# LPMP/BDD

Hardware: AMD Instinct MI355X
Metric: parallel-MMA iterations/sec, 10.5M BDD nodes, 1 GPU (+ achieved HBM GB/s in roofline) (higher is better)
Workload: dtype f32

## Files before the change

### bdd_amd/capi.py

```python
from __future__ import annotations

import ctypes as C
import os
import subprocess

_HERE = os.path.dirname(os.path.abspath(__file__))
LIB_PATH = os.path.abspath(os.environ["BDDMMA_LIB"]) if os.environ.get("BDDMMA_LIB") else os.path.join(_HERE, "csrc", "libbdd_mma_hip.so")

OK = 0
ERR_INVALID_ARGUMENT, ERR_INVALID_BDD, ERR_DEVICE, ERR_STATE, ERR_UNSUPPORTED, ERR_IO = -1, -2, -3, -4, -5, -6
F32, F64 = 0, 1
K_FORWARD_MM, K_BACKWARD_MM, K_FINISH_DELTA, K_OTHER, K_COUNT = 0, 1, 2, 3, 4


class Options(C.Structure):
    _fields_ = [("pack_width", C.c_uint32), ("wide_pack_width", C.c_uint32), ("deterministic", C.c_uint32),
                ("vars_per_bin", C.c_uint32), ("stage_cap", C.c_uint32), ("waves_per_block", C.c_uint32),
                ("keep_bdd_order", C.c_uint32), ("resident_sweeps", C.c_uint32), ("exchange_by_variable", C.c_uint32),
                ("variant_flags", C.c_uint32), ("pack_fill", C.c_uint32), ("pack_stagger", C.c_uint32)]


class LbfgsParams(C.Structure):
    _fields_ = [("history_size", C.c_int32), ("init_step_size", C.c_double), ("req_rel_lb_increase", C.c_double),
                ("step_size_decrease_factor", C.c_double), ("step_size_increase_factor", C.c_double)]


class LbfgsState(C.Structure):
    _fields_ = [("step_size", C.c_double), ("last_applied_step", C.c_double), ("mma_iterations", C.c_uint64),
                ("lbfgs_iterations", C.c_uint64), ("history_entries", C.c_int32), ("num_unsuccessful_updates", C.c_int32),
                ("last_kind", C.c_int32), ("last_trials", C.c_int32)]


class RunResult(C.Structure):
    _fields_ = [("iterations", C.c_uint64), ("lb_initial", C.c_double), ("lb_final", C.c_double),
                ("seconds", C.c_double), ("stop_reason", C.c_int32)]


class Profile(C.Structure):
    _fields_ = [("launches", C.c_uint64 * K_COUNT), ("total_ms", C.c_double * K_COUNT)]


_V, _U64, _I, _D = C.c_void_p, C.c_uint64, C.c_int, C.c_double
SIGNATURES = {
    "bddmma_create": (_I, [C.POINTER(_V), _I, _I, _V, _V, _U64, _V, _U64, C.POINTER(Options)]),
    "bddmma_destroy": (None, [_V]),
    "bddmma_device_count": (_I, []),
    "bddmma_device_chip": (_I, [_I, C.POINTER(C.c_uint32), C.POINTER(C.c_uint32), C.POINTER(C.c_uint64)]),
    "bddmma_set_layout_threads": (_I, [_I]),
    "bddmma_set_thread_layout_threads": (_I, [_I]),
    "bddmma_last_error": (C.c_char_p, [_V]),
    "bddmma_nr_variables": (_U64, [_V]),
    "bddmma_nr_bdds": (_U64, [_V]),
    "bddmma_nr_layers": (_U64, [_V]),
    "bddmma_nr_bdd_nodes": (_U64, [_V]),
    "bddmma_nr_hops": (_U64, [_V]),
    "bddmma_nr_packs": (_U64, [_V]),
    "bddmma_solve_sweep_kind": (_I, [_V]),
    "bddmma_fused_small": (_I, [_V]),
    "bddmma_nontemporal_loads": (_I, [_V]),
    "bddmma_precision": (_I, [_V]),
    "bddmma_device": (_I, [_V]),
    "bddmma_num_bdds_per_var": (_I, [_V, _V]),
    "bddmma_layer_variables": (_I, [_V, _V]),
    "bddmma_layer_bdds": (_I, [_V, _V]),
    "bddmma_nodes_per_hop": (_I, [_V, _V]),
    "bddmma_layers_per_hop": (_I, [_V, _V]),
    "bddmma_update_costs": (_I, [_V, _V, _U64, _V, _U64, _I, _I]),
    "bddmma_set_cost": (_I, [_V, _D, _U64]),
    "bddmma_get_solver_costs": (_I, [_V, _V, _V, _V, _I]),
    "bddmma_set_solver_costs": (_I, [_V, _V, _V, _V, _I]),
    "bddmma_primal_objective_vec": (_I, [_V, _V, _I]),
    "bddmma_forward_run": (_I, [_V]),
    "bddmma_backward_run": (_I, [_V]),
    "bddmma_lower_bound": (_I, [_V, C.POINTER(_D)]),
    "bddmma_lower_bound_per_bdd": (_I, [_V, _V, _I]),
    "bddmma_iteration": (_I, [_V, _D]),
    "bddmma_iterations": (_I, [_V, _D, _U64]),
    "bddmma_learned_iterations": (_I, [_V, _V, _I, _U64, _D, _D, _V, _V, _V, _U64, _D, _I, C.POINTER(_U64)]),
    "bddmma_learned_iterations_omega_vec": (_I, [_V, _V, _I, _U64, _V, _I, _D, _V, _V, _V, _U64, _D, _I, C.POINTER(_U64)]),
    "bddmma_isotropic_dist_weights": (_I, [_V, _V, _I]),
    "bddmma_forward_mm": (_I, [_V, _D, _V, _I]),
    "bddmma_backward_mm": (_I, [_V, _D, _V, _I]),
    "bddmma_normalize_delta": (_I, [_V, _V, _I]),
    "bddmma_distribute_delta": (_I, [_V]),
    "bddmma_get_delta": (_I, [_V, _V, _I]),
    "bddmma_set_delta": (_I, [_V, _V, _I]),
    "bddmma_min_marginals": (_I, [_V, _I, _V, _V, _V, _I]),
    "bddmma_min_marginal_diff": (_I, [_V, _V, _I]),
    "bddmma_sum_marginals": (_I, [_V, _I, _I, _V, _V, _V, _I]),
    "bddmma_smooth_solution": (_I, [_V, _V, _I]),
    "bddmma_grad_min_marginal_diff": (_I, [_V, _V, _V, _V, _I]),
    "bddmma_grad_lower_bound_per_bdd": (_I, [_V, _V, _V, _V, _I, _I]),
    "bddmma_grad_distribute_delta": (_I, [_V, _V, _V, _V, _I]),
    "bddmma_grad_cost_perturbation": (_I, [_V, _V, _V, _V, _V, _I]),
    "bddmma_grad_learned_iterations": (_I, [_V, _V, _I, _D, _V, _I, _V, _V, _V, _V, _V, _U64, _U64, _U64, _I]),
    "bddmma_bdds_solution": (_I, [_V, _I, _V, _I]),
    "bddmma_net_solver_costs": (_I, [_V, _V, _I]),
    "bddmma_make_dual_feasible": (_I, [_V, _V, _I]),
    "bddmma_gradient_step": (_I, [_V, _V, _D, _I]),
    "bddmma_lbfgs_create": (_I, [C.POINTER(_V), _V, C.POINTER(LbfgsParams)]),
    "bddmma_lbfgs_destroy": (None, [_V]),
    "bddmma_lbfgs_iteration": (_I, [_V]),
    "bddmma_lbfgs_update_costs": (_I, [_V, _V, _U64, _V, _U64, _I, _I]),
    "bddmma_lbfgs_flush": (_I, [_V]),
    "bddmma_lbfgs_get_state": (_I, [_V, C.POINTER(LbfgsState)]),
    "bddmma_perturb_primal_costs": (_I, [_V, _V, _D, C.c_uint32, C.c_uint32, C.POINTER(C.c_uint32), _V, _V, _V]),
    "bddmma_run_solver": (_I, [_V, _V, _U64, _D, _D, _D, _I, C.POINTER(RunResult)]),
    "bddmma_run_solver_host_loop": (_I, [_V, _V, _U64, _D, _D, _D, _I, C.POINTER(RunResult)]),
    "bddmma_batch_create": (_I, [C.POINTER(_V), C.POINTER(_V), _U64]),
    "bddmma_batch_destroy": (None, [_V]),
    "bddmma_batch_last_error": (C.c_char_p, [_V]),
    "bddmma_batch_size": (_U64, [_V]),
    "bddmma_batch_iterations": (_I, [_V, _D, _U64]),
    "bddmma_batch_time_iterations": (_I, [_V, _D, _U64, C.POINTER(_D)]),
    "bddmma_batch_run_solver": (_I, [_V, _U64, _D, _D, _D, C.POINTER(RunResult)]),
    "bddmma_batch_lower_bounds": (_I, [_V, C.POINTER(_D)]),
    "bddmma_incremental_mm_agreement_rounding": (_I, [_V, _V, _D, _D, _U64, _U64, C.c_uint32, _I, _V, C.POINTER(_I)]),
    "bddmma_save": (_I, [_V, C.c_char_p]),
    "bddmma_load": (_I, [C.POINTER(_V), _I, C.c_char_p]),
    "bddmma_synchronize": (_I, [_V]),
    "bddmma_set_profiling": (_I, [_V, _I]),
    "bddmma_get_profile": (_I, [_V, C.POINTER(Profile)]),
    "bddmma_time_iterations": (_I, [_V, _D, _U64, C.POINTER(_D)]),
    "bddmma_time_kernel": (_I, [_V, _I, _U64, C.POINTER(_D)]),
    "bddmma_device_bytes": (_U64, [_V]),
    "bddmma_device_allocated_bytes": (_U64, [_V]),
    "bddmma_layout_create": (_I, [C.POINTER(_V), _V, _V, _U64, C.POINTER(Options)]),
    "bddmma_layout_create_for_chip": (_I, [C.POINTER(_V), _V, _V, _U64, C.POINTER(Options), _I, C.c_uint32, C.c_uint32]),
    "bddmma_layout_destroy": (None, [_V]),
    "bddmma_layout_size": (_U64, [_V, _I]),
    "bddmma_layout_copy": (_I, [_V, _I, _V]),
    "bddmma_layout_res2_records": (_I, [_V, _I, _V, _V, _V]),
    "bddmma_layout_stream_records": (_I, [_V, _I, _V, _V, _V]),
    "bddmma_layout_layer_records": (_I, [_V, _I, _V, _V, _V]),
    "bddmma_layout_seg_exchange": (_I, [_V, _I, _I, _V, _V, _V, _V]),
}

_I64P, _U64P = C.POINTER(C.c_int64), C.POINTER(C.c_uint64)
ILP_SIGNATURES = {
    "bddilp_last_error": (C.c_char_p, []),
    "bddilp_parse_lp": (_I, [C.c_char_p, C.POINTER(_V)]),
    "bddilp_parse_opb": (_I, [C.c_char_p, C.POINTER(_V)]),
    "bddilp_parse": (_I, [C.c_char_p, C.POINTER(_V)]),
    "bddilp_destroy": (None, [_V]),
    "bddilp_nr_variables": (_U64, [_V]),
    "bddilp_nr_constraints": (_U64, [_V]),
    "bddilp_variable_name": (C.c_char_p, [_V, _U64]),
    "bddilp_objective": (_I, [_V, _V, C.POINTER(_D)]),
    "bddilp_constraint_size": (_U64, [_V, _U64]),
    "bddilp_constraint": (_I, [_V, _U64, _V, _V, C.POINTER(_I), C.POINTER(C.c_int64)]),
    "bddilp_constraint_name": (C.c_char_p, [_V, _U64]),
    "bddilp_normalize": (_I, [_V]),
    "bddilp_to_bdds": (_I, [_V, _I, _U64, C.POINTER(_V)]),
    "bddilp_bdds_create": (_I, [C.POINTER(_V)]),
    "bddilp_bdds_add_row": (_I, [_V, _V, _V, _U64, _I, C.c_int64, C.POINTER(_I)]),
    "bddilp_bdds_split": (_I, [_V, _U64, _U64, _I, _U64P, _U64P]),
    "bddilp_bdds_destroy": (None, [_V]),
    "bddilp_bdds_nr_bdds": (_U64, [_V]),
    "bddilp_bdds_nr_instructions": (_U64, [_V]),
    "bddilp_bdds_nr_variables": (_U64, [_V]),
    "bddilp_bdds_instructions": (_V, [_V]),
    "bddilp_bdds_delimiters": (_V, [_V]),
    "bddilp_write_bdd_lp": (_I, [_V, _V, _U64, _V, _U64, C.c_char_p]),
    "bddilp_export_graphviz": (_I, [_V, _V, _U64, _U64, C.c_char_p]),
    "bddilp_random_set_cover": (_I, [_U64, _U64, _U64, _U64, _V, _V]),
}

_lib = None


def build(verbose: bool = False) -> None:
    out = subprocess.run(["make", "-C", os.path.join(_HERE, "csrc"), "-j4"], capture_output=True, text=True)
    if out.returncode != 0:
        raise RuntimeError("building libbdd_mma_hip.so failed:\n" + out.stdout + out.stderr)
    if verbose:
        print(out.stdout)


def lib():
    global _lib
    if _lib is None:
        if not os.path.exists(LIB_PATH):
            raise RuntimeError(f"{LIB_PATH} is missing: run `make -C bdd_amd/csrc` (or __graft_entry__.build()); "
                               "bdd_amd has no CPU fallback")
        L = C.CDLL(LIB_PATH)
        for name, (res, args) in list(SIGNATURES.items()) + list(ILP_SIGNATURES.items()):
            f = getattr(L, name)
            f.restype = res
            f.argtypes = args
        _lib = L
    return _lib


class BddMmaError(RuntimeError):
    pass


def check(rc: int, handle=None):
    if rc != OK:
        msg = lib().bddmma_last_error(handle)
        raise BddMmaError(f"bdd_mma error {rc}: {msg.decode() if msg else ''}")
```

### bdd_amd/csrc/capi.cpp

```cpp
#include <chrono>
#include <cmath>
#include <cstdio>
#include <cstdlib>
#include <cstring>
#include <limits>
#include <new>
#include <string>
#include <vector>

#include "../../include/bdd_mma.h"
#include "layout.hpp"
#include "solver.hpp"

using namespace bddmma;

struct bddmma_lbfgs;
extern "C" int bddmma_lbfgs_iteration(bddmma_lbfgs* l);
extern "C" int bddmma_lbfgs_update_costs(bddmma_lbfgs* l, const void* lo, uint64_t n_lo, const void* hi, uint64_t n_hi, int elem_precision,
                                         int on_device);

namespace {
thread_local std::string g_err;

template <typename F>
int guarded(bddmma_solver* s, F&& f)
{
    if (!s || !s->impl) return BDDMMA_ERR_INVALID_ARGUMENT;
    try {
        return f(s->impl);
    } catch (const std::bad_alloc&) {
        s->impl->err = "out of host memory";
        return BDDMMA_ERR_DEVICE;
    } catch (const std::exception& e) {
        s->impl->err = e.what();
        return BDDMMA_ERR_DEVICE;
    }
}
template <typename F>
int guarded(const bddmma_solver* s, F&& f) { return guarded(const_cast<bddmma_solver*>(s), f); }

template <typename F>
int guarded_batch(bddmma_batch* b, F&& f)
{
    if (!b || !b->impl) return BDDMMA_ERR_INVALID_ARGUMENT;
    try {
        return f(b->impl);
    } catch (const std::exception& e) {
        b->impl->err = e.what();
        return BDDMMA_ERR_DEVICE;
    }
}

template <typename T>
int copy_host(const std::vector<T>& v, T* out)
{
    if (!out) return BDDMMA_ERR_INVALID_ARGUMENT;
    if (!v.empty()) std::memcpy(out, v.data(), v.size() * sizeof(T));
    return BDDMMA_OK;
}
}

extern "C" {

int bddmma_create(bddmma_solver** out, int precision, int device, const bddmma_instruction* instr,
                  const uint64_t* bdd_delims, uint64_t n_bdds, const double* costs_hi, uint64_t n_costs,
                  const bddmma_options* opts)
{
    if (!out) return BDDMMA_ERR_INVALID_ARGUMENT;
    *out = nullptr;
    try {
#ifdef BDDMMA_EXPERIMENTAL
        static const bool timing = std::getenv("BDDMMA_LAYOUT_TIMING") != nullptr;
#else
        constexpr bool timing = false;
#endif
        auto t_last = std::chrono::steady_clock::now();
        auto lap = [&](const char* what) {
            if (!timing) return;
            const auto now = std::chrono::steady_clock::now();
            std::fprintf(stderr, "[create] %-28s %8.1f ms\n", what, std::chrono::duration<double, std::milli>(now - t_last).count());
            t_last = now;
        };
        HostLayout L;
        ChipInfo chip;
        int rc = query_chip(device, &chip, g_err);
        if (rc) return rc;
        rc = build_layout(instr, bdd_delims, n_bdds, opts, L, g_err, false, precision == BDDMMA_F64 ? 8 : 4, chip);
        if (rc) return rc;
        lap("host layout");
        SolverBase* impl = nullptr;
        rc = create_solver(&impl, precision, device, L, opts, g_err);
        if (rc) return rc;
        lap("device buffers + upload");
        impl->n_packs_narrow = L.narrow.n_packs();
        impl->n_packs_wide = L.wide.n_packs() + L.huge.n_packs();
        if (costs_hi && n_costs) {
            rc = impl->update_costs(nullptr, 0, costs_hi, n_costs, BDDMMA_F64, 0);
            if (rc) {
                g_err = impl->err;
                delete impl;
                return rc;
            }
        }
        lap("update_costs");
        *out = new bddmma_solver{impl};
        return BDDMMA_OK;
    } catch (const std::exception& e) {
        g_err = e.what();
        return BDDMMA_ERR_DEVICE;
    }
}

int bddmma_device_count(void) { return device_count(); }
int bddmma_device_chip(int device, uint32_t* n_cus, uint32_t* lds_bytes_per_cu, uint64_t* max_resident_threads)
{
    if (device < 0 || device >= device_count()) { g_err = "no such HIP device"; return BDDMMA_ERR_DEVICE; }
    ChipInfo chip;
    const int rc = query_chip(device, &chip, g_err);
    if (rc) return rc;
    if (n_cus) *n_cus = chip.n_cus;
    if (lds_bytes_per_cu) *lds_bytes_per_cu = chip.lds_bytes;
    if (max_resident_threads) *max_resident_threads = chip.max_resident_threads;
    return BDDMMA_OK;
}
int bddmma_set_layout_threads(int n)
{
    if (n < 0) return BDDMMA_ERR_INVALID_ARGUMENT;
    set_layout_threads((unsigned)n);
    return BDDMMA_OK;
}
int bddmma_set_thread_layout_threads(int n)
{
    if (n < 0) return BDDMMA_ERR_INVALID_ARGUMENT;
    set_thread_layout_threads((unsigned)n);
    return BDDMMA_OK;
}

void bddmma_destroy(bddmma_solver* s)
{
    if (!s) return;
    delete s->impl;
    delete s;
}

const char* bddmma_last_error(const bddmma_solver* s) { return (s && s->impl) ? s->impl->err.c_str() : g_err.c_str(); }

uint64_t bddmma_nr_variables(const bddmma_solver* s) { return s && s->impl ? s->impl->n_vars : 0; }
uint64_t bddmma_nr_bdds(const bddmma_solver* s) { return s && s->impl ? s->impl->n_bdds : 0; }
uint64_t bddmma_nr_layers(const bddmma_solver* s) { return s && s->impl ? s->impl->n_layers : 0; }
uint64_t bddmma_nr_bdd_nodes(const bddmma_solver* s) { return s && s->impl ? s->impl->n_input_nodes : 0; }
uint64_t bddmma_nr_hops(const bddmma_solver* s) { return s && s->impl ? s->impl->n_hops : 0; }
uint64_t bddmma_nr_packs(const bddmma_solver* s) { return s && s->impl ? s->impl->n_packs_narrow + s->impl->n_packs_wide : 0; }
int bddmma_solve_sweep_kind(const bddmma_solver* s) { return s && s->impl ? s->impl->solve_sweep_kind : -1; }
int bddmma_fused_small(const bddmma_solver* s) { return s && s->impl ? (s->impl->fused_small ? 1 : 0) : -1; }
int bddmma_nontemporal_loads(const bddmma_solver* s) { return s && s->impl ? (s->impl->nt_loads ? 1 : 0) : -1; }
int bddmma_precision(const bddmma_solver* s) { return s && s->impl ? s->impl->precision : -1; }
int bddmma_device(const bddmma_solver* s) { return s && s->impl ? s->impl->device : -1; }
uint64_t bddmma_device_bytes(const bddmma_solver* s) { return s && s->impl ? s->impl->dev_bytes : 0; }
uint64_t bddmma_device_allocated_bytes(const bddmma_solver* s) { return s && s->impl ? s->impl->dev_alloc_bytes : 0; }

int bddmma_num_bdds_per_var(const bddmma_solver* s, int32_t* out)
{
    return guarded(s, [&](SolverBase* b) { return copy_host(b->h_nbdds, out); });
}
int bddmma_layer_variables(const bddmma_solver* s, int32_t* out)
{
    return guarded(s, [&](SolverBase* b) { return copy_host(b->h_layer_var, out); });
}
int bddmma_layer_bdds(const bddmma_solver* s, int32_t* out)
{
    return guarded(s, [&](SolverBase* b) { return copy_host(b->h_layer_bdd, out); });
}
int bddmma_nodes_per_hop(const bddmma_solver* s, uint64_t* out)
{
    return guarded(s, [&](SolverBase* b) { return copy_host(b->nodes_per_hop, out); });
}
int bddmma_layers_per_hop(const bddmma_solver* s, uint64_t* out)
{
    return guarded(s, [&](SolverBase* b) { return copy_host(b->layers_per_hop, out); });
}

int bddmma_update_costs(bddmma_solver* s, const void* lo, uint64_t n_lo, const void* hi, uint64_t n_hi,
                        int elem_precision, int on_device)
{
    return guarded(s, [&](SolverBase* b) {
        if (elem_precision != BDDMMA_F32 && elem_precision != BDDMMA_F64) {
            b->err = "elem_precision must be BDDMMA_F32 or BDDMMA_F64";
            return BDDMMA_ERR_INVALID_ARGUMENT;
        }
        return b->update_costs(lo, n_lo, hi, n_hi, elem_precision, on_device);
    });
}
int bddmma_set_cost(bddmma_solver* s, double c, uint64_t var)
{
    return guarded(s, [&](SolverBase* b) { return b->set_cost(c, var); });
}
int bddmma_get_solver_costs(const bddmma_solver* s, void* lo, void* hi, void* mm, int on_device)
{
    return guarded(s, [&](SolverBase* b) { return b->get_solver_costs(lo, hi, mm, on_device); });
}
int bddmma_set_solver_costs(bddmma_solver* s, const void* lo, const void* hi, const void* mm, int on_device)
{
    return guarded(s, [&](SolverBase* b) { return b->set_solver_costs(lo, hi, mm, on_device); });
}
int bddmma_primal_objective_vec(bddmma_solver* s, void* out, int on_device)
{
    return guarded(s, [&](SolverBase* b) { return b->primal_objective_vec(out, on_device); });
}
int bddmma_forward_run(bddmma_solver* s) { return guarded(s, [&](SolverBase* b) { return b->forward_run(); }); }
int bddmma_backward_run(bddmma_solver* s) { return guarded(s, [&](SolverBase* b) { return b->backward_run(); }); }
int bddmma_lower_bound(bddmma_solver* s, double* lb)
{
    return guarded(s, [&](SolverBase* b) { return lb ? b->lower_bound(lb) : BDDMMA_ERR_INVALID_ARGUMENT; });
}
int bddmma_lower_bound_per_bdd(bddmma_solver* s, void* out, int on_device)
{
    return guarded(s, [&](SolverBase* b) { return b->lower_bound_per_bdd(out, on_device); });
}
int bddmma_iteration(bddmma_solver* s, double omega)
{
    return guarded(s, [&](SolverBase* b) { return b->iteration(omega); });
}
int bddmma_iterations(bddmma_solver* s, double omega, uint64_t n)
{
    return guarded(s, [&](SolverBase* b) { return b->iterations(omega, n); });
}
int bddmma_learned_iterations(bddmma_solver* s, const void* dist_weights, int weights_on_device, uint64_t num_itr, double omega,
                              double improvement_slope, void* sol_avg, void* lb_first_diff_avg, void* lb_second_diff_avg,
                              uint64_t compute_history_for_itr, double history_avg_beta, int outputs_on_device, uint64_t* itr_done)
{
    return guarded(s, [&](SolverBase* b) {
        return b->learned_iterations(dist_weights, weights_on_device, num_itr, omega, improvement_slope, sol_avg, lb_first_diff_avg,
                                     lb_second_diff_avg, compute_history_for_itr, history_avg_beta, outputs_on_device, itr_done, nullptr, 0);
    });
}
int bddmma_learned_iterations_omega_vec(bddmma_solver* s, const void* dist_weights, int weights_on_device, uint64_t num_itr, const void* omega_vec,
                                        int omega_vec_on_device, double improvement_slope, void* sol_avg, void* lb_first_diff_avg,
                                        void* lb_second_diff_avg, uint64_t compute_history_for_itr, double history_avg_beta, int outputs_on_device,
                                        uint64_t* itr_done)
{
    return guarded(s, [&](SolverBase* b) {
        if (!omega_vec) {
            if (itr_done) *itr_done = 0;
            b->err = "learned_iterations: omega_vec is null";
            return BDDMMA_ERR_INVALID_ARGUMENT;
        }
        return b->learned_iterations(dist_weights, weights_on_device, num_itr, 0.0, improvement_slope, sol_avg, lb_first_diff_avg,
                                     lb_second_diff_avg, compute_history_for_itr, history_avg_beta, outputs_on_device, itr_done, omega_vec,
                                     omega_vec_on_device);
    });
}
int bddmma_isotropic_dist_weights(bddmma_solver* s, void* out, int on_device)
{
    return guarded(s, [&](SolverBase* b) { return out ? b->isotropic_dist_weights(out, on_device) : BDDMMA_ERR_INVALID_ARGUMENT; });
}
int bddmma_forward_mm(bddmma_solver* s, double omega, void* d, int on_device)
{
    return guarded(s, [&](SolverBase* b) { return d ? b->forward_mm(omega, d, on_device) : BDDMMA_ERR_INVALID_ARGUMENT; });
}
int bddmma_backward_mm(bddmma_solver* s, double omega, void* d, int on_device)
{
    return guarded(s, [&](SolverBase* b) { return d ? b->backward_mm(omega, d, on_device) : BDDMMA_ERR_INVALID_ARGUMENT; });
}
int bddmma_normalize_delta(const bddmma_solver* s, void* d, int on_device)
{
    return guarded(s, [&](SolverBase* b) { return d ? b->normalize_delta(d, on_device) : BDDMMA_ERR_INVALID_ARGUMENT; });
}
int bddmma_distribute_delta(bddmma_solver* s) { return guarded(s, [&](SolverBase* b) { return b->distribute_delta(); }); }
int bddmma_get_delta(const bddmma_solver* s, void* out, int on_device)
{
    return guarded(s, [&](SolverBase* b) { return out ? b->get_delta(out, on_device) : BDDMMA_ERR_INVALID_ARGUMENT; });
}
int bddmma_set_delta(bddmma_solver* s, const void* in, int on_device)
{
    return guarded(s, [&](SolverBase* b) { return in ? b->set_delta(in, on_device) : BDDMMA_ERR_INVALID_ARGUMENT; });
}
int bddmma_min_marginals(bddmma_solver* s, int sorted, int32_t* var, void* mm0, void* mm1, int on_device)
{
    return guarded(s, [&](SolverBase* b) { return b->min_marginals(sorted, var, mm0, mm1, on_device); });
}
int bddmma_min_marginal_diff(bddmma_solver* s, void* out, int on_device)
{
    return guarded(s, [&](SolverBase* b) { return out ? b->min_marginal_diff(out, on_device) : BDDMMA_ERR_INVALID_ARGUMENT; });
}
int bddmma_sum_marginals(bddmma_solver* s, int sorted, int log_probs, int32_t* var, void* sm0, void* sm1, int on_device)
{
    return guarded(s, [&](SolverBase* b) { return (sm0 && sm1) ? b->sum_marginals(sorted, log_probs, var, sm0, sm1, on_device) : BDDMMA_ERR_INVALID_ARGUMENT; });
}
int bddmma_smooth_solution(bddmma_solver* s, void* out, int on_device)
{
    return guarded(s, [&](SolverBase* b) { return out ? b->smooth_solution(out, on_device) : BDDMMA_ERR_INVALID_ARGUMENT; });
}
int bddmma_grad_min_marginal_diff(bddmma_solver* s, const void* grad_mm, void* grad_lo_out, void* grad_hi_out, int on_device)
{
    return guarded(s, [&](SolverBase* b) {
        return (grad_mm && grad_lo_out && grad_hi_out) ? b->grad_min_marginal_diff(grad_mm, grad_lo_out, grad_hi_out, on_device) : BDDMMA_ERR_INVALID_ARGUMENT;
    });
}
int bddmma_grad_lower_bound_per_bdd(bddmma_solver* s, const void* grad_lb_per_bdd, void* grad_lo_out, void* grad_hi_out, int smooth, int on_device)
{
    return guarded(s, [&](SolverBase* b) {
        return (grad_lb_per_bdd && grad_lo_out && grad_hi_out) ? b->grad_lower_bound_per_bdd(grad_lb_per_bdd, grad_lo_out, grad_hi_out, smooth, on_device)
                                                               : BDDMMA_ERR_INVALID_ARGUMENT;
    });
}
int bddmma_grad_distribute_delta(bddmma_solver* s, const void* grad_lo, const void* grad_hi, void* grad_deferred_mm_out, int on_device)
{
    return guarded(s, [&](SolverBase* b) {
// ... 671 lines not shown
```

### bdd_amd/csrc/kernels/common.hpp

```cpp
#pragma once

namespace bddmma {

enum : int { FWD_PLAIN = 0, FWD_SOLVE = 1, FWD_SOLUTION = 2 };
enum : int { BWD_PLAIN = 0, BWD_SOLVE = 1, BWD_MARGINALS = 2 };

template <typename REAL>
struct DevPtrs {
    const uint32_t* nwords;
    uint32_t n_nwords;
    const uint64_t* wwords;
    uint32_t wide_slot_base;
    REAL* F;
    REAL* T;
    REAL* lohi;
    const REAL* delta_lay;
    REAL* mm_binned;
    const uint32_t* lpos;
    const uint32_t* cs_entry;
    const uint16_t* cs_slot;
    uint32_t n_slots;
    uint32_t n_layers;
    uint32_t n_narrow_layers;
    double* lb_partial;
    REAL* x_layer;
    union {
        REAL* mm0_out;
        const REAL* omega_lay;
    };
    REAL* mm1_out;
    char* sol_out;
    const uint32_t* stop;
    uint32_t run_iter;
    uint32_t big;
};
struct RunGate {
    const uint32_t* stop = nullptr;
    uint32_t iter = 0;
};
constexpr uint32_t RUN_NOT_STOPPED = 0xFFFFFFFFu;

__device__ __forceinline__ bool run_stopped(const RunGate& g) { return g.stop != nullptr && *g.stop <= g.iter; }
#define BDDMMA_EXIT_IF(done_cond, dev)                                     \
    {                                                                      \
        const bool done_ = (done_cond);                                    \
        if (done_ | ((dev).stop != nullptr)) {                             \
            if (done_ || *(dev).stop <= (dev).run_iter) return;            \
        }                                                                  \
    }

struct PackDev {
    const uint32_t* pack_hop_ptr;
    const uint32_t* hop_node_off;
    const uint32_t* hop_layer_off;
    const uint8_t* pack_steps;
    const uint16_t* hop_root;
    const uint32_t* pack_word_off;
    const uint32_t* pack_group_ptr;
    const uint32_t* grp_layer_off;
    const uint32_t* grp_hop_end;
    const uint32_t* quad_round_ptr;
    const uint32_t* cs_ptr;
    uint32_t stage_cap;
    uint32_t seg_off;
    uint32_t n_packs;
    uint32_t lb_base;
    uint32_t nt_potentials;
    uint32_t xcd_chunk;
    const uint32_t* hdr_pack;
    const uint32_t* hdr_quad;
};

#ifdef BDDMMA_STAMPS
__device__ unsigned long long* g_bddmma_stamps = nullptr;
#define BDDMMA_STAMP(slot, idx)                                                                              \
    do {                                                                                                     \
        if (g_bddmma_stamps != nullptr) {                                                                    \
            asm volatile("s_waitcnt vmcnt(0) lgkmcnt(0)" ::: "memory");                                      \
            const unsigned long long t_ = __builtin_amdgcn_s_memrealtime();                      \
            if ((threadIdx.x & 63) == 0) g_bddmma_stamps[(size_t)(slot) * 8 + (idx)] = t_;                   \
        }                                                                                                    \
    } while (0)
#else
#define BDDMMA_STAMP(slot, idx) do { } while (0)
#endif

template <typename REAL> struct Pair;
template <> struct Pair<float> { using type = float2; };
template <> struct Pair<double> { using type = double2; };

template <typename REAL> __device__ __forceinline__ REAL inf_v();
template <> __device__ __forceinline__ float inf_v<float>() { return __builtin_huge_valf(); }
template <> __device__ __forceinline__ double inf_v<double>() { return __builtin_huge_val(); }

__device__ __forceinline__ float rmin(float a, float b) { return __builtin_fminf(a, b); }
__device__ __forceinline__ double rmin(double a, double b) { return __builtin_fmin(a, b); }
__device__ __forceinline__ bool rfinite(float a) { return __builtin_isfinite(a); }
__device__ __forceinline__ bool rfinite(double a) { return __builtin_isfinite(a); }

template <typename REAL>
__device__ __forceinline__ REAL mm_diff(REAL m0, REAL m1, REAL omega)
{
    const bool fin = (int)rfinite(m0) & (int)rfinite(m1);
    const REAL t = omega * (m1 - m0);
    return fin ? t : REAL(0);
}
template <bool OV, typename REAL>
__device__ __forceinline__ REAL omega_of(const DevPtrs<REAL>& d, REAL omega, uint32_t l)
{
    if constexpr (OV) return d.omega_lay[l];
    else return omega;
}
__device__ __forceinline__ float min0(float x)
{
    float r;
    asm("v_min_f32_e64 %0, %1, 0" : "=v"(r) : "v"(x));
    return r;
}
__device__ __forceinline__ float min0_neg(float x)
{
    float r;
    asm("v_min_f32_e64 %0, -%1, 0" : "=v"(r) : "v"(x));
    return r;
}
__device__ __forceinline__ double min0(double x) { return rmin(x, 0.0); }
__device__ __forceinline__ double min0_neg(double x) { return rmin(-x, 0.0); }

template <typename REAL>
__device__ __forceinline__ void lds_min(REAL* p, REAL v)
{
    __hip_atomic_fetch_min(p, v, __ATOMIC_RELAXED, __HIP_MEMORY_SCOPE_WORKGROUP);
}

template <bool GLOBAL, typename REAL>
__device__ __forceinline__ void frontier_min(REAL* p, REAL v)
{
    if (GLOBAL) __hip_atomic_fetch_min(p, v, __ATOMIC_RELAXED, __HIP_MEMORY_SCOPE_AGENT);
    else __hip_atomic_fetch_min(p, v, __ATOMIC_RELAXED, __HIP_MEMORY_SCOPE_WORKGROUP);
}
template <bool GLOBAL, typename REAL>
__device__ __forceinline__ REAL frontier_load(const REAL* p)
{
    if (GLOBAL) return __hip_atomic_load(p, __ATOMIC_RELAXED, __HIP_MEMORY_SCOPE_AGENT);
    return *p;
}

__device__ __forceinline__ uint32_t block_to_pack(uint32_t bid, uint32_t n_packs, uint32_t chunk)
{
    if (chunk == 0) {
        const uint32_t per = (n_packs + 7u) >> 3;
        return (bid & 7u) * per + (bid >> 3);
    }
    const uint32_t x = bid & 7u, i = bid >> 3;
    return ((i / chunk) * 8u + x) * chunk + i % chunk;
}

__device__ __forceinline__ float dpp_from_next(float v)
{
    const int x = __builtin_bit_cast(int, v);
    return __builtin_bit_cast(float, __builtin_amdgcn_update_dpp(x, x, 0x130, 0xF, 0xF, false));
}
__device__ __forceinline__ float dpp_from_prev(float v)
{
    const int x = __builtin_bit_cast(int, v);
    return __builtin_bit_cast(float, __builtin_amdgcn_update_dpp(x, x, 0x138, 0xF, 0xF, false));
}
__device__ __forceinline__ double dpp_from_next(double v)
{
    const long long x = __builtin_bit_cast(long long, v);
    const int lo = (int)x, hi = (int)(x >> 32);
    const unsigned int l2 = (unsigned int)__builtin_amdgcn_update_dpp(lo, lo, 0x130, 0xF, 0xF, false);
    const unsigned int h2 = (unsigned int)__builtin_amdgcn_update_dpp(hi, hi, 0x130, 0xF, 0xF, false);
    return __builtin_bit_cast(double, ((unsigned long long)h2 << 32) | l2);
}
#ifndef BDDMMA_SEG_FOLD_F32
#define BDDMMA_SEG_FOLD_F32 2
#endif
template <typename REAL>
constexpr int SEG_FOLD_STEPS = sizeof(REAL) == 4 ? BDDMMA_SEG_FOLD_F32 : 1;
template <int CTRL>
__device__ __forceinline__ float dpp_row(float v)
{
    const int x = __builtin_bit_cast(int, v);
    return __builtin_bit_cast(float, __builtin_amdgcn_update_dpp(x, x, CTRL, 0xF, 0xF, false));
}
template <int CTRL>
__device__ __forceinline__ double dpp_row(double v)
{
    const long long x = __builtin_bit_cast(long long, v);
    const int lo = (int)x, hi = (int)(x >> 32);
    const unsigned int l2 = (unsigned int)__builtin_amdgcn_update_dpp(lo, lo, CTRL, 0xF, 0xF, false);
    const unsigned int h2 = (unsigned int)__builtin_amdgcn_update_dpp(hi, hi, CTRL, 0xF, 0xF, false);
    return __builtin_bit_cast(double, ((unsigned long long)h2 << 32) | l2);
}
__device__ __forceinline__ double dpp_from_prev(double v)
{
    const long long x = __builtin_bit_cast(long long, v);
    const int lo = (int)x, hi = (int)(x >> 32);
    const unsigned int l2 = (unsigned int)__builtin_amdgcn_update_dpp(lo, lo, 0x138, 0xF, 0xF, false);
    const unsigned int h2 = (unsigned int)__builtin_amdgcn_update_dpp(hi, hi, 0x138, 0xF, 0xF, false);
    return __builtin_bit_cast(double, ((unsigned long long)h2 << 32) | l2);
}

__device__ __forceinline__ void seg_fence()
{
    __builtin_amdgcn_fence(__ATOMIC_RELEASE, "wavefront");
    __builtin_amdgcn_wave_barrier();
    __builtin_amdgcn_fence(__ATOMIC_ACQUIRE, "wavefront");
}
__device__ __forceinline__ void seg_pair_min(double& a, double& b, uint32_t pos, uint32_t len)
{
    const double a2 = dpp_from_next(a), b2 = dpp_from_next(b);
    if (pos == 0 && len == 2) {
        a = rmin(a, a2);
        b = rmin(b, b2);
    }
    const double a1 = dpp_from_prev(a), b1 = dpp_from_prev(b);
    if (pos == 1) {
        a = a1;
        b = b1;
    }
}
__device__ __forceinline__ void seg_pair_min(float& a, float& b, uint32_t pos, uint32_t len)
// ... 247 lines not shown
```

### bdd_amd/csrc/kernels/narrow3.hpp

```cpp
#pragma once

namespace bddmma {

constexpr int N3_W = 128;
template <typename REAL>
__device__ __forceinline__ void lds_ld2(REAL& a, REAL& b, const unsigned char* lds, uint32_t off)
{
    const REAL* p = reinterpret_cast<const REAL*>(lds + off);
    a = p[0];
    b = p[1];
}

template <typename REAL, bool NT>
__device__ __forceinline__ void pot_pair_load(typename Pair<REAL>::type& v, rsrc_t rh, uint32_t voff, uint32_t soff)
{
    constexpr int AUX = NT ? 2 : BDDMMA_LD_POT_AUX;
    if constexpr (sizeof(REAL) == 4) v = __builtin_bit_cast(float2, __builtin_amdgcn_raw_buffer_load_b64(rh, voff, soff, AUX));
    else v = __builtin_bit_cast(double2, __builtin_amdgcn_raw_buffer_load_b128(rh, voff, soff, AUX));
}

__device__ __forceinline__ void pot_store(float v, rsrc_t rh, uint32_t voff, uint32_t soff, uint32_t ) { hop_store(v, rh, voff, soff); }
__device__ __forceinline__ void pot_store(double v, rsrc_t rh, uint32_t voff, uint32_t soff, uint32_t nt)
{
    if (nt) hop_store<2>(v, rh, voff, soff);
    else hop_store<>(v, rh, voff, soff);
}

template <typename REAL>
__device__ __forceinline__ void pot_store_layer(REAL a, REAL b, bool two, rsrc_t rh, uint32_t off_a, uint32_t soff, uint32_t nt)
{
    using P2 = typename Pair<REAL>::type;
    const uint32_t off2 = two ? off_a : (uint32_t)LREC_NO_STORE, off1 = two ? (uint32_t)LREC_NO_STORE : off_a;
    P2 v;
    v.x = a;
    v.y = b;
    if constexpr (sizeof(REAL) == 4) {
        using u2 = decltype(__builtin_amdgcn_raw_buffer_load_b64(rh, 0, 0, 0));
        __builtin_amdgcn_raw_buffer_store_b64(__builtin_bit_cast(u2, v), rh, off2, soff, BDDMMA_ST_FT_AUX_F32);
        pot_store(a, rh, off1, soff, nt);
    } else {
        using u4 = decltype(__builtin_amdgcn_raw_buffer_load_b128(rh, 0, 0, 0));
        const u4 data = __builtin_bit_cast(u4, v);
        if (nt) __builtin_amdgcn_raw_buffer_store_b128(data, rh, off2, soff, 2);
        else __builtin_amdgcn_raw_buffer_store_b128(data, rh, off2, soff, BDDMMA_ST_AUX);
        asm volatile("s_nop 0" ::"v"(data) : "memory");
        pot_store(a, rh, off1, soff, nt);
    }
}

#ifndef BDDMMA_N3_LOOKAHEAD
#define BDDMMA_N3_LOOKAHEAD(REAL) (sizeof(REAL) == 8 ? 2 : BDDMMA_LOOKAHEAD)
#endif
template <typename REAL, int WPB, bool NT = false, int LA = BDDMMA_LOOKAHEAD, bool OV = false>
__device__ __forceinline__ void fwd_narrow3_body(const DevPtrs<REAL>& d, const PackDev& pk, const uint32_t* __restrict__ lrec,
                                                 const uint32_t* __restrict__ lrec_off, uint32_t lrec_words, REAL omega, uint32_t block_id)
{
    constexpr int W = N3_W;
    constexpr uint32_t S = sizeof(REAL);
    constexpr uint32_t BUF = (W + 128) * S;
    using P2 = typename Pair<REAL>::type;
    extern __shared__ __attribute__((aligned(16))) unsigned char dyn_lds[];
    P2* sD = reinterpret_cast<P2*>(dyn_lds);
    __shared__ __attribute__((aligned(16))) unsigned char sF_[WPB][2][BUF];
    __shared__ __attribute__((aligned(16))) unsigned char sT_[WPB][2][BUF];
    __shared__ uint32_t sOffN_[WPB][HOP_WIN], sOffL_[WPB][HOP_WIN], sOffR_[WPB][HOP_WIN];
    const uint32_t tid = threadIdx.x;
    const int wave = __builtin_amdgcn_readfirstlane((int)(tid >> 6));
    const int lane = tid & 63;
    unsigned char* sFw = &sF_[wave][0][0];
    unsigned char* sTw = &sT_[wave][0][0];
    const uint32_t n_quads = (pk.n_packs + WPB - 1) / WPB;
    const uint32_t quad = block_to_pack(block_id, n_quads, pk.xcd_chunk);
    BDDMMA_EXIT_IF(quad >= n_quads, d)
    const uint32_t p = quad * WPB + wave;
    const bool has_pack = p < pk.n_packs;
    const bool hdr = pk.hdr_pack != nullptr;
    const uint32_t* const hp = hdr ? pk.hdr_pack + 8 * (size_t)(has_pack ? p : 0) : nullptr;
    const uint32_t q0 = !has_pack ? 0 : (hdr ? hp[4] : pk.pack_hop_ptr[p]);
    const uint32_t q1 = !has_pack ? 0 : (hdr ? q0 + (hp[5] & 0xFFFFu) : pk.pack_hop_ptr[p + 1]);
    const uint32_t rbase = has_pack ? lrec_off[p] : 0;
    const uint32_t c0_h = hdr ? pk.hdr_quad[4 * (size_t)quad] : 0, cnt_h = hdr ? pk.hdr_quad[4 * (size_t)quad + 1] : 0;
    BDDMMA_STAMP(p, 0);
    const REAL INF = inf_v<REAL>();
    const uint32_t slot_first = !has_pack ? 0 : (hdr ? hp[0] : pk.hop_node_off[q0]), l0 = !has_pack ? 0 : (hdr ? hp[2] : pk.hop_layer_off[q0]);
    NarrowRs<REAL> rs(d);
    rs.rebase_layers(d, l0);
    uint32_t ent[STAGE_ITERS], esl[STAGE_ITERS];
    if (hdr) stage_load_tables<REAL, WPB, (NT ? 2 : BDDMMA_LD_TAB_AUX)>(ent, esl, rs, c0_h, cnt_h, tid);
    REAL* const Tp = d.T + slot_first;
    REAL* const Fp = d.F + slot_first;
    const REAL* const lohi_p = d.lohi + 2 * (size_t)l0;
    const rsrc_t rr = make_rsrc(lrec, lrec_words);
    HopWindow hw{sOffN_[wave], sOffL_[wave], sOffR_[wave], q0, q1, slot_first, l0};
    constexpr int D = LA;
    uint32_t o[2 * D + 3];
    uint32_t lb[D + 2];
    u4v rc[2 * D + 1];
    P2 tr[D + 1];
    P2 Lr[D + 1];
    REAL Wr[OV ? D + 1 : 1];
    const rsrc_t rw = omega_rsrc<OV>(d, l0);
#pragma unroll
    for (int i = 0; i < 2 * D + 3; ++i) o[i] = 0;
#pragma unroll
    for (int i = 0; i < D + 2; ++i) lb[i] = 0;
    auto ldrec = [&](uint32_t h) { return __builtin_amdgcn_raw_buffer_load_b128(rr, (uint32_t)lane * 16u, (rbase + h * 64u) * 16u, 0); };
    const uint32_t sink = (W + 2 * (uint32_t)lane) * S;
    if (has_pack) {
        hw.fill(pk, q0, lane);
#pragma unroll
        for (int i = 0; i < 2 * D + 3; ++i) o[i] = hw.node_off(q0 + i);
#pragma unroll
        for (int i = 0; i < D + 2; ++i) lb[i] = hw.layer_off(q0 + i);
#pragma unroll
        for (int r = 0; r < 2; ++r) {
            const uint32_t j = lane + 64 * r;
            lds_st<REAL>(sFw, j * S, (j < o[1] - o[0]) ? REAL(0) : INF);
        }
#pragma unroll
        for (int b = 0; b < 2; ++b) {
            lds_st<REAL>(sTw, b * BUF + sink, REAL(0));
            lds_st<REAL>(sTw, b * BUF + sink + S, INF);
        }
#pragma unroll
        for (int i = 0; i < 2 * D; ++i) rc[i] = ldrec((uint32_t)i);
        {
            P2 t1;
            pot_pair_load<REAL, NT>(t1, hop_rsrc(Tp, o[1], o[2] - o[1]), 2u * (uint32_t)lane * S, o[1] * S);
#pragma unroll
            for (int i = 0; i < D; ++i) pot_pair_load<REAL, NT>(tr[i], hop_rsrc(Tp, o[i + 2], o[i + 3] - o[i + 2]), 2u * (uint32_t)lane * S, o[i + 2] * S);
            if (2u * (uint32_t)lane < o[2] - o[1]) lds_st<P2>(sTw, 2u * (uint32_t)lane * S, t1);
        }
#pragma unroll
        for (int i = 0; i < D; ++i) hop_load(Lr[i], rs.lohi, (uint32_t)lane * (uint32_t)sizeof(P2), lb[i] * (uint32_t)sizeof(P2));
        if constexpr (OV) {
#pragma unroll
            for (int i = 0; i < D; ++i) hop_load(Wr[i], rw, (uint32_t)lane * S, lb[i] * S);
        }
        wave_sync();
    } else {
#pragma unroll
        for (int i = 0; i < 2 * D; ++i) rc[i] = u4v{0u, 0u, 0u, 0u};
    }
    uint32_t cur = 0;
    uint32_t q = q0;
    const uint32_t g0 = (has_pack && !hdr) ? pk.pack_group_ptr[p] : 0;
    const uint32_t ng = !has_pack ? 0 : (hdr ? 1u : pk.pack_group_ptr[p + 1] - g0);
    const uint32_t r0 = hdr ? 0 : pk.quad_round_ptr[quad];
    const uint32_t n_rounds = hdr ? 1u : pk.quad_round_ptr[quad + 1] - r0;
    const uint32_t db = (uint32_t)wave * pk.stage_cap * (uint32_t)sizeof(P2);
    for (uint32_t k = 0; k < n_rounds; ++k) {
    uint32_t gl0 = 0, cnt = 0, qe = q1;
    if (hdr) {
        cnt = cnt_h;
        stage_load_pairs<REAL, WPB>(sD, ent, esl, rs, cnt, tid);
        qe = has_pack ? q1 : q;
    } else {
        const uint32_t c0 = pk.cs_ptr[r0 + k];
        cnt = pk.cs_ptr[r0 + k + 1] - c0;
        stage_load<REAL, WPB, (NT ? 2 : BDDMMA_LD_TAB_AUX)>(sD, ent, esl, rs, c0, cnt, tid);
        if (k < ng) {
            gl0 = pk.grp_layer_off[g0 + k] - l0;
            qe = pk.grp_hop_end[g0 + k];
        } else {
            qe = q;
        }
    }
    if (WPB > 1) __syncthreads(); else wave_sync();
    BDDMMA_STAMP(p, 1);
    auto hop = [&]() {
        if (q + 2 * D + 3 >= hw.base + HOP_WIN && hw.base + HOP_WIN <= q1) hw.fill(pk, q, lane);
        const uint32_t nb = o[0];
        const uint32_t n3 = o[3] - o[2];
        const uint32_t fc = cur * BUF, fn = (cur ^ 1u) * BUF;
        const uint32_t stg = db + (lb[0] - gl0 + (uint32_t)lane) * (uint32_t)sizeof(P2);
        rc[2 * D] = ldrec(q - q0 + 2 * D);
#ifndef BDDMMA_EXP_NO_HOP_LOADS
        pot_pair_load<REAL, NT>(tr[D], hop_rsrc(Tp, o[D + 2], o[D + 3] - o[D + 2]), 2u * (uint32_t)lane * S, o[D + 2] * S);
        hop_load(Lr[D], rs.lohi, (uint32_t)lane * (uint32_t)sizeof(P2), lb[D] * (uint32_t)sizeof(P2));
        if constexpr (OV) hop_load(Wr[D], rw, (uint32_t)lane * S, lb[D] * S);
#endif
        const u4v ra = rc[0];
        const P2 c = Lr[0];
        const uint32_t flags = ra[2] >> 16;
        REAL fa, fb;
        lds_ld2(fa, fb, sFw, fc + (ra[2] & 0xFFFFu));
        const REAL tla = lds_ld<REAL>(sTw, fc + (ra[0] & 0xFFFFu)), tha = lds_ld<REAL>(sTw, fc + (ra[0] >> 16));
        const REAL tlb = lds_ld<REAL>(sTw, fc + (ra[1] & 0xFFFFu)), thb = lds_ld<REAL>(sTw, fc + (ra[1] >> 16));
        const P2 dd = lds_ld<P2>(dyn_lds, stg);
        const uint32_t o_new = hw.node_off(q + 2 * D + 3);
        const uint32_t l_next = hw.layer_off(q + D + 2);
        if (2u * (uint32_t)lane < n3) lds_st<P2>(sTw, fn + 2u * (uint32_t)lane * S, tr[0]);
        lds_st<P2>(sFw, fn + 2u * (uint32_t)lane * S, P2{INF, INF});
        wave_sync();
        fa = (flags & LREC_REAL) ? fa : INF;
        fb = (flags & LREC_TWO) ? fb : INF;
        const REAL m0 = rmin((fa + c.x) + tla, (fb + c.x) + tlb);
        const REAL m1 = rmin((fa + c.y) + tha, (fb + c.y) + thb);
        const REAL mm = mm_diff1(m0, m1, OV ? Wr[0] : omega);
        P2 nc;
        nc.x = (c.x + min0(mm)) + dd.x;
        nc.y = (c.y + min0_neg(mm)) + dd.y;
#ifndef BDDMMA_EXP_NO_HOP_STORES
        const rsrc_t rl = hop_rsrc(reinterpret_cast<const P2*>(lohi_p), lb[0], lb[1] - lb[0]);
        hop_store(nc, rl, (uint32_t)lane * (uint32_t)sizeof(P2), lb[0] * (uint32_t)sizeof(P2));
#endif
        if (flags & LREC_REAL) lds_st<REAL>(dyn_lds, stg, mm);
        lds_min(reinterpret_cast<REAL*>(sFw + fn + (ra[0] & 0xFFFFu)), fa + nc.x);
        lds_min(reinterpret_cast<REAL*>(sFw + fn + (ra[0] >> 16)), fa + nc.y);
        lds_min(reinterpret_cast<REAL*>(sFw + fn + (ra[1] & 0xFFFFu)), fb + nc.x);
        lds_min(reinterpret_cast<REAL*>(sFw + fn + (ra[1] >> 16)), fb + nc.y);
#ifndef BDDMMA_EXP_NO_HOP_STORES
        {
            const rsrc_t rf = hop_rsrc(Fp, nb, o[1] - o[0]);
            pot_store_layer<REAL>(fa, fb, (flags & LREC_TWO) != 0, rf, ra[3] & 0xFFFFu, nb * S, pk.nt_potentials);
        }
#endif
        wave_sync();
        cur ^= 1u;
        shift(o, o_new);
        shift(lb, l_next);
        shift(rc);
        shift(Lr);
        shift(tr);
        shift(Wr);
        ++q;
    };
    while (q + HOP_UNROLL <= qe) {
#pragma unroll
        for (int u = 0; u < HOP_UNROLL; ++u) hop();
    }
    while (q < qe) hop();
    BDDMMA_STAMP(p, 3);
    if (WPB > 1) __syncthreads(); else wave_sync();
    BDDMMA_STAMP(p, 2);
    stage_flush<REAL, WPB>(sD, ent, esl, rs, cnt, tid);
    BDDMMA_STAMP(p, 4);
    if (WPB > 1 && k + 1 < n_rounds) __syncthreads();
    }
}

#ifndef BDDMMA_N3_WAVES
#define BDDMMA_N3_WAVES(REAL) (sizeof(REAL) == 4 ? 5 : 4)
#endif
template <typename REAL, int WPB, bool NT = false, bool OV = false>
__global__ void __launch_bounds__(64 * WPB) __attribute__((amdgpu_waves_per_eu(BDDMMA_N3_WAVES(REAL)))) k_fwd_narrow3(DevPtrs<REAL> d, PackDev pk, const uint32_t* __restrict__ lrec, const uint32_t* __restrict__ lrec_off,
                                                          uint32_t lrec_words, REAL omega)
{
    fwd_narrow3_body<REAL, WPB, NT, BDDMMA_N3_LOOKAHEAD(REAL), OV>(d, pk, lrec, lrec_off, lrec_words, omega, blockIdx.x);
}

template <typename REAL, int WPB, bool NT = false, int LA = BDDMMA_LOOKAHEAD, bool OV = false>
__device__ __forceinline__ void bwd_narrow3_body(const DevPtrs<REAL>& d, const PackDev& pk, const uint32_t* __restrict__ lrec,
                                                 const uint32_t* __restrict__ lrec_off, uint32_t lrec_words, REAL omega, uint32_t block_id)
{
    constexpr int W = N3_W;
    constexpr uint32_t S = sizeof(REAL);
    constexpr uint32_t BUF = (W + 128) * S;
    using P2 = typename Pair<REAL>::type;
    extern __shared__ __attribute__((aligned(16))) unsigned char dyn_lds[];
    P2* sD = reinterpret_cast<P2*>(dyn_lds);
    __shared__ __attribute__((aligned(16))) unsigned char sT_[WPB][2][BUF];
    __shared__ uint32_t sOffN_[WPB][HOP_WIN], sOffL_[WPB][HOP_WIN], sOffR_[WPB][HOP_WIN];
    const uint32_t tid = threadIdx.x;
    const int wave = __builtin_amdgcn_readfirstlane((int)(tid >> 6));
    const int lane = tid & 63;
    unsigned char* sTw = &sT_[wave][0][0];
    const uint32_t n_quads = (pk.n_packs + WPB - 1) / WPB;
    const uint32_t quad = block_to_pack(block_id, n_quads, pk.xcd_chunk);
    BDDMMA_EXIT_IF(quad >= n_quads, d)
    const uint32_t p = quad * WPB + wave;
    const bool has_pack = p < pk.n_packs;
    const bool hdr = pk.hdr_pack != nullptr;
    const uint32_t* const hp = hdr ? pk.hdr_pack + 8 * (size_t)(has_pack ? p : 0) : nullptr;
    const uint32_t q0 = !has_pack ? 0 : (hdr ? hp[4] : pk.pack_hop_ptr[p]);
    const uint32_t q1 = !has_pack ? 0 : (hdr ? q0 + (hp[5] & 0xFFFFu) : pk.pack_hop_ptr[p + 1]);
    const uint32_t rbase = has_pack ? lrec_off[p] : 0;
    const uint32_t c0_h = hdr ? pk.hdr_quad[4 * (size_t)quad] : 0, cnt_h = hdr ? pk.hdr_quad[4 * (size_t)quad + 1] : 0;
    BDDMMA_STAMP(p, 0);
    const REAL INF = inf_v<REAL>();
    const uint32_t slot_first = !has_pack ? 0 : (hdr ? hp[0] : pk.hop_node_off[q0]), l0 = !has_pack ? 0 : (hdr ? hp[2] : pk.hop_layer_off[q0]);
    NarrowRs<REAL> rs(d);
    rs.rebase_layers(d, l0);
    uint32_t ent[STAGE_ITERS], esl[STAGE_ITERS];
    if (hdr) stage_load_tables<REAL, WPB, (NT ? 2 : BDDMMA_LD_TAB_AUX)>(ent, esl, rs, c0_h, cnt_h, tid);
    REAL* const Tp = d.T + slot_first;
    REAL* const Fp = d.F + slot_first;
    const REAL* const lohi_p = d.lohi + 2 * (size_t)l0;
    REAL* const x_p = d.x_layer != nullptr ? d.x_layer + l0 : nullptr;
    const rsrc_t rr = make_rsrc(lrec, lrec_words);
    HopWindow hw{sOffN_[wave], sOffL_[wave], sOffR_[wave], q0, q1, slot_first, l0};
    auto nb_of = [&](uint32_t qq) { return hw.node_off(qq); };
    constexpr int D = LA;
    uint32_t o[2 * D + 2];
    uint32_t lb[D + 2];
    u4v rc[2 * D + 1];
    P2 fr[D + 1];
    P2 Lr[D + 1];
    REAL Wr[OV ? D + 1 : 1];
    const rsrc_t rw = omega_rsrc<OV>(d, l0);
#pragma unroll
    for (int i = 0; i < 2 * D + 2; ++i) o[i] = 0;
#pragma unroll
    for (int i = 0; i < D + 2; ++i) lb[i] = 0;
    uint32_t q = q1;
    auto ldrec = [&](uint32_t qq) { return __builtin_amdgcn_raw_buffer_load_b128(rr, (uint32_t)lane * 16u, (rbase + (qq >= q0 ? qq - q0 : 0u) * 64u) * 16u, 0); };
    auto ldf = [&](P2& f, const u4v& r, uint32_t nb, uint32_t n) {
        pot_pair_load<REAL, NT>(f, hop_rsrc(Fp, nb, n), r[3] & 0xFFFFu, nb * S);
    };
    const uint32_t sink = (W + 2 * (uint32_t)lane) * S;
    if (has_pack) {
#pragma unroll
        for (int b = 0; b < 2; ++b) {
            lds_st<REAL>(sTw, b * BUF + sink, REAL(0));
            lds_st<REAL>(sTw, b * BUF + sink + S, INF);
        }
        hw.fill(pk, q1 + 1 > q0 + HOP_WIN ? q1 + 1 - HOP_WIN : q0, lane);
#pragma unroll
        for (int i = 0; i < 2 * D + 2; ++i) o[i] = nb_of(q1 >= q0 + i ? q1 - i : q0);
#pragma unroll
        for (int i = 0; i < D + 2; ++i) lb[i] = hw.layer_off(q1 >= q0 + i ? q1 - i : q0);
#pragma unroll
        for (int i = 0; i < 2 * D; ++i) rc[i] = ldrec(q1 >= q0 + i + 1 ? q1 - 1 - i : q0);
#pragma unroll
        for (int i = 0; i < D; ++i) {
            ldf(fr[i], rc[i], o[i + 1], o[i] - o[i + 1]);
            hop_load(Lr[i], rs.lohi, (uint32_t)lane * (uint32_t)sizeof(P2), lb[i + 1] * (uint32_t)sizeof(P2));
            if constexpr (OV) hop_load(Wr[i], rw, (uint32_t)lane * S, lb[i + 1] * S);
        }
    } else {
#pragma unroll
        for (int i = 0; i < 2 * D; ++i) rc[i] = u4v{0u, 0u, 0u, 0u};
    }
    uint32_t cur = 0;
    const uint32_t g0 = (has_pack && !hdr) ? pk.pack_group_ptr[p] : 0;
    const uint32_t ng = !has_pack ? 0 : (hdr ? 1u : pk.pack_group_ptr[p + 1] - g0);
    const uint32_t r0 = hdr ? 0 : pk.quad_round_ptr[quad];
    const uint32_t n_rounds = hdr ? 1u : pk.quad_round_ptr[quad + 1] - r0;
    const uint32_t db = (uint32_t)wave * pk.stage_cap * (uint32_t)sizeof(P2);
    for (uint32_t k = n_rounds; k-- > 0;) {
    uint32_t gl0 = 0, cnt = 0, qs = q0;
    if (hdr) {
        cnt = cnt_h;
        stage_load_pairs<REAL, WPB>(sD, ent, esl, rs, cnt, tid);
        qs = has_pack ? q0 : q;
    } else {
        const uint32_t c0 = pk.cs_ptr[r0 + k];
        cnt = pk.cs_ptr[r0 + k + 1] - c0;
        stage_load<REAL, WPB, (NT ? 2 : BDDMMA_LD_TAB_AUX)>(sD, ent, esl, rs, c0, cnt, tid);
        if (k < ng) {
            gl0 = pk.grp_layer_off[g0 + k] - l0;
            qs = (k == 0) ? q0 : pk.grp_hop_end[g0 + k - 1];
        } else {
            qs = q;
        }
    }
    if (WPB > 1) __syncthreads(); else wave_sync();
    BDDMMA_STAMP(p, 1);
    auto hop = [&]() {
        --q;
        if (q < hw.base + 2 * D + 1 && hw.base > q0) hw.fill(pk, q + 1 > q0 + HOP_WIN ? q + 1 - HOP_WIN : q0, lane);
        const uint32_t nb = o[1];
        const uint32_t tc = cur * BUF, tn = (cur ^ 1u) * BUF;
        const uint32_t stg = db + (lb[1] - gl0 + (uint32_t)lane) * (uint32_t)sizeof(P2);
        rc[2 * D] = ldrec(q >= q0 + 2 * D ? q - 2 * D : q0);
#ifndef BDDMMA_EXP_NO_HOP_LOADS
        ldf(fr[D], rc[D], o[D + 1], o[D] - o[D + 1]);
        hop_load(Lr[D], rs.lohi, (uint32_t)lane * (uint32_t)sizeof(P2), lb[D + 1] * (uint32_t)sizeof(P2));
        if constexpr (OV) hop_load(Wr[D], rw, (uint32_t)lane * S, lb[D + 1] * S);
#endif
        const u4v ra = rc[0];
        const P2 c = Lr[0];
        const uint32_t flags = ra[2] >> 16;
        const REAL tla = lds_ld<REAL>(sTw, tc + (ra[0] & 0xFFFFu)), tha = lds_ld<REAL>(sTw, tc + (ra[0] >> 16));
        const REAL tlb = lds_ld<REAL>(sTw, tc + (ra[1] & 0xFFFFu)), thb = lds_ld<REAL>(sTw, tc + (ra[1] >> 16));
        const P2 dd = lds_ld<P2>(dyn_lds, stg);
        const uint32_t o_new = (q >= q0 + 2 * D + 1) ? nb_of(q - 1 - 2 * D) : o[2 * D + 1];
        const uint32_t l_next = hw.layer_off(q >= q0 + D + 1 ? q - 1 - D : q0);
        const REAL fa = (flags & LREC_REAL) ? fr[0].x : INF;
        const REAL fb = (flags & LREC_TWO) ? fr[0].y : INF;
        const REAL m0 = rmin((fa + c.x) + tla, (fb + c.x) + tlb);
        const REAL m1 = rmin((fa + c.y) + tha, (fb + c.y) + thb);
        const REAL mm = mm_diff1(m0, m1, OV ? Wr[0] : omega);
        P2 nc;
        nc.x = (c.x + min0(mm)) + dd.x;
        nc.y = (c.y + min0_neg(mm)) + dd.y;
        const REAL ta = rmin(nc.y + tha, nc.x + tla);
        const REAL tb = rmin(nc.y + thb, nc.x + tlb);
#ifndef BDDMMA_EXP_NO_HOP_STORES
        const rsrc_t rl = hop_rsrc(reinterpret_cast<const P2*>(lohi_p), lb[1], lb[0] - lb[1]);
        hop_store(nc, rl, (uint32_t)lane * (uint32_t)sizeof(P2), lb[1] * (uint32_t)sizeof(P2));
#endif
        if (flags & LREC_REAL) {
            lds_st<REAL>(dyn_lds, stg, mm);
            lds_st<REAL>(sTw, tn + (ra[2] & 0xFFFFu), ta);
        }
        if (flags & LREC_TWO) lds_st<REAL>(sTw, tn + (ra[2] & 0xFFFFu) + S, tb);
        if (x_p != nullptr) {
            const rsrc_t rx = hop_rsrc(x_p, lb[1], lb[0] - lb[1]);
            hop_store((nc.y - nc.x) + mm, rx, (uint32_t)lane * S, lb[1] * S);
        }
#ifndef BDDMMA_EXP_NO_HOP_STORES
        {
            const rsrc_t rt = hop_rsrc(Tp, nb, o[0] - o[1]);
            pot_store_layer<REAL>(ta, tb, (flags & LREC_TWO) != 0, rt, ra[3] & 0xFFFFu, nb * S, pk.nt_potentials);
        }
#endif
        wave_sync();
        cur ^= 1u;
        shift(o, o_new);
        shift(lb, l_next);
        shift(rc);
        shift(Lr);
        shift(fr);
        shift(Wr);
    };
    while (q >= qs + HOP_UNROLL) {
#pragma unroll
        for (int u = 0; u < HOP_UNROLL; ++u) hop();
    }
    while (q > qs) hop();
    BDDMMA_STAMP(p, 3);
    if (WPB > 1) __syncthreads(); else wave_sync();
    BDDMMA_STAMP(p, 2);
    stage_flush<REAL, WPB>(sD, ent, esl, rs, cnt, tid);
    BDDMMA_STAMP(p, 4);
    if (WPB > 1 && k > 0) __syncthreads();
    }
    if (!has_pack) return;
    const uint32_t n0 = nb_of(q0 + 1) - nb_of(q0);
    double s = 0.0;
#pragma unroll
    for (int r = 0; r < 2; ++r) {
        const uint32_t j = lane + 64 * r;
        if (j < n0) s += (double)lds_ld<REAL>(sTw, cur * BUF + j * S);
    }
    for (int off2 = 32; off2 > 0; off2 >>= 1) s += __shfl_down(s, off2);
    if (lane == 0) d.lb_partial[pk.lb_base + p] = s;
}

template <typename REAL, int WPB, bool NT = false, bool OV = false>
__global__ void __launch_bounds__(64 * WPB) __attribute__((amdgpu_waves_per_eu(BDDMMA_N3_WAVES(REAL)))) k_bwd_narrow3(DevPtrs<REAL> d, PackDev pk, const uint32_t* __restrict__ lrec, const uint32_t* __restrict__ lrec_off,
                                                          uint32_t lrec_words, REAL omega)
{
    bwd_narrow3_body<REAL, WPB, NT, BDDMMA_N3_LOOKAHEAD(REAL), OV>(d, pk, lrec, lrec_off, lrec_words, omega, blockIdx.x);
}

}
```

### bdd_amd/csrc/solver.hpp

```cpp
#pragma once
#include <hip/hip_runtime.h>

#include <cstdint>
#include <limits>
#include <memory>
#include <string>
#include <utility>
#include <vector>

#include "../../include/bdd_mma.h"
#include "layout.hpp"

namespace bddmma {

struct SolverBase {
    int precision = BDDMMA_F32, device = -1;
    hipStream_t stream = nullptr;
    std::string err;
    uint64_t n_vars = 0, n_bdds = 0, n_layers = 0, n_hops = 0, n_input_nodes = 0, n_slots = 0;
    int solve_sweep_kind = 0;
    uint32_t pack_width = 0, wide_pack_width = 0, wide_slot_base = 0;
    uint64_t dev_bytes = 0;
    uint64_t dev_alloc_bytes = 0;
    bool fwd_valid = false, bwd_valid = false;
    uint64_t cost_epoch = 0;
    bool deterministic = false;
    std::vector<uint64_t> nodes_per_hop, layers_per_hop;
    std::vector<int32_t> h_nbdds, h_layer_var, h_layer_bdd;
    std::vector<uint32_t> h_var_ptr;
    uint32_t n_packs_narrow = 0, n_packs_wide = 0;
    LayoutScalars lay_scalars{};
    bddmma_options saved_opts{};
    virtual int download_layout(HostLayout& H) = 0;
    virtual int init_from_layout(const HostLayout& L, const bddmma_options* opts) = 0;

    bool profiling = false;
    uint32_t prof_stride = 1;
    uint64_t prof_iter = 0;
    bool prof_active = false;
    std::vector<std::pair<hipEvent_t, hipEvent_t>> ev_pool;
    std::vector<int> ev_class;
    size_t ev_used = 0;
    hipEvent_t ev_t0 = nullptr, ev_t1 = nullptr;

    virtual ~SolverBase() {}
    virtual int forward_run() = 0;
    virtual int backward_run() = 0;
    virtual int lower_bound(double* lb) = 0;
    virtual int lower_bound_enqueue(int slot) = 0;
    virtual int lower_bound_fetch(int slot, double* lb) = 0;
    virtual int lower_bound_per_bdd(void* out, int on_device) = 0;
    virtual int iteration(double omega) = 0;
    virtual int iterations(double omega, uint64_t n)
    {
        for (uint64_t i = 0; i < n; ++i)
            if (int rc = iteration(omega)) return rc;
        return BDDMMA_OK;
    }
    virtual int learned_iterations(const void* dist_weights, int weights_on_device, uint64_t num_itr, double omega, double improvement_slope,
                                   void* sol_avg, void* lb_first_diff_avg, void* lb_second_diff_avg, uint64_t compute_history_for_itr,
                                   double history_avg_beta, int outputs_on_device, uint64_t* itr_done, const void* omega_vec,
                                   int omega_vec_on_device) = 0;
    virtual int isotropic_dist_weights(void* out, int on_device) = 0;
    double initial_lb_change = std::numeric_limits<double>::infinity();
    std::shared_ptr<int> lbfgs_attached = std::make_shared<int>(0);
    bool fused_small = false;
    bool nt_loads = false;
    virtual int run_plain(uint64_t max_iter, double tolerance, double slope, double time_limit, int verbose, bddmma_run_result* res) = 0;
    virtual int forward_mm(double omega, void* delta, int on_device) = 0;
    virtual int backward_mm(double omega, void* delta, int on_device) = 0;
    virtual int normalize_delta(void* delta, int on_device) = 0;
    virtual int distribute_delta() = 0;
    virtual int get_delta(void* out, int on_device) = 0;
    virtual int set_delta(const void* in, int on_device) = 0;
    virtual int update_costs(const void* lo, uint64_t n_lo, const void* hi, uint64_t n_hi, int elem_precision, int on_device) = 0;
    virtual int set_cost(double c, uint64_t var) = 0;
    virtual int get_solver_costs(void* lo, void* hi, void* mm, int on_device) = 0;
    virtual int set_solver_costs(const void* lo, const void* hi, const void* mm, int on_device) = 0;
    virtual int primal_objective_vec(void* out, int on_device) = 0;
    virtual int min_marginals(int sorted, int32_t* var, void* mm0, void* mm1, int on_device) = 0;
    virtual int min_marginal_diff(void* out, int on_device) = 0;
    virtual int sum_marginals(int sorted, int log_probs, int32_t* var, void* sm0, void* sm1, int on_device) = 0;
    virtual int smooth_solution(void* out, int on_device) = 0;
    virtual int grad_min_marginal_diff(const void* grad_mm, void* grad_lo, void* grad_hi, int on_device) = 0;
    virtual int grad_lower_bound_per_bdd(const void* grad_lb, void* grad_lo, void* grad_hi, int smooth, int on_device) = 0;
    virtual int grad_distribute_delta(const void* grad_lo, const void* grad_hi, void* grad_deferred_mm, int on_device) = 0;
    virtual int grad_cost_perturbation(const void* grad_lo, const void* grad_hi, void* grad_lo_pert, void* grad_hi_pert, int on_device) = 0;
    virtual int grad_learned_iterations(const void* dist_weights, int weights_on_device, double omega, const void* omega_vec, int omega_vec_on_device,
                                        void* grad_lo, void* grad_hi, void* grad_mm, void* grad_dist_weights_out, void* grad_omega_out, uint64_t after,
                                        uint64_t n, uint64_t num_caches, int on_device) = 0;
    virtual int bdds_solution(int sorted, char* sol, int on_device) = 0;
    virtual int net_solver_costs(void* out, int on_device) = 0;
    virtual int make_dual_feasible(void* g, int on_device) = 0;
    virtual int gradient_step(const void* g, double step, int on_device) = 0;
    virtual int projection_means(const void* g_dev) = 0;
    virtual int gradient_step_projected(const void* g_dev, double step) = 0;
    virtual bool projection_fuses_lincomb() const = 0;
    virtual int projection_means_lincomb(const LinComb& lc, const void* tag) = 0;
    virtual void* stream_handle() = 0;
    struct LbfgsViews {
        const void* x_layer;
    };
    virtual int bdds_solution_async(char* dev_out, int prezeroed) = 0;
    virtual int lbfgs_views(LbfgsViews* out) = 0;
    virtual int time_kernel(int kind, uint64_t reps, double* ms) = 0;
    virtual int rounding_round(double delta, uint32_t round, uint32_t seed, uint32_t counts[4], char* sol_host, void* c0_host, void* c1_host,
                               bool apply_update, int* applied) = 0;
    virtual int rounding_scratch(void** c0_dev, void** c1_dev) = 0;

    int synchronize();
    void prof_begin(int kclass);
    void prof_end(int kclass);
    int set_profiling(int on);
    int get_profile(bddmma_profile* out);
    int time_iterations(double omega, uint64_t n, double* ms);
};

struct BatchBase {
    std::string err;
    virtual ~BatchBase() {}
    virtual uint64_t size() const = 0;
    virtual int iterations(double omega, uint64_t n) = 0;
    virtual int run_plain(uint64_t max_iter, double tolerance, double slope, double time_limit, bddmma_run_result* res) = 0;
    virtual int time_iterations(double omega, uint64_t n, double* ms) = 0;
    virtual int lower_bounds(double* out) = 0;
};
int create_batch(BatchBase** out, SolverBase* const* members, uint64_t n, std::string& err);

int device_count();
int query_chip(int device, ChipInfo* out, std::string& err);
int create_solver(SolverBase** out, int precision, int device, const HostLayout& L, const bddmma_options* opts, std::string& err);

}

struct bddmma_solver {
    bddmma::SolverBase* impl = nullptr;
};
struct bddmma_batch {
    bddmma::BatchBase* impl = nullptr;
};
```

### bdd_amd/csrc/solver_impl.hpp

```cpp
#pragma once
#include <hip/hip_runtime.h>
#include <atomic>
#include <chrono>
#include <cmath>
#include <cstdio>
#include <cstdlib>
#include <cstring>
#include <limits>
#include <memory>
#include <string>
#include <thread>
#include <type_traits>
#include <vector>
#include "../../include/bdd_mma.h"
#include "kernels.hpp"
#include "layout.hpp"
#include "solver.hpp"

namespace bddmma {

static inline void cpu_relax()
{
#if defined(__x86_64__) || defined(__i386__)
    __asm__ __volatile__("pause");
#elif defined(__aarch64__)
    __asm__ __volatile__("yield");
#else
    std::this_thread::yield();
#endif
}


#define HIPCHK(expr)                                                                                   \
    do {                                                                                               \
        hipError_t e_ = (expr);                                                                        \
        if (e_ != hipSuccess) {                                                                        \
            err = std::string(#expr) + ": " + hipGetErrorString(e_);                                   \
            return BDDMMA_ERR_DEVICE;                                                                  \
        }                                                                                              \
    } while (0)

static inline uint32_t cdiv(uint64_t a, uint32_t b) { return (uint32_t)((a + b - 1) / b); }

template <int V0, int... Vs, class F>
decltype(auto) pick(uint32_t v, F&& f)
{
    if constexpr (sizeof...(Vs) == 0) return f(std::integral_constant<int, V0>{});
    else return v == (uint32_t)V0 ? f(std::integral_constant<int, V0>{}) : pick<Vs...>(v, static_cast<F&&>(f));
}

template <typename REAL, typename... TAIL>
struct PullSweep {
    using Fn = void (*)(DevPtrs<REAL>, PackDev, const uint32_t*, const uint32_t*, uint32_t, unsigned char*, TAIL...);
    Fn narrow, wide, huge;
    size_t (*bytes)(size_t, uint32_t);
    unsigned char* scratch;
};

#ifndef BDDMMA_EX_ACC
#define BDDMMA_EX_ACC double
#endif
template <typename REAL>
struct SolverT final : SolverBase {
    uint32_t* d_nwords = nullptr;
    uint32_t* d_pack_word_off = nullptr;
    uint32_t n_nwords = 0;
    uint64_t* d_wwords = nullptr;
    REAL *d_F = nullptr, *d_T = nullptr, *d_lohi = nullptr;
    REAL* d_lo = nullptr;
    REAL* d_hi = nullptr;
    int32_t *d_var = nullptr, *d_bdd = nullptr, *d_nbdds = nullptr;
    uint32_t *d_var_ptr = nullptr, *d_var_layers = nullptr, *d_root_slot = nullptr;
    REAL* d_delta_var = nullptr;
    bool delta_var_valid = true;
    REAL* d_delta_lay = nullptr;
    REAL* d_mm_binned = nullptr;
    REAL *d_delta_c = nullptr, *d_delta_lay_c = nullptr;
    REAL* d_alpha_ent = nullptr;
    REAL* d_omega_lay = nullptr;
    REAL* d_hist = nullptr;
    REAL* d_hist_out = nullptr;
    uint16_t* d_bvar = nullptr;
    uint32_t *d_evar = nullptr, *d_lpos = nullptr, *d_vpos = nullptr, *d_bin_ptr = nullptr;
    uint32_t *d_pack_group_ptr = nullptr, *d_grp_layer_off = nullptr, *d_grp_hop_end = nullptr;
    uint32_t *d_quad_round_ptr = nullptr, *d_cs_ptr = nullptr, *d_cs_entry = nullptr;
    uint16_t* d_cs_slot = nullptr;
    uint32_t wpb = 1;
    bool entry_by_var = false;
    bool exch_small = false, exch_medium = false;
    bool use_seg = false;
    uint32_t *d_seg_bin = nullptr, *d_seg_thr = nullptr;
    uint16_t* d_seg_perm = nullptr;
    uint32_t seg_lds = 0, seg_tile_off = 0, seg_cnt_off = 0, seg_groups = 0;
    bool big = false;
    uint32_t opts_variant = 0;
    uint32_t n_cus = 256, lds_cu = 160 * 1024;
    bool narrow_seg = false;
    uint32_t vars_per_bin = 0, n_bins = 0, stage_cap = 0, stage_lds = 0, exch_lds = 0, n_narrow_layers = 0;
    double *d_lb_partial = nullptr, *d_lb = nullptr;
    double* h_lb = nullptr;
    uint64_t *h_lb_seq = nullptr, *d_lb_seq = nullptr;
    uint64_t lb_seq_next = 0, lb_seq_expect[3] = {0, 0, 0};
    bool lb_cached = false;
    double lb_cache = 0.0;
    bool lb_slot_known[2] = {false, false}, lb_slot_enqueued[2] = {false, false};
    double lb_slot_value[2] = {0.0, 0.0};
    uint64_t lb_gen = 0, lb_slot_gen[2] = {0, 0};
    RunCtl* d_run_ctl = nullptr;
    RunHost *h_run = nullptr, *d_run_host = nullptr;
    const uint32_t* run_stop = nullptr;
    uint32_t run_iter = 0;
    RunGate gate() const { return RunGate{run_stop, run_iter}; }
    RunStep run_step{};
    REAL* d_x_layer = nullptr;
    bool x_layer_valid = false;
    void costs_changed()
    {
        fwd_valid = bwd_valid = x_layer_valid = false;
        ++cost_epoch;
    }
    CostQuot* d_cost_q = nullptr;
    uint8_t* d_cost_flags = nullptr;
    uint32_t* d_counts = nullptr;
    REAL *d_tmp0 = nullptr, *d_tmp1 = nullptr;
    char* d_sol = nullptr;
    struct PackBufs {
        uint32_t *pack_hop_ptr = nullptr, *hop_node_off = nullptr, *hop_layer_off = nullptr;
        uint8_t* pack_steps = nullptr;
        uint16_t* hop_root = nullptr;
        uint32_t n_packs = 0;
    } nb_, wb_, hb_;
    uint32_t wide_lds = 0, wide_threads = 256, wide_npt = 1;
    bool n3_nt = false;
    bool beyond_cache = false;
    bool n12_nt = false;
    uint32_t nt_potentials = 0;
    bool mixed = false;
    bool mixed_fwd = true;
    uint32_t mixed_npt = 1, mixed_lds = 0;
    uint32_t *d_pack_hdr = nullptr, *d_quad_hdr = nullptr;
    bool use_res = false;
    uint32_t res_ns = 0, res_nl = 0, res_lds = 0;
    bool use_res2 = false;
    uint32_t *d_res2_rec = nullptr, *d_res2_rec_off = nullptr;
    uint32_t res2_n_words = 0, res2_lds = 0, res2_ns = 0, res2_nl = 0;
    bool use_narrow2 = false, narrow_gen = false;
    uint32_t *d_srec = nullptr, *d_srec_off = nullptr;
    bool res_hdr_ok = false;
    const uint32_t* n2_hdr_pack() const { return res_hdr_ok ? d_pack_hdr : nullptr; }
    const uint32_t* n2_hdr_quad() const { return res_hdr_ok ? d_quad_hdr : nullptr; }
    uint32_t srec_words = 0;
    bool small_ok = false, small_rl = false;
    int small_nw = 1;
    uint32_t small_lds = 0;
    SmallDev small{};
    uint32_t* d_small_lds = nullptr;
    bool use_narrow3 = false;
    uint32_t *d_lrec = nullptr, *d_lrec_off = nullptr;
    uint32_t lrec_words = 0;
    uint32_t huge_pack_width = 0;
    unsigned char* d_huge_scratch = nullptr;

    std::vector<void*> allocs;

    ~SolverT() override
    {
        if (device >= 0) (void)hipSetDevice(device);
        for (void* p : allocs) (void)hipFree(p);
        if (h_lb) (void)hipHostFree(h_lb);
        if (h_lb_seq) (void)hipHostFree(h_lb_seq);
        if (h_run) (void)hipHostFree(h_run);
        if (d_run_ctl) (void)hipFree(d_run_ctl);
        for (auto& e : ev_pool) {
            (void)hipEventDestroy(e.first);
            (void)hipEventDestroy(e.second);
        }
        if (ev_t0) (void)hipEventDestroy(ev_t0);
        if (ev_t1) (void)hipEventDestroy(ev_t1);
        if (stream) (void)hipStreamDestroy(stream);
    }

    struct Arena { char* base = nullptr; uint64_t size = 0, used = 0; };
    std::vector<Arena> arenas;
    uint64_t arena_chunk = 0;
    uint64_t arena_skew = 0;
    template <typename T>
    int dalloc(T** p, uint64_t n)
    {
        const uint64_t bytes = std::max<uint64_t>(n, 1) * sizeof(T) + 1024;
        if (arena_chunk == 0) {
            HIPCHK(hipMalloc((void**)p, bytes));
            allocs.push_back(*p);
            dev_bytes += bytes;
            dev_alloc_bytes += bytes;
            return BDDMMA_OK;
        }
        const uint64_t need = (bytes + 4095) / 4096 * 4096 + arena_skew;
        if (arenas.empty() || arenas.back().used + need > arenas.back().size) {
            Arena a;
            a.size = std::max(arenas.empty() ? arena_chunk : std::min<uint64_t>(arena_chunk, 64ull << 20), need);
            HIPCHK(hipMalloc((void**)&a.base, a.size));
            allocs.push_back(a.base);
            arenas.push_back(a);
            dev_alloc_bytes += a.size;
        }
        Arena& a = arenas.back();
        *p = reinterpret_cast<T*>(a.base + a.used);
        a.used += need;
        dev_bytes += bytes;
        return BDDMMA_OK;
    }
    struct DevField { const void* ptr = nullptr; uint64_t count = 0; };
    DevField dev_fields[LAYOUT_ARRAY_IDS];
    template <typename T>
    int upload(T** p, const std::vector<T>& h, int id = 0)
    {
        int rc = dalloc(p, h.size());
        if (rc) return rc;
        if (!h.empty()) HIPCHK(hipMemcpyAsync(*p, h.data(), h.size() * sizeof(T), hipMemcpyHostToDevice, stream));
        if (id) dev_fields[id] = DevField{*p, h.size()};
        return BDDMMA_OK;
    }
    int download_layout(HostLayout& H) override
    {
        HIPCHK(hipSetDevice(device));
        H = HostLayout();
        set_layout_scalars(H, lay_scalars);
        hipError_t e = hipSuccess;
        visit_layout_arrays(H, [&](int id, auto& vec) {
            using T = typename std::remove_reference_t<decltype(vec)>::value_type;
            if (id == 36) { vec.assign(nodes_per_hop.begin(), nodes_per_hop.end()); return; }
            if (id == 37) { vec.assign(layers_per_hop.begin(), layers_per_hop.end()); return; }
            const DevField& f = dev_fields[id];
            vec.resize(f.count);
            if (f.count && e == hipSuccess) e = hipMemcpyAsync(vec.data(), f.ptr, f.count * sizeof(T), hipMemcpyDeviceToHost, stream);
        });
        if (e == hipSuccess) e = hipStreamSynchronize(stream);
        HIPCHK(e);
        return BDDMMA_OK;
    }
    int upload_packs(PackBufs& b, const PackSet& ps, int id0)
    {
        b.n_packs = ps.n_packs();
        int rc;
        if ((rc = upload(&b.pack_hop_ptr, ps.pack_hop_ptr, id0))) return rc;
        if ((rc = upload(&b.hop_node_off, ps.hop_node_off, id0 + 1))) return rc;
        if ((rc = upload(&b.hop_layer_off, ps.hop_layer_off, id0 + 2))) return rc;
        if ((rc = upload(&b.pack_steps, ps.pack_steps, id0 + 3))) return rc;
        return BDDMMA_OK;
    }

    int init_from_layout(const HostLayout& L, const bddmma_options* opts) override { return init(L, opts); }
    int init(const HostLayout& L, const bddmma_options* opts)
    {
        HIPCHK(hipSetDevice(device));
        {
            ChipInfo chip;
            std::string e;
            if (query_chip(device, &chip, e)) { err = e; return BDDMMA_ERR_DEVICE; }
            n_cus = chip.n_cus;
            lds_cu = chip.lds_bytes;
        }
        HIPCHK(hipStreamCreateWithFlags(&stream, hipStreamNonBlocking));
        HIPCHK(hipEventCreate(&ev_t0));
        HIPCHK(hipEventCreate(&ev_t1));
        n_vars = L.n_vars; n_bdds = L.n_bdds; n_layers = L.n_layers; n_hops = L.n_hops;
        n_input_nodes = L.n_input_nodes; n_slots = L.n_slots; pack_width = L.pack_width;
        wide_pack_width = L.wide_pack_width;
        nodes_per_hop = L.nodes_per_hop; layers_per_hop = L.layers_per_hop;
        h_nbdds = L.num_bdds_per_var; h_var_ptr = L.var_ptr;
        h_layer_var = L.layer_var; h_layer_bdd = L.layer_bdd;
        lay_scalars = layout_scalars(L);
        if (opts) saved_opts = *opts;
        deterministic = opts && opts->deterministic;
        {
            const uint64_t est = (uint64_t)n_slots * 2 * sizeof(REAL) + (uint64_t)n_layers * (5 * sizeof(REAL) + 24) + (uint64_t)n_vars * 24 +
                                 L.narrow_words_unique.size() * 4 + L.wide_words.size() * 8;
            const uint64_t want = est + est / 2 + est / 8 + std::min<uint64_t>(16ull << 20, est / 2 + (1ull << 20));
            if (want <= (640ull << 20)) arena_chunk = (want + (2ull << 20) - 1) / (2ull << 20) * (2ull << 20);
#ifdef BDDMMA_EXPERIMENTAL
            if (const char* ar = std::getenv("BDDMMA_EXP_ARENA")) {
                unsigned long long mib = 0, skew = 0;
                if (std::sscanf(ar, "%llu,%llu", &mib, &skew) >= 1) { arena_chunk = mib << 20; arena_skew = skew; }
            }
#endif
        }
        big = (uint64_t)n_slots * sizeof(REAL) >= 0xFFFF0000ull || 2ull * n_layers * sizeof(REAL) >= 0xFFFF0000ull || (opts && (opts->variant_flags & 0x4000u));
        if ((uint64_t)n_slots * sizeof(REAL) >= 0xFFFF0000ull || 2ull * n_layers * sizeof(REAL) >= 0xFFFF0000ull) {
            if (L.wide.n_packs() || L.huge.n_packs() || deterministic || L.ex.entry_by_var) {
                err = "instance too large for the 32-bit buffer offsets of this configuration: " + std::to_string(n_slots) + " node slots, " +
                      std::to_string(n_layers) + " layers of " + std::to_string(sizeof(REAL)) +
                      "-byte values (arrays of 4 GiB and more are supported for narrow packs with the binned exchange)";
                return BDDMMA_ERR_UNSUPPORTED;
            }
        }
        int rc;
        if ((rc = upload(&d_nwords, L.narrow_words_unique, 1))) return rc;
        n_nwords = (uint32_t)L.narrow_words_unique.size();
        if ((rc = upload(&d_pack_word_off, L.narrow_word_off, 2))) return rc;
        if ((rc = upload(&d_wwords, L.wide_words, 3))) return rc;
        if ((rc = upload(&d_var, L.layer_var, 4))) return rc;
        if ((rc = upload(&d_bdd, L.layer_bdd, 5))) return rc;
        if ((rc = upload(&d_nbdds, L.num_bdds_per_var, 6))) return rc;
        if ((rc = upload(&d_var_ptr, L.var_ptr, 7))) return rc;
        if ((rc = upload(&d_var_layers, L.var_layers, 8))) return rc;
        if ((rc = upload(&d_root_slot, L.bdd_root_slot, 9))) return rc;
        if ((rc = upload_packs(nb_, L.narrow, 10))) return rc;
        if (L.narrow.hop_root.size() + 1 != L.narrow.hop_node_off.size() && !L.narrow.hop_node_off.empty()) {
            err = "narrow hop_root table does not match the hop records";
            return BDDMMA_ERR_INVALID_ARGUMENT;
// ... 11 lines not shown
        wide_slot_base = L.narrow_slots;
        if ((rc = dalloc(&d_F, n_slots))) return rc;
        if ((rc = dalloc(&d_T, n_slots))) return rc;
        if ((rc = dalloc(&d_lohi, 2 * n_layers + 2))) return rc;
        d_lo = d_lohi;
        d_hi = d_lohi + 1;
        if ((rc = dalloc(&d_mm_binned, n_layers))) return rc;
        if ((rc = dalloc(&d_delta_lay, 2 * n_layers))) return rc;
        if ((rc = dalloc(&d_delta_lay_c, 2 * n_layers))) return rc;
        if ((rc = upload(&d_evar, L.ex.evar, 22))) return rc;
        if ((rc = upload(&d_bvar, L.ex.bvar, 23))) return rc;
        if ((rc = upload(&d_lpos, L.ex.lpos, 24))) return rc;
        if ((rc = upload(&d_vpos, L.ex.vpos, 25))) return rc;
        if ((rc = upload(&d_bin_ptr, L.ex.bin_ptr, 26))) return rc;
        if ((rc = upload(&d_pack_group_ptr, L.ex.pack_group_ptr, 27))) return rc;
        if ((rc = upload(&d_grp_layer_off, L.ex.grp_layer_off, 28))) return rc;
        if ((rc = upload(&d_grp_hop_end, L.ex.grp_hop_end, 29))) return rc;
        if ((rc = upload(&d_quad_round_ptr, L.ex.quad_round_ptr, 30))) return rc;
        if ((rc = upload(&d_cs_ptr, L.ex.cs_ptr, 31))) return rc;
        if ((rc = upload(&d_cs_entry, L.ex.cs_entry, 32))) return rc;
        if ((rc = upload(&d_cs_slot, L.ex.cs_slot, 33))) return rc;
        wpb = L.ex.waves_per_block;
        entry_by_var = L.ex.entry_by_var;
        {
            const uint32_t P = L.narrow.n_packs();
            if (P >= 64) {
                uint64_t part[8] = {0, 0, 0, 0, 0, 0, 0, 0}, total = 0;
                const uint32_t per = (P + 7) / 8;
                for (uint32_t p = 0; p < P; ++p) {
                    const uint32_t h = L.narrow.pack_hop_ptr[p + 1] - L.narrow.pack_hop_ptr[p];
                    part[std::min<uint32_t>(7, p / per)] += h;
                    total += h;
                }
                uint64_t mx = 0;
                for (uint64_t v : part) mx = std::max(mx, v);
                if (mx * 8 * 10 > total * 11) xcd_chunk_auto = 32;
            }
        }
        for (uint8_t st : L.narrow.pack_steps) narrow_seg = narrow_seg || st >= 2;
        vars_per_bin = L.ex.vars_per_bin; n_bins = L.ex.n_bins; stage_cap = L.ex.stage_cap;
        n_narrow_layers = L.ex.grp_layer_off.empty() ? 0 : L.ex.grp_layer_off.back();
        stage_lds = L.ex.waves_per_block * stage_cap * 2 * (uint32_t)sizeof(REAL);
        exch_lds = vars_per_bin * 2 * (uint32_t)sizeof(double);
        const uint32_t narrow_static = L.ex.waves_per_block * (3 * (pack_width + 2) * (uint32_t)sizeof(REAL) + 2 * 64 * 4 + 2) + seg_bytes(L.ex.waves_per_block);
        if (exch_lds > lds_cu - 1024 || stage_lds + narrow_static > lds_cu - 1024) {
            err = "vars_per_bin / stage_cap / waves_per_block need more LDS than a CU has (" + std::to_string(stage_lds + narrow_static) + " B per sweep workgroup)";
            return BDDMMA_ERR_INVALID_ARGUMENT;
        }
        if ((rc = dalloc(&d_tmp0, n_layers))) return rc;
        if ((rc = dalloc(&d_tmp1, n_layers))) return rc;
        if ((rc = dalloc(&d_sol, n_layers))) return rc;
        if ((rc = dalloc(&d_delta_var, 2 * n_vars))) return rc;
        if ((rc = dalloc(&d_delta_c, 2 * n_vars))) return rc;
        if ((rc = dalloc(&d_lb_partial, nb_.n_packs + wb_.n_packs + hb_.n_packs))) return rc;
        HIPCHK(hipHostMalloc((void**)&h_lb, 3 * sizeof(double), hipHostMallocMapped | hipHostMallocCoherent));
        HIPCHK(hipHostGetDevicePointer((void**)&d_lb, h_lb, 0));
        HIPCHK(hipHostMalloc((void**)&h_lb_seq, 3 * sizeof(uint64_t), hipHostMallocMapped | hipHostMallocCoherent));
        HIPCHK(hipHostGetDevicePointer((void**)&d_lb_seq, h_lb_seq, 0));
        std::memset((void*)h_lb_seq, 0, 3 * sizeof(uint64_t));
        if ((rc = dalloc(&d_counts, 4))) return rc;
        HIPCHK(hipMemsetAsync(d_F, 0, n_slots * sizeof(REAL), stream));
        HIPCHK(hipMemsetAsync(d_T, 0, n_slots * sizeof(REAL), stream));
        HIPCHK(hipMemsetAsync(d_lohi, 0, 2 * n_layers * sizeof(REAL), stream));
        HIPCHK(hipMemsetAsync(d_mm_binned, 0, n_layers * sizeof(REAL), stream));
        for (REAL* p : {d_delta_var, d_delta_c}) HIPCHK(hipMemsetAsync(p, 0, 2 * n_vars * sizeof(REAL), stream));
        for (REAL* p : {d_delta_lay, d_delta_lay_c}) HIPCHK(hipMemsetAsync(p, 0, 2 * n_layers * sizeof(REAL), stream));
        opts_variant = opts ? opts->variant_flags : 0u;
        mixed_fwd = (opts_variant & 2u) == 0;
        beyond_cache = dev_bytes > (640ull << 20);
        nt_potentials = (sizeof(REAL) == 8 && beyond_cache) ? 1u : 0u;
        exch_small = vars_per_bin <= EXS_MAX_VARS_PER_BIN;
        exch_medium = !exch_small && vars_per_bin <= EXM_MAX_VARS_PER_BIN;
        if (deterministic && !entry_by_var && !big && !(opts_variant & 0x20000u)) {
            const uint32_t T = exch_small ? EXS_THREADS : exch_medium ? EXM_THREADS : EX_THREADS;
            SegExchange SE;
            build_seg_exchange(L, T, (uint32_t)sizeof(REAL), SE);
            constexpr uint32_t VEC = 16 / sizeof(REAL);
            if (SE.ok && SE.max_groups <= 4 && SE.max_entries <= (uint64_t)SEG_MAXL * T * VEC) {
                const uint32_t Z = (SE.max_entries + VEC - 1) / VEC * VEC;
                seg_tile_off = ((Z + 1) * (uint32_t)sizeof(REAL) + 15u) & ~15u;
                seg_cnt_off = seg_tile_off + SE.max_slots * 2u * (uint32_t)sizeof(REAL);
                seg_lds = (seg_cnt_off + SE.max_slots * 2u + 15u) & ~15u;
                if (seg_lds + 1024 <= lds_cu) {
                    if ((rc = upload(&d_seg_bin, SE.bin))) return rc;
                    if ((rc = upload(&d_seg_perm, SE.perm))) return rc;
                    if ((rc = upload(&d_seg_thr, SE.thr))) return rc;
                    use_seg = true;
                    seg_groups = SE.max_groups;
                }
            }
        }
        if ((rc = upload(&d_pack_hdr, L.res.pack_hdr, 34))) return rc;
        if ((rc = upload(&d_quad_hdr, L.res.quad_hdr, 35))) return rc;
        res_hdr_ok = L.res.ok && nb_.n_packs > 0;
        if (nb_.n_packs && L.res.ok) {
            res_ns = (L.res.max_slots + 255) / 256 * 256;
            res_nl = (L.res.max_layers + 127) / 128 * 128;
            res_lds = wpb * stage_cap * 2 * (uint32_t)sizeof(REAL) + wpb * res_wave_bytes(sizeof(REAL), res_ns, res_nl);
            const uint32_t static_lds = wpb * (2 * (pack_width + 2) * (uint32_t)sizeof(REAL) + 512) + seg_bytes(wpb);
            const uint32_t mode = opts ? opts->resident_sweeps : 0;
            const bool fits = res_lds + static_lds <= lds_cu - 512;
            const uint64_t wgs_per_cu = fits ? (lds_cu) / (res_lds + static_lds) : 0;
            const bool all_in_flight = (uint64_t)nb_.n_packs * 256 <= 2880ull * n_cus && (uint64_t)cdiv(nb_.n_packs, wpb) <= (uint64_t)n_cus * std::min<uint64_t>(wgs_per_cu, 2048 / (64 * wpb));
            use_res = fits && mode != 1 && (mode == 2 || all_in_flight) && !big;
            if (pack_width == 64 && !narrow_seg && mode != 1 && !big && !(opts && (opts->variant_flags & 0x800u))) {
                res2_ns = res2_slot_capacity((uint32_t)sizeof(REAL), L.res.max_slots);
                res2_nl = res2_layer_capacity((uint32_t)sizeof(REAL), L.res.max_layers);
                res2_lds = wpb * stage_cap * 2 * (uint32_t)sizeof(REAL) + wpb * res2_wave_bytes(sizeof(REAL), res2_ns, res2_nl);
                const uint64_t wgs2 = res2_lds + 256 <= lds_cu ? std::min<uint64_t>((lds_cu) / (res2_lds + 256), 2048 / (64 * wpb)) : 0;
                const uint64_t in_flight = (uint64_t)n_cus * wgs2 * wpb;
                const bool auto_ok = sizeof(REAL) == 4 ? (uint64_t)nb_.n_packs * 100 <= in_flight * 145 : (uint64_t)nb_.n_packs <= in_flight;
                if (wgs2 && (mode == 2 || auto_ok)) {
                    Res2Records R2;
                    build_res2_records(L, sizeof(REAL), res2_ns, res2_nl, R2);
                    if (R2.ok && R2.rec.size() * sizeof(uint32_t) < (1ull << 31)) {
                        if ((rc = upload(&d_res2_rec, R2.rec))) return rc;
                        if ((rc = upload(&d_res2_rec_off, R2.rec_off))) return rc;
                        res2_n_words = (uint32_t)R2.rec.size();
                        use_res2 = use_res = true;
                    }
                }
            }
        }
        uint32_t narrow2_static = 0;
        if (nb_.n_packs && !use_res && !wb_.n_packs && !(opts && (opts->variant_flags & 0x1000u))) {
            StreamRecords SR;
            build_stream_records(L, sizeof(REAL), SR);
            narrow2_static = L.ex.waves_per_block * ((2 * pack_width + 2 + pack_width + 2) * (uint32_t)sizeof(REAL) + 3 * 64 * 4 + 64);
            const bool forced = opts && (opts->variant_flags & 0x2000u);
            const bool shared = forced || (SR.rec.size() * sizeof(uint32_t) <= (uint64_t)L.narrow_slots * sizeof(REAL) / 2 &&
                                           (sizeof(REAL) == 8 || n_slots <= 16'000'000ull));
            if (SR.ok && shared && stage_lds + narrow2_static + seg_bytes(L.ex.waves_per_block) <= 64 * 1024) {
                if ((rc = upload(&d_srec, SR.rec))) return rc;
                if ((rc = upload(&d_srec_off, SR.rec_off))) return rc;
                srec_words = (uint32_t)SR.rec.size();
                use_narrow2 = true;
                narrow_gen = narrow_seg;
                for (uint16_t r : L.narrow.hop_root) narrow_gen = narrow_gen || r != NO_ROOT;
            }
        }
        if (nb_.n_packs && !use_res && !wb_.n_packs && !hb_.n_packs && !narrow_seg && pack_width == 128 && (L.ex.waves_per_block == 4 || L.ex.waves_per_block == 8) &&
            !(opts && (opts->variant_flags & 0x41000u))) {
            LayerRecords LR;
            build_layer_records(L, sizeof(REAL), LR);
            const uint32_t n3_static = L.ex.waves_per_block * (4 * (128 + 128) * (uint32_t)sizeof(REAL) + 3 * 64 * 4);
            const bool forced = opts && (opts->variant_flags & 0x2000u);
            const bool shared = forced || (LR.rec.size() * sizeof(uint32_t) <= (uint64_t)L.narrow_slots * sizeof(REAL) / 2 && n_slots <= 16'000'000ull);
            if (LR.ok && shared && stage_lds + n3_static <= lds_cu - 1024) {
                if ((rc = upload(&d_lrec, LR.rec))) return rc;
                if ((rc = upload(&d_lrec_off, LR.rec_off))) return rc;
                lrec_words = (uint32_t)LR.rec.size();
                use_narrow3 = true;
                n3_nt = sizeof(REAL) == 8 && nt_potentials != 0;
            }
        }
        if (nb_.n_packs && !use_res && !use_narrow3 && !wb_.n_packs && !hb_.n_packs && !narrow_seg && !narrow_gen && pack_width == 128 &&
            (L.ex.waves_per_block == 4 || L.ex.waves_per_block == 8) && (beyond_cache || (opts && (opts->variant_flags & 0x100000u))))
#ifndef BDDMMA_EXP_NO_N12_NT
            n12_nt = !use_narrow2 || sizeof(REAL) == 8;
#else
            n12_nt = false;
#endif
        nt_loads = n3_nt || n12_nt;
        if (wb_.n_packs) {
            wide_threads = std::min<uint32_t>(1024, std::max<uint32_t>(64, ((wide_pack_width + 1) / 2 + 63) / 64 * 64));
            wide_npt = (wide_pack_width + wide_threads - 1) / wide_threads;
            wide_npt = wide_npt <= 1 ? 1 : (wide_npt <= 2 ? 2 : 4);
            wide_lds = (uint32_t)wide2_lds_bytes(sizeof(REAL), wide_pack_width, true);
            if (wide_lds > lds_cu || wide_pack_width > 4096) {
                err = "wide_pack_width " + std::to_string(wide_pack_width) + " needs " + std::to_string(wide_lds) + " B of LDS (> 160 KiB)";
                return BDDMMA_ERR_UNSUPPORTED;
            }
        }
        if (wb_.n_packs && nb_.n_packs && !use_res && !(opts && (opts->variant_flags & 1u))) {
            const uint32_t threads = 64 * wpb;
            const uint32_t npt = (wide_pack_width + threads - 1) / threads;
            const uint32_t narrow_dyn = stage_lds + seg_bytes(wpb);
            if (npt <= 4 && wide_lds <= narrow_dyn + 16 * 1024 && std::max(narrow_dyn, wide_lds) + narrow_static <= 64 * 1024) {
                mixed = true;
                mixed_npt = npt <= 1 ? 1 : (npt <= 2 ? 2 : 4);
                mixed_lds = std::max(narrow_dyn, wide_lds);
            }
        }
        if (use_res2 && res_hdr_ok && nb_.n_packs <= SMALL_MAX_PACKS && !wb_.n_packs && !hb_.n_packs && !deterministic && !entry_by_var && !big &&
            L.var_ptr.size() == n_vars + 1 && L.ex.vpos.size() == n_layers && !(opts && (opts->variant_flags & 0x80000u))) {
            const uint32_t np = nb_.n_packs;
            std::vector<uint32_t> lds_off(n_layers);
            uint32_t max_hops = 0;
            bool ok = true;
            for (uint32_t k = 0; k < (uint32_t)n_layers && ok; ++k) {
                const uint32_t l = L.var_layers[k];
                uint32_t p = 0;
                while (p < np && !(l >= L.res.pack_hdr[8 * (size_t)p + 2] && l < L.res.pack_hdr[8 * (size_t)p + 2] + L.res.pack_hdr[8 * (size_t)p + 3])) ++p;
                if (p == np || l - L.res.pack_hdr[8 * (size_t)p + 2] >= res2_nl) { ok = false; break; }
                lds_off[k] = (p * small_stage_stride(res2_nl) + (l - L.res.pack_hdr[8 * (size_t)p + 2])) * 2u * (uint32_t)sizeof(REAL);
            }
            for (uint32_t p = 0; p < np; ++p) max_hops = std::max(max_hops, L.res.pack_hdr[8 * (size_t)p + 5] & 0xFFFFu);
            small = SmallDev{};
            small.ns = res2_ns; small.nl = res2_nl; small.n_packs = np; small.wpb = wpb; small.n_quads = cdiv(np, wpb);
            small.n_vars = (uint32_t)n_vars; small.n_entries = (uint32_t)n_layers; small.rec_words = res2_n_words;
            small.rec_cap = (max_hops + 1u) * 1024u;
            uint32_t bytes = small_lds_bytes((uint32_t)sizeof(REAL), np, (uint32_t)n_vars, (uint32_t)n_layers, small);
            small_rl = bytes + 512 <= lds_cu;
            if (!small_rl) {
                small.rec_cap = 0;
                bytes = small_lds_bytes((uint32_t)sizeof(REAL), np, (uint32_t)n_vars, (uint32_t)n_layers, small);
            }
            if (ok && bytes + 512 <= lds_cu) {
                if ((rc = upload(&d_small_lds, lds_off))) return rc;
                small.pack_hdr = d_pack_hdr; small.quad_hdr = d_quad_hdr; small.rec = d_res2_rec; small.rec_off = d_res2_rec_off;
                small.var_ptr = d_var_ptr; small.var_lds = d_small_lds; small.var_ent = d_vpos;
                small_lds = bytes;
                small_nw = np <= 1 ? 1 : np <= 2 ? 2 : np <= 4 ? 4 : np <= 8 ? 8 : 16;
                small_ok = true;
                fused_small = true;
            }
        }
        resolve_kernels();
        if ((rc = raise_lds_limits(kern))) return rc;
        solve_sweep_kind = !nb_.n_packs ? BDDMMA_SWEEPS_NONE : mixed ? BDDMMA_SWEEPS_MIXED : (use_res && use_res2) ? BDDMMA_SWEEPS_RESIDENT2 : use_res ? BDDMMA_SWEEPS_RESIDENT1
                           : use_narrow3 ? BDDMMA_SWEEPS_STREAMING3 : use_narrow2 ? BDDMMA_SWEEPS_STREAMING2 : BDDMMA_SWEEPS_STREAMING1;
        HIPCHK(hipStreamSynchronize(stream));
        return BDDMMA_OK;
    }

    DevPtrs<REAL> ptrs(const REAL* delta_lay) const
    {
        DevPtrs<REAL> d;
        d.nwords = d_nwords; d.n_nwords = n_nwords; d.wwords = d_wwords; d.wide_slot_base = wide_slot_base;
        d.F = d_F; d.T = d_T; d.lohi = d_lohi;
        d.delta_lay = delta_lay; d.mm_binned = d_mm_binned; d.lpos = d_lpos; d.cs_entry = d_cs_entry; d.cs_slot = d_cs_slot;
        d.n_slots = (uint32_t)n_slots; d.n_layers = (uint32_t)n_layers; d.n_narrow_layers = n_narrow_layers;
        d.lb_partial = d_lb_partial;
        d.mm0_out = d_tmp0; d.mm1_out = d_tmp1; d.sol_out = d_sol;
        d.x_layer = d_x_layer;
        d.stop = run_stop;
        d.run_iter = run_iter;
        d.big = big ? 1u : 0u;
        return d;
    }
    PackDev pdev(const PackBufs& b, uint32_t lb_base, uint32_t seg_off = 0) const
    {
        const bool narrow_set = &b == &nb_;
        return PackDev{b.pack_hop_ptr, b.hop_node_off, b.hop_layer_off, b.pack_steps, b.hop_root, d_pack_word_off,
                       d_pack_group_ptr, d_grp_layer_off, d_grp_hop_end, d_quad_round_ptr, d_cs_ptr, stage_cap, seg_off, b.n_packs, lb_base,
                       nt_potentials, xcd_chunk(), narrow_set ? n2_hdr_pack() : nullptr, narrow_set ? n2_hdr_quad() : nullptr};
    }
    uint32_t seg_bytes(uint32_t w) const { return narrow_seg ? w * 128 * (uint32_t)sizeof(REAL) : 0; }
    uint32_t xcd_chunk_auto = 0;
    uint32_t xcd_chunk() const { return xcd_chunk_auto; }
    uint32_t narrow_grid(uint32_t n_quads) const
    {
        const uint32_t c = xcd_chunk();
        return c ? 8 * c * cdiv(n_quads, 8 * c) : 8 * cdiv(n_quads, 8);
    }

    template <typename FN>
    struct Kern { FN fn = nullptr; uint32_t lds = 0; };
    using NarrowFn = void (*)(DevPtrs<REAL>, PackDev, REAL);
    using RecFn = void (*)(DevPtrs<REAL>, PackDev, const uint32_t*, const uint32_t*, uint32_t, REAL);
    using ResFn = void (*)(const uint32_t*, const uint32_t*, uint32_t, uint32_t, uint32_t, uint32_t, const uint32_t*, uint32_t, DevPtrs<REAL>, PackDev, REAL);
    using Res2Fn = void (*)(const uint32_t*, const uint32_t*, uint32_t, uint32_t, uint32_t, uint32_t, const uint32_t*, uint32_t, const uint32_t*,
                            const uint32_t*, uint32_t, DevPtrs<REAL>, PackDev, REAL);
    using WideFn = void (*)(DevPtrs<REAL>, PackDev, REAL, uint32_t);
    using HugeFn = void (*)(DevPtrs<REAL>, PackDev, REAL, uint32_t, unsigned char*);
    using MixedFn = void (*)(DevPtrs<REAL>, PackDev, PackDev, REAL, uint32_t);
    using ExFn = void (*)(const REAL*, const uint32_t*, const uint16_t*, const uint32_t*, uint32_t, uint32_t, uint32_t, uint32_t, const int32_t*, REAL*, REAL*,
                          RunStep, const REAL*);
    using SegFn = void (*)(const REAL*, const uint4*, const uint32_t*, uint32_t, const uint4*, const uint2*, uint32_t, uint32_t, REAL*, RunStep, const REAL*);
    using ProjFn = void (*)(REAL*, const uint32_t*, const uint16_t*, const int32_t*, uint32_t, uint32_t, uint32_t);
    using SmallFn = void (*)(SmallDev, DevPtrs<REAL>, PackDev, REAL, uint32_t, RunStep);
    using TransFn = void (*)(const REAL*, REAL*, PackDev, const uint32_t*, const uint16_t*, uint32_t, uint32_t, REAL*, REAL);
    using LincombFn = void (*)(LinComb, REAL*, PackDev, const uint32_t*, const uint16_t*, uint32_t, uint32_t);
    struct Sweep {
        Res2Fn res2 = nullptr;
        ResFn res = nullptr;
        RecFn rec = nullptr;
        NarrowFn narrow = nullptr;
        uint32_t narrow_lds = 0, w = 1, seg_off = 0;
        const uint32_t *rec_tab = nullptr, *rec_off = nullptr;
        uint32_t rec_words = 0;
        Kern<WideFn> wide;
        Kern<MixedFn> mixed;
        HugeFn huge = nullptr;
        const void* narrow_fn() const { return res2 ? (const void*)res2 : res ? (const void*)res : rec ? (const void*)rec : (const void*)narrow; }
    };
    struct Kernels {
        Sweep sweep[2][3];
        uint32_t ex_threads = 0;
        Kern<ExFn> ex[2], ex_w, ex_raw;
        Kern<SegFn> seg[2], seg_w;
        Kern<ProjFn> project;
        Kern<SmallFn> small;
        Kern<TransFn> transpose[2];
        Kern<LincombFn> lincomb[2];
    } kern;
    Sweep ov_sweep[2];
    template <int MODE, bool OV>
    Sweep resolve_sweep(bool bwd) const
    {
        constexpr bool SOLVE = MODE == FWD_SOLVE;
        static_assert(!OV || SOLVE, "omega per layer: solve sweeps only");
        Sweep s;
        if (hb_.n_packs) s.huge = bwd ? &k_bwd_wide<REAL, MODE, true, OV> : &k_fwd_wide<REAL, MODE, true, OV>;
        if (wb_.n_packs)
            s.wide = {pick<1, 2, 4>(wide_npt, [&](auto N) -> WideFn { return bwd ? &k_bwd_wide2<REAL, MODE, N.value, OV> : &k_fwd_wide2<REAL, MODE, N.value, OV>; }),
                      wide_lds};
        if (!nb_.n_packs) return s;
        if constexpr (!SOLVE) {
            s.narrow = pick<64, 128, 256>(pack_width, [&](auto PW) -> NarrowFn {
                constexpr int R = PW.value / 64;
                return bwd ? &k_bwd_narrow<REAL, R, MODE, 1, true, false, false> : &k_fwd_narrow<REAL, R, MODE, 1, true, false, false>;
            });
            s.narrow_lds = seg_bytes(1);
        } else {
            s.w = wpb;
            s.seg_off = use_res ? res_lds : stage_lds;
            s.narrow_lds = (use_res && use_res2) ? res2_lds : s.seg_off + seg_bytes(wpb);
            pick<64, 128, 256>(pack_width, [&](auto PW) {
                pick<1, 2, 4, 8>(wpb, [&](auto W_) {
                    constexpr int R = PW.value / 64, W = W_.value, W48 = W == 8 ? 8 : 4;
                    const bool w48 = W == 4 || W == 8;
                    if (use_res && use_res2) s.res2 = bwd ? &k_bwd_res2<REAL, W, OV> : &k_fwd_res2<REAL, W, OV>;
                    else if (use_res) s.res = bwd ? &k_bwd_res<REAL, R, W, OV> : &k_fwd_res<REAL, R, W, OV>;
                    else if (use_narrow3 && w48) {
                        s.rec = bwd ? &k_bwd_narrow3<REAL, W48, false, OV> : &k_fwd_narrow3<REAL, W48, false, OV>;
                        if constexpr (sizeof(REAL) == 8)
                            if (n3_nt) s.rec = bwd ? &k_bwd_narrow3<REAL, W48, true, OV> : &k_fwd_narrow3<REAL, W48, true, OV>;
                        s.rec_tab = d_lrec; s.rec_off = d_lrec_off; s.rec_words = lrec_words;
                    } else if (use_narrow2) {
                        if (n12_nt && R == 2 && w48) s.rec = bwd ? &k_bwd_narrow2<REAL, 2, W48, false, sizeof(REAL) == 8, OV> : &k_fwd_narrow2<REAL, 2, W48, false, sizeof(REAL) == 8, OV>;
                        else if (narrow_gen) s.rec = bwd ? &k_bwd_narrow2<REAL, R, W, true, false, OV> : &k_fwd_narrow2<REAL, R, W, true, false, OV>;
                        else s.rec = bwd ? &k_bwd_narrow2<REAL, R, W, false, false, OV> : &k_fwd_narrow2<REAL, R, W, false, false, OV>;
                        s.rec_tab = d_srec; s.rec_off = d_srec_off; s.rec_words = srec_words;
                    } else if (n12_nt && R == 2 && w48) s.narrow = bwd ? &k_bwd_narrow<REAL, 2, MODE, W48, false, true, OV> : &k_fwd_narrow<REAL, 2, MODE, W48, false, true, OV>;
                    else if (!narrow_seg) s.narrow = bwd ? &k_bwd_narrow<REAL, R, MODE, W, false, false, OV> : &k_fwd_narrow<REAL, R, MODE, W, false, false, OV>;
                    else s.narrow = bwd ? &k_bwd_narrow<REAL, R, MODE, W, true, false, OV> : &k_fwd_narrow<REAL, R, MODE, W, true, false, OV>;
                });
            });
            if (mixed)
                s.mixed = {pick<64, 128, 256>(pack_width, [&](auto PW) {
                               return pick<1, 2, 4, 8>(wpb, [&](auto W) {
                                   return pick<1, 2, 4>(mixed_npt, [&](auto N) -> MixedFn {
                                       constexpr int R = PW.value / 64;
                                       return bwd ? &k_bwd_mixed<REAL, R, W.value, N.value, OV> : &k_fwd_mixed<REAL, R, W.value, N.value, OV>;
                                   });
                               });
                           }),
                           mixed_lds};
        }
        return s;
    }
    void resolve_kernels()
    {
        for (int bwd = 0; bwd < 2; ++bwd) {
            kern.sweep[bwd][FWD_PLAIN] = resolve_sweep<FWD_PLAIN, false>(bwd);
            kern.sweep[bwd][FWD_SOLVE] = resolve_sweep<FWD_SOLVE, false>(bwd);
            kern.sweep[bwd][FWD_SOLUTION] = resolve_sweep<FWD_SOLUTION, false>(bwd);
        }
        kern.ex_threads = exch_small ? EXS_THREADS : exch_medium ? EXM_THREADS : EX_THREADS;
        pick<EXS_THREADS, EXM_THREADS, EX_THREADS>(kern.ex_threads, [&](auto T_) {
            constexpr int T = T_.value, U = T == EXS_THREADS ? EXS_UNROLL : T == EXM_THREADS ? EXM_UNROLL : EX_UNROLL,
                          N = T == EXS_THREADS ? EXS_NPT : T == EXM_THREADS ? EXM_NPT : EX_NPT;
            kern.ex[0] = {&k_exchange_reduce<REAL, BDDMMA_EX_ACC, EX_ITER, T, U, N, false>, exch_lds};
            kern.ex[1] = {&k_exchange_reduce<REAL, BDDMMA_EX_ACC, EX_ITER, T, U, N, true>, exch_lds};
            kern.ex_w = {&k_exchange_reduce<REAL, BDDMMA_EX_ACC, EX_ITER, T, U, N, false, true>, exch_lds};
            kern.project = {&k_project_entries<REAL, T>, vars_per_bin * (uint32_t)sizeof(double)};
            if (use_seg)
                pick<2, 4>(seg_groups <= 2 ? 2 : 4, [&](auto G) {
                    kern.seg[0] = {&k_exchange_seg<REAL, T, G.value, false>, seg_lds};
                    kern.seg[1] = {&k_exchange_seg<REAL, T, G.value, true>, seg_lds};
                    kern.seg_w = {&k_exchange_seg<REAL, T, G.value, false, true>, seg_lds};
                });
        });
        kern.ex_raw = {&k_exchange_reduce<REAL, BDDMMA_EX_ACC, EX_RAW>, exch_lds};
        if (small_ok)
            kern.small = {pick<1, 2, 4, 8, 16>(small_nw, [&](auto NW) -> SmallFn {
                              return small_rl ? &k_iterate_small<REAL, NW.value, true> : &k_iterate_small<REAL, NW.value, false>;
                          }),
                          small_lds};
        if (n_narrow_layers)
            pick<1, 2, 4, 8>(wpb, [&](auto W) {
                const uint32_t lds = wpb * stage_cap * (uint32_t)sizeof(REAL);
                kern.transpose[0] = {&k_stage_transpose<REAL, W.value, 0>, lds};
                kern.transpose[1] = {&k_stage_transpose<REAL, W.value, 1>, lds};
                kern.lincomb[0] = {&k_stage_lincomb<REAL, W.value, 0>, lds};
                kern.lincomb[1] = {&k_stage_lincomb<REAL, W.value, 5>, lds};
            });
    }
    int raise_lds_limit(const void* fn, uint32_t lds)
    {
        if (fn && lds) HIPCHK(hipFuncSetAttribute(fn, hipFuncAttributeMaxDynamicSharedMemorySize, (int)lds));
        return BDDMMA_OK;
    }
    template <typename FN>
    int raise_lds_limit(const Kern<FN>& k) { return raise_lds_limit(reinterpret_cast<const void*>(k.fn), k.lds); }
    int raise_lds_limits(const Sweep& s)
    {
        if (int rc = raise_lds_limit(s.narrow_fn(), s.narrow_lds)) return rc;
        return raise_lds_limit(s.wide);
    }
    int raise_lds_limits(const Kernels& k)
    {
        int rc = BDDMMA_OK;
        for (const auto& dir : k.sweep)
            for (const Sweep& s : dir)
                if ((rc = raise_lds_limits(s))) return rc;
        for (const auto* e : {&k.ex[0], &k.ex[1], &k.ex_w, &k.ex_raw})
            if ((rc = raise_lds_limit(*e))) return rc;
        for (const auto* e : {&k.seg[0], &k.seg[1], &k.seg_w})
            if ((rc = raise_lds_limit(*e))) return rc;
        for (const auto* e : {&k.transpose[0], &k.transpose[1]})
            if ((rc = raise_lds_limit(*e))) return rc;
        for (const auto* e : {&k.lincomb[0], &k.lincomb[1]})
            if ((rc = raise_lds_limit(*e))) return rc;
        if ((rc = raise_lds_limit(k.project))) return rc;
        return raise_lds_limit(k.small);
    }

    int ov_prepare();
    bool ov_ready = false;
    int launch_sweep(bool bwd, const Sweep& s, const REAL* delta_lay, REAL omega, int kclass, bool ov = false)
    {
        if (bwd) {
            lb_cached = false;
            ++lb_gen;
        }
        DevPtrs<REAL> d = ptrs(delta_lay);
        if (ov) d.omega_lay = d_omega_lay;
        prof_begin(kclass);
        if (s.mixed.fn && (bwd || mixed_fwd)) {
            const PackDev pkw = pdev(wb_, nb_.n_packs), pkn = pdev(nb_, 0, stage_lds);
            const uint32_t nw8 = (wb_.n_packs + 7u) & ~7u;
            const dim3 grid(nw8 + narrow_grid(cdiv(nb_.n_packs, wpb))), block(64 * wpb);
            hipLaunchKernelGGL(s.mixed.fn, grid, block, s.mixed.lds, stream, d, pkn, pkw, omega, wide_pack_width);
        } else {
            if (s.wide.fn) hipLaunchKernelGGL(s.wide.fn, dim3(wb_.n_packs), dim3(wide_threads), s.wide.lds, stream, d, pdev(wb_, nb_.n_packs), omega, wide_pack_width);
            if (nb_.n_packs) {
                const PackDev pk = pdev(nb_, 0, s.seg_off);
                const dim3 grid(narrow_grid(cdiv(nb_.n_packs, s.w))), block(64 * s.w);
                if (s.res2)
                    hipLaunchKernelGGL(s.res2, grid, block, s.narrow_lds, stream, d_pack_hdr, d_quad_hdr, res2_ns, res2_nl, pk.n_packs, pk.xcd_chunk, d.stop, d.run_iter,
                                       d_res2_rec, d_res2_rec_off, res2_n_words, d, pk, omega);
                else if (s.res)
                    hipLaunchKernelGGL(s.res, grid, block, s.narrow_lds, stream, d_pack_hdr, d_quad_hdr, res_ns, res_nl, pk.n_packs, pk.xcd_chunk, d.stop, d.run_iter, d, pk, omega);
                else if (s.rec) hipLaunchKernelGGL(s.rec, grid, block, s.narrow_lds, stream, d, pk, s.rec_tab, s.rec_off, s.rec_words, omega);
                else hipLaunchKernelGGL(s.narrow, grid, block, s.narrow_lds, stream, d, pk, omega);
            }
        }
        if (s.huge) hipLaunchKernelGGL(s.huge, dim3(hb_.n_packs), dim3(WIDE_THREADS), 0, stream, d, pdev(hb_, nb_.n_packs + wb_.n_packs), omega, huge_pack_width, d_huge_scratch);
        prof_end(kclass);
        HIPCHK(hipGetLastError());
        return BDDMMA_OK;
    }
    int launch_fwd(int mode, const REAL* delta_lay, REAL omega, int kclass) { return launch_sweep(false, kern.sweep[0][mode], delta_lay, omega, kclass); }
    int launch_bwd(int mode, const REAL* delta_lay, REAL omega, int kclass) { return launch_sweep(true, kern.sweep[1][mode], delta_lay, omega, kclass); }
    void launch_bcast(const REAL* delta_var, REAL* delta_lay, RunGate g = RunGate{}, RunStep run = RunStep{})
    {
        hipLaunchKernelGGL((k_exchange_bcast<REAL>), dim3(cdiv(cdiv(n_layers, 4), 256)), dim3(256), 0, stream, delta_var, d_evar, delta_lay,
                           (uint32_t)n_layers, (uint32_t)n_vars, g, run);
    }
    void launch_reduce_raw(REAL* delta_var)
    {
        if (deterministic)
            hipLaunchKernelGGL((k_delta_gather<REAL, false>), dim3(cdiv(n_vars, 256)), dim3(256), 0, stream, d_mm_binned, d_var_ptr,
                               d_vpos, delta_var, (uint32_t)n_vars, RunGate{});
        else
            hipLaunchKernelGGL(kern.ex_raw.fn, dim3(n_bins), dim3(EX_THREADS), kern.ex_raw.lds, stream, d_mm_binned, d_bin_ptr, d_bvar,
                               (const uint32_t*)nullptr, 0u, vars_per_bin, (uint32_t)n_vars, (uint32_t)n_layers, d_nbdds, delta_var, (REAL*)nullptr, RunStep{},
                               (const REAL*)nullptr);
    }
    int exchange(bool ends_iteration = false)
    {
        const RunStep rstep = (ends_iteration && run_stop) ? run_step : RunStep{};
        prof_begin(BDDMMA_K_FINISH_DELTA);
        if (entry_by_var) {
            hipLaunchKernelGGL((k_exchange_byvar<REAL>), dim3(cdiv(n_vars, 256)), dim3(256), 0, stream, d_mm_binned, d_var_ptr, d_delta_lay,
                               (uint32_t)n_vars, (uint32_t)n_layers, gate(), rstep);
            delta_var_valid = false;
        } else if (deterministic && !use_seg) {
            hipLaunchKernelGGL((k_delta_gather<REAL, true>), dim3(cdiv(n_vars, 256)), dim3(256), 0, stream, d_mm_binned, d_var_ptr,
                               d_vpos, d_delta_var, (uint32_t)n_vars, gate());
            launch_bcast(d_delta_var, d_delta_lay, gate(), rstep);
            delta_var_valid = true;
        } else {
            const bool run = run_stop != nullptr;
            const dim3 grid(n_bins + (run && rstep.ctl != nullptr ? 1u : 0u)), block(kern.ex_threads);
            if (use_seg)
                hipLaunchKernelGGL(kern.seg[run].fn, grid, block, kern.seg[run].lds, stream, d_mm_binned, reinterpret_cast<const uint4*>(d_seg_bin), gate().stop,
                                   gate().iter, reinterpret_cast<const uint4*>(d_seg_perm), reinterpret_cast<const uint2*>(d_seg_thr), seg_tile_off, seg_cnt_off,
                                   d_delta_lay, rstep, (const REAL*)nullptr);
            else
                hipLaunchKernelGGL(kern.ex[run].fn, grid, block, kern.ex[run].lds, stream, d_mm_binned, d_bin_ptr, d_bvar, gate().stop, gate().iter, vars_per_bin,
                                   (uint32_t)n_vars, (uint32_t)n_layers, d_nbdds, (REAL*)nullptr, d_delta_lay, rstep, (const REAL*)nullptr);
            delta_var_valid = false;
        }
        prof_end(BDDMMA_K_FINISH_DELTA);
        HIPCHK(hipGetLastError());
        return BDDMMA_OK;
    }

    int forward_run() override
    {
        if (fwd_valid) return BDDMMA_OK;
        HIPCHK(hipSetDevice(device));
        int rc = launch_fwd(FWD_PLAIN, nullptr, REAL(0), BDDMMA_K_OTHER);
        if (rc) return rc;
        fwd_valid = true;
        return BDDMMA_OK;
    }
    int backward_run() override
    {
        if (bwd_valid) return BDDMMA_OK;
        HIPCHK(hipSetDevice(device));
        int rc = launch_bwd(BWD_PLAIN, nullptr, REAL(0), BDDMMA_K_OTHER);
        if (rc) return rc;
        bwd_valid = true;
        return BDDMMA_OK;
    }
    int lower_bound(double* lb) override
    {
        int rc = backward_run();
        if (rc) return rc;
        if (lb_cached) {
            *lb = lb_cache;
            return BDDMMA_OK;
        }
        if ((rc = launch_bound(0))) return rc;
        if ((rc = wait_bound(0))) return rc;
        *lb = lb_cache = ((volatile double*)h_lb)[0];
        lb_cached = true;
        return BDDMMA_OK;
    }
    int launch_bound(int k)
    {
        lb_seq_expect[k] = ++lb_seq_next;
        hipLaunchKernelGGL(k_lb_reduce, dim3(1), dim3(1024), 0, stream, d_lb_partial, nb_.n_packs + wb_.n_packs + hb_.n_packs, d_lb + k, d_lb_seq + k, lb_seq_expect[k]);
        HIPCHK(hipGetLastError());
        return BDDMMA_OK;
    }
    int wait_bound(int k)
    {
        volatile uint64_t* w = h_lb_seq + k;
        const auto t0 = std::chrono::steady_clock::now();
        uint32_t spins = 0;
        while (*w != lb_seq_expect[k]) {
            cpu_relax();
            if ((++spins & 1023u) == 0 && std::chrono::duration<double>(std::chrono::steady_clock::now() - t0).count() > 2e-3) {
                HIPCHK(hipStreamSynchronize(stream));
                if (*w != lb_seq_expect[k]) { err = "lower bound: the reduce kernel did not report"; return BDDMMA_ERR_DEVICE; }
                break;
            }
        }
        std::atomic_thread_fence(std::memory_order_acquire);
        return BDDMMA_OK;
    }
    int lower_bound_enqueue(int slot) override
    {
        if (slot < 0 || slot > 1) { err = "lower_bound_enqueue: slot must be 0 or 1"; return BDDMMA_ERR_INVALID_ARGUMENT; }
        int rc = backward_run();
        if (rc) return rc;
        lb_slot_gen[slot] = lb_gen;
        if (lb_cached) {
            lb_slot_known[slot] = true;
            lb_slot_value[slot] = lb_cache;
            return BDDMMA_OK;
        }
        if ((rc = launch_bound(1 + slot))) return rc;
        lb_slot_known[slot] = false;
        lb_slot_enqueued[slot] = true;
        return BDDMMA_OK;
    }
    int lower_bound_fetch(int slot, double* lb) override
    {
        if (slot < 0 || slot > 1) { err = "lower_bound_fetch: slot must be 0 or 1"; return BDDMMA_ERR_INVALID_ARGUMENT; }
        if (!lb_slot_known[slot]) {
            if (!lb_slot_enqueued[slot]) { err = "lower_bound_fetch without lower_bound_enqueue"; return BDDMMA_ERR_STATE; }
            int rc = wait_bound(1 + slot);
            if (rc) return rc;
            lb_slot_value[slot] = ((volatile double*)h_lb)[1 + slot];
            lb_slot_known[slot] = true;
        }
        *lb = lb_slot_value[slot];
        if (lb_slot_gen[slot] == lb_gen && bwd_valid) {
            lb_cache = *lb;
            lb_cached = true;
        }
        return BDDMMA_OK;
    }
    int lower_bound_per_bdd(void* out, int on_device) override
    {
        int rc = backward_run();
        if (rc) return rc;
        REAL* tmp = nullptr;
        REAL* dst = (REAL*)out;
        if (!on_device) { HIPCHK(hipMalloc((void**)&tmp, n_bdds * sizeof(REAL))); dst = tmp; }
        hipLaunchKernelGGL((k_lb_per_bdd<REAL>), dim3(cdiv(n_bdds, 256)), dim3(256), 0, stream, d_T, d_root_slot, dst, (uint32_t)n_bdds);
        if (!on_device) {
            hipError_t e = hipMemcpyAsync(out, tmp, n_bdds * sizeof(REAL), hipMemcpyDeviceToHost, stream);
            if (e == hipSuccess) e = hipStreamSynchronize(stream);
            (void)hipFree(tmp);
            HIPCHK(e);
        }
        return BDDMMA_OK;
    }

    int mma_forward(REAL omega, const REAL* delta_lay, bool ov = false)
    {
        int rc;
        if (!bwd_valid && (rc = backward_run())) return rc;
        rc = launch_sweep(false, ov ? ov_sweep[0] : kern.sweep[0][FWD_SOLVE], delta_lay, omega, BDDMMA_K_FORWARD_MM, ov);
        x_layer_valid = false;
        if (rc) return rc;
        fwd_valid = true;
        bwd_valid = false;
        return BDDMMA_OK;
    }
    int mma_backward(REAL omega, const REAL* delta_lay, bool ov = false)
    {
        if (!fwd_valid) {
            err = "backward_mm requires a valid forward state (call forward_mm first)";
            return BDDMMA_ERR_STATE;
        }
        int rc = launch_sweep(true, ov ? ov_sweep[1] : kern.sweep[1][BWD_SOLVE], delta_lay, omega, BDDMMA_K_BACKWARD_MM, ov);
        if (rc) return rc;
        x_layer_valid = d_x_layer != nullptr;
        fwd_valid = false;
        bwd_valid = true;
        return BDDMMA_OK;
    }
    bool small_usable() const { return small_ok && !profiling && d_x_layer == nullptr; }
    void small_launched()
    {
        lb_cached = false;
        ++lb_gen;
        x_layer_valid = false;
        fwd_valid = false;
        bwd_valid = true;
        delta_var_valid = false;
    }
    int launch_small(REAL omega, uint32_t n, const RunStep& rstep)
    {
        int rc;
        if (!bwd_valid && (rc = backward_run())) return rc;
        const DevPtrs<REAL> d = ptrs(d_delta_lay);
        const PackDev pk = pdev(nb_, 0, 0);
        hipLaunchKernelGGL(kern.small.fn, dim3(1), dim3(64 * small_nw), kern.small.lds, stream, small, d, pk, omega, n, rstep);
        HIPCHK(hipGetLastError());
        small_launched();
        return BDDMMA_OK;
    }
    SmallItem<REAL> small_item() const { return SmallItem<REAL>{small, ptrs(d_delta_lay), pdev(nb_, 0, 0), RunStep{d_lb_partial, nb_.n_packs + wb_.n_packs + hb_.n_packs, nullptr, nullptr}}; }
    int iterations(double omega, uint64_t n) override
    {
        HIPCHK(hipSetDevice(device));
        if (!small_usable() || run_stop) {
            for (uint64_t i = 0; i < n; ++i)
                if (int rc = iteration(omega)) return rc;
            return BDDMMA_OK;
        }
        while (n) {
            const uint32_t chunk = (uint32_t)std::min<uint64_t>(n, 1u << 14);
            if (int rc = launch_small((REAL)omega, chunk, RunStep{})) return rc;
            n -= chunk;
        }
        return BDDMMA_OK;
    }
    int iteration(double omega) override
    {
        HIPCHK(hipSetDevice(device));
        int rc;
        if (small_usable() && !run_stop) return launch_small((REAL)omega, 1, RunStep{});
        prof_active = profiling && (prof_iter++ % prof_stride == 0);
        if ((rc = mma_forward((REAL)omega, d_delta_lay))) return rc;
        if ((rc = exchange())) return rc;
        if ((rc = mma_backward((REAL)omega, d_delta_lay))) return rc;
        if ((rc = exchange(true))) return rc;
        return BDDMMA_OK;
    }
    void weighted_exchange()
    {
        const REAL* al = d_alpha_ent;
        prof_begin(BDDMMA_K_FINISH_DELTA);
        if (entry_by_var) {
            hipLaunchKernelGGL((k_exchange_byvar<REAL, true>), dim3(cdiv(n_vars, 256)), dim3(256), 0, stream, d_mm_binned, d_var_ptr, d_delta_lay,
                               (uint32_t)n_vars, (uint32_t)n_layers, RunGate{}, RunStep{}, al);
        } else if (deterministic && !use_seg) {
            hipLaunchKernelGGL((k_delta_gather<REAL, false>), dim3(cdiv(n_vars, 256)), dim3(256), 0, stream, d_mm_binned, d_var_ptr,
                               d_vpos, d_delta_c, (uint32_t)n_vars, RunGate{});
            hipLaunchKernelGGL((k_exchange_bcast<REAL, true>), dim3(cdiv(cdiv(n_layers, 4), 256)), dim3(256), 0, stream, (const REAL*)d_delta_c, d_evar,
                               d_delta_lay, (uint32_t)n_layers, (uint32_t)n_vars, RunGate{}, RunStep{}, al);
        } else if (use_seg) {
            hipLaunchKernelGGL(kern.seg_w.fn, dim3(n_bins), dim3(kern.ex_threads), kern.seg_w.lds, stream, d_mm_binned, reinterpret_cast<const uint4*>(d_seg_bin),
                               (const uint32_t*)nullptr, 0u, reinterpret_cast<const uint4*>(d_seg_perm), reinterpret_cast<const uint2*>(d_seg_thr), seg_tile_off,
                               seg_cnt_off, d_delta_lay, RunStep{}, al);
        } else {
            hipLaunchKernelGGL(kern.ex_w.fn, dim3(n_bins), dim3(kern.ex_threads), kern.ex_w.lds, stream, d_mm_binned, d_bin_ptr, d_bvar, (const uint32_t*)nullptr,
                               0u, vars_per_bin, (uint32_t)n_vars, (uint32_t)n_layers, d_nbdds, (REAL*)nullptr, d_delta_lay, RunStep{}, al);
        }
        delta_var_valid = false;
        prof_end(BDDMMA_K_FINISH_DELTA);
    }
    int isotropic_dist_weights(void* out, int on_device) override
    {
        HIPCHK(hipSetDevice(device));
        REAL* dst = on_device ? (REAL*)out : d_tmp0;
        hipLaunchKernelGGL((k_isotropic_alpha<REAL>), dim3(cdiv(n_layers, 256)), dim3(256), 0, stream, d_var, d_nbdds, dst, (uint32_t)n_layers);
        HIPCHK(hipGetLastError());
        if (!on_device) return copy_out(out, dst, n_layers * sizeof(REAL), 0);
        HIPCHK(hipStreamSynchronize(stream));
        return BDDMMA_OK;
    }
    int load_layer_values(REAL* dst, const void* src, int on_dev, const char* what)
    {
        if (!on_dev) {
            const REAL* h = (const REAL*)src;
            for (uint64_t l = 0; l < n_layers; ++l)
                if (!(h[l] >= REAL(0) && h[l] < std::numeric_limits<REAL>::infinity())) {
                    err = std::string("learned_iterations: ") + what + "[" + std::to_string(l) + "] is negative or not finite";
                    return BDDMMA_ERR_INVALID_ARGUMENT;
                }
        }
        HIPCHK(hipMemcpyAsync(dst, src, n_layers * sizeof(REAL), on_dev ? hipMemcpyDeviceToDevice : hipMemcpyHostToDevice, stream));
        if (on_dev) {
            HIPCHK(hipMemsetAsync(d_counts, 0, sizeof(uint32_t), stream));
            hipLaunchKernelGGL((k_count_bad_weights<REAL>), dim3(cdiv(n_layers, 256)), dim3(256), 0, stream, (const REAL*)dst, d_counts, (uint32_t)n_layers);
            uint32_t bad = 0;
            HIPCHK(hipMemcpyAsync(&bad, d_counts, sizeof(uint32_t), hipMemcpyDeviceToHost, stream));
            HIPCHK(hipStreamSynchronize(stream));
            if (bad) {
                err = "learned_iterations: " + std::to_string(bad) + " of the " + what + " are negative or not finite";
                return BDDMMA_ERR_INVALID_ARGUMENT;
            }
        }
        return BDDMMA_OK;
    }
    int learned_iterations(const void* w, int w_dev, uint64_t num_itr, double omega, double slope, void* sol_avg, void* lb1_avg, void* lb2_avg,
                           uint64_t cfi, double beta_d, int out_dev, uint64_t* itr_done, const void* omega_vec, int ov_dev) override
    {
        HIPCHK(hipSetDevice(device));
        int rc;
        if (itr_done) *itr_done = 0;
        if (!w) { err = "learned_iterations: dist_weights is null"; return BDDMMA_ERR_INVALID_ARGUMENT; }
        if (cfi > 0 && (!sol_avg || !lb1_avg || !lb2_avg)) {
            err = "learned_iterations: compute_history_for_itr > 0 needs sol_avg, lb_first_diff_avg and lb_second_diff_avg";
            return BDDMMA_ERR_INVALID_ARGUMENT;
        }
        if (*lbfgs_attached > 0) {
            err = "learned_iterations: an L-BFGS wrapper is attached to this solver (destroy it first: its history would not describe the costs any more)";
            return BDDMMA_ERR_STATE;
        }
        if (run_stop) { err = "learned_iterations: run_solver is queueing iterations"; return BDDMMA_ERR_STATE; }
        if (!d_alpha_ent && (rc = dalloc(&d_alpha_ent, n_layers))) return rc;
        const bool ov = omega_vec != nullptr;
        if (ov) {
            if (!ov_ready) {
                if ((rc = ov_prepare())) return rc;
                ov_ready = true;
            }
            if (!d_omega_lay && (rc = dalloc(&d_omega_lay, n_layers))) return rc;
            if ((rc = load_layer_values(d_omega_lay, omega_vec, ov_dev, "omega_vec"))) return rc;
        }
        if ((rc = load_layer_values(d_tmp0, w, w_dev, "dist_weights"))) return rc;
        hipLaunchKernelGGL((k_layers_to_entries<REAL>), dim3(cdiv(n_layers, 256)), dim3(256), 0, stream, (const REAL*)d_tmp0, d_lpos, d_alpha_ent, (uint32_t)n_layers);
        HIPCHK(hipGetLastError());
        const uint64_t B = n_bdds, L = n_layers;
        REAL *o_sol = (REAL*)sol_avg, *o_lb1 = (REAL*)lb1_avg, *o_lb2 = (REAL*)lb2_avg;
        REAL *last_sol = nullptr, *lb_last = nullptr, *lb_second = nullptr, *lb_third = nullptr, *chg = nullptr, *prev_chg = nullptr;
        if (cfi > 0) {
            if (!d_hist && (rc = dalloc(&d_hist, L + 5 * B))) return rc;
            last_sol = d_hist; lb_last = d_hist + L; lb_second = lb_last + B; lb_third = lb_second + B; chg = lb_third + B; prev_chg = chg + B;
            if (!out_dev) {
                if (!d_hist_out && (rc = dalloc(&d_hist_out, L + 2 * B))) return rc;
                o_sol = d_hist_out; o_lb1 = d_hist_out + L; o_lb2 = o_lb1 + B;
                HIPCHK(hipMemcpyAsync(o_sol, sol_avg, L * sizeof(REAL), hipMemcpyHostToDevice, stream));
                HIPCHK(hipMemcpyAsync(o_lb1, lb1_avg, B * sizeof(REAL), hipMemcpyHostToDevice, stream));
                HIPCHK(hipMemcpyAsync(o_lb2, lb2_avg, B * sizeof(REAL), hipMemcpyHostToDevice, stream));
            }
        }
        const REAL omega_r = (REAL)omega, beta = (REAL)beta_d;
        const dim3 gl(cdiv(L, 256)), gb(cdiv(B, 256)), blk(256);
        const bool track_lb = slope > 0;
        const bool want_initial = !std::isfinite(initial_lb_change);
        double lb_initial = 0.0, lb_prev = 0.0, lb_post = 0.0;
        if (num_itr > 0) {
            if (track_lb) {
                if ((rc = lower_bound(&lb_initial))) return rc;
            } else if (want_initial && (rc = lower_bound_enqueue(0))) return rc;
        }
        lb_post = lb_initial;
        bool converged = false;
        uint64_t tracked = 0, itr = 0, ran = 0;
        for (itr = 0; itr < num_itr; ++itr) {
            prof_active = profiling && (prof_iter++ % prof_stride == 0);
            weighted_exchange();
            if ((rc = mma_forward(omega_r, d_delta_lay, ov))) return rc;
            weighted_exchange();
            if ((rc = mma_backward(omega_r, d_delta_lay, ov))) return rc;
            ++ran;
            if (cfi > 0 && (cfi >= num_itr - itr || converged)) {
                HIPCHK(hipMemsetAsync(d_sol, 0, n_layers, stream));
                if ((rc = launch_fwd(FWD_SOLUTION, nullptr, REAL(0), BDDMMA_K_OTHER))) return rc;
                hipLaunchKernelGGL((k_char_to_real<REAL>), gl, blk, 0, stream, (const char*)d_sol, last_sol, (uint32_t)L);
                hipLaunchKernelGGL((k_lb_per_bdd<REAL>), gb, blk, 0, stream, d_T, d_root_slot, lb_last, (uint32_t)B);
                if (tracked == 0) {
                    HIPCHK(hipMemcpyAsync(o_sol, last_sol, L * sizeof(REAL), hipMemcpyDeviceToDevice, stream));
                } else {
                    hipLaunchKernelGGL((k_ema<REAL>), gl, blk, 0, stream, o_sol, (const REAL*)last_sol, beta, (uint32_t)L);
                    hipLaunchKernelGGL((k_diff<REAL, REAL>), gb, blk, 0, stream, chg, (const REAL*)lb_last, (const REAL*)lb_second, (uint32_t)B);
                    if (tracked == 1) {
                        HIPCHK(hipMemcpyAsync(o_lb1, chg, B * sizeof(REAL), hipMemcpyDeviceToDevice, stream));
                    } else {
                        hipLaunchKernelGGL((k_ema<REAL>), gb, blk, 0, stream, o_lb1, (const REAL*)chg, beta, (uint32_t)B);
                        hipLaunchKernelGGL((k_diff<REAL, REAL>), gb, blk, 0, stream, prev_chg, (const REAL*)lb_second, (const REAL*)lb_third, (uint32_t)B);
                        hipLaunchKernelGGL((k_diff<REAL, REAL>), gb, blk, 0, stream, chg, (const REAL*)chg, (const REAL*)prev_chg, (uint32_t)B);
                        if (tracked == 2) HIPCHK(hipMemcpyAsync(o_lb2, chg, B * sizeof(REAL), hipMemcpyDeviceToDevice, stream));
                        else hipLaunchKernelGGL((k_ema<REAL>), gb, blk, 0, stream, o_lb2, (const REAL*)chg, beta, (uint32_t)B);
                    }
                }
                HIPCHK(hipGetLastError());
                REAL* t = lb_third;
                lb_third = lb_second;
                lb_second = lb_last;
                lb_last = t;
                ++tracked;
            }
            if (track_lb) {
                lb_prev = lb_post;
                if ((rc = lower_bound(&lb_post))) return rc;
// ... 735 lines not shown
```

### bdd_amd/csrc/solver_sm.hpp

```cpp
#pragma once
#include "solver_impl.hpp"
#include "kernels/summarg.hpp"

namespace bddmma {

struct SmPackSet {
    std::vector<uint32_t> pack_hop_ptr, hop_node_off;
};
template <typename WORD, typename DECODE, typename WORDOF>
static bool sm_build_parents(const std::vector<SmPackSet>& sets, const std::vector<WORD>& words, DECODE decode, WORDOF word_of, std::vector<uint32_t>& ptr,
                             std::vector<uint32_t>& par)
{
    const size_t nw = words.size();
    ptr.assign(nw + 1, 0);
    std::vector<uint8_t> seen(nw, 0);
    for (int pass = 0; pass < 2; ++pass) {
        std::vector<uint32_t> fill;
        if (pass == 1) {
            for (size_t i = 0; i < nw; ++i) ptr[i + 1] += ptr[i];
            par.assign(ptr[nw], 0);
            fill.assign(ptr.begin(), ptr.end() - 1);
            std::fill(seen.begin(), seen.end(), 0);
        }
        for (const SmPackSet& ps : sets)
        for (size_t p = 0; p + 1 < ps.pack_hop_ptr.size(); ++p) {
            const std::vector<uint32_t>& hop_node_off = ps.hop_node_off;
            const uint32_t q0 = ps.pack_hop_ptr[p], q1 = ps.pack_hop_ptr[p + 1];
            if (q0 == q1) continue;
            const size_t w0 = word_of(ps, p);
            if (w0 + (hop_node_off[q1] - hop_node_off[q0]) > nw) return false;
            if (seen[w0]) continue;
            seen[w0] = 1;
            for (uint32_t q = q0; q + 1 < q1; ++q) {
                const size_t wq = w0 + (hop_node_off[q] - hop_node_off[q0]), wn = w0 + (hop_node_off[q + 1] - hop_node_off[q0]);
                const uint32_t n = hop_node_off[q + 1] - hop_node_off[q], n_next = hop_node_off[q + 2] - hop_node_off[q + 1];
                for (uint32_t j = 0; j < n; ++j) {
                    uint32_t ch[2];
                    if (!decode(words[wq + j], ch)) continue;
                    for (uint32_t arc = 0; arc < 2; ++arc) {
                        if (ch[arc] >= n_next) continue;
                        if (pass == 0) ++ptr[wn + ch[arc] + 1];
                        else par[fill[wn + ch[arc]]++] = (j << 1) | arc;
                    }
                }
            }
        }
    }
    return true;
}

template <typename REAL>
int SolverT<REAL>::sm_prepare()
{
    if (sm_ready) return BDDMMA_OK;
    HIPCHK(hipSetDevice(device));
    auto fetch = [&](int id, auto& vec) -> hipError_t {
        using T = typename std::remove_reference_t<decltype(vec)>::value_type;
        const DevField& f = dev_fields[id];
        vec.resize(f.count);
        return f.count ? hipMemcpyAsync(vec.data(), f.ptr, f.count * sizeof(T), hipMemcpyDeviceToHost, stream) : hipSuccess;
    };
    int rc;
    if (nb_.n_packs) {
        std::vector<uint32_t> words, word_off;
        std::vector<SmPackSet> sets(1);
        HIPCHK(fetch(LAY_NARROW_WORDS, words)); HIPCHK(fetch(LAY_NARROW_WORD_OFF, word_off));
        HIPCHK(fetch(LAY_NARROW_PACK_HOP_PTR, sets[0].pack_hop_ptr)); HIPCHK(fetch(LAY_NARROW_HOP_NODE_OFF, sets[0].hop_node_off));
        HIPCHK(hipStreamSynchronize(stream));
        std::vector<uint32_t> ptr, par;
        const uint32_t W = pack_width;
        const bool ok = sm_build_parents(sets, words,
                         [W](uint32_t w, uint32_t (&ch)[2]) {
                             if (w & NW_PAD) return false;
                             ch[0] = w & NW_CHILD_MASK;
                             ch[1] = (w >> NW_CHILD_BITS) & NW_CHILD_MASK;
                             if (ch[0] >= W) ch[0] = 0xFFFFFFFFu;
                             if (ch[1] >= W) ch[1] = 0xFFFFFFFFu;
                             return true;
                         },
                         [&](const SmPackSet&, size_t p) { return (size_t)word_off[p]; }, ptr, par);
        if (!ok) { err = "sum-marginals: a narrow pack's node words lie outside the word array"; return BDDMMA_ERR_STATE; }
        if ((rc = upload(&d_sm_nptr, ptr))) return rc;
        if ((rc = upload(&d_sm_npar, par))) return rc;
        HIPCHK(hipStreamSynchronize(stream));
    }
    if (wb_.n_packs || hb_.n_packs) {
        std::vector<uint64_t> words;
        HIPCHK(fetch(LAY_WIDE_WORDS, words));
        std::vector<SmPackSet> sets(2);
        HIPCHK(fetch(LAY_WIDE_PACK_HOP_PTR, sets[0].pack_hop_ptr)); HIPCHK(fetch(LAY_WIDE_HOP_NODE_OFF, sets[0].hop_node_off));
        HIPCHK(fetch(LAY_HUGE_PACK_HOP_PTR, sets[1].pack_hop_ptr)); HIPCHK(fetch(LAY_HUGE_HOP_NODE_OFF, sets[1].hop_node_off));
        HIPCHK(hipStreamSynchronize(stream));
        std::vector<uint32_t> ptr, par;
        const uint32_t wsb = wide_slot_base;
        const bool ok = sm_build_parents(sets, words,
                         [](uint64_t w, uint32_t (&ch)[2]) {
                             const uint64_t lo = w & WW_CHILD_MASK, hi = (w >> WW_CHILD_BITS) & WW_CHILD_MASK;
                             ch[0] = lo < WW_TOP ? (uint32_t)lo : 0xFFFFFFFFu;
                             ch[1] = hi < WW_TOP ? (uint32_t)hi : 0xFFFFFFFFu;
                             return true;
                         },
                         [&](const SmPackSet& ps, size_t p) { return (size_t)(ps.hop_node_off[ps.pack_hop_ptr[p]] - wsb); }, ptr, par);
        if (!ok) { err = "sum-marginals: a wide pack's node words lie outside the word array"; return BDDMMA_ERR_STATE; }
        if ((rc = upload(&d_sm_wptr, ptr))) return rc;
        if ((rc = upload(&d_sm_wpar, par))) return rc;
        HIPCHK(hipStreamSynchronize(stream));
    }
    if (hb_.n_packs && (rc = dalloc(&d_sm_scratch, (uint64_t)hb_.n_packs * sm_lds_bytes(sizeof(REAL), huge_pack_width)))) return rc;
    if ((rc = pull_wide_lds("sum-marginals", sm_fwd_sweep(), sm_bwd_sweep()))) return rc;
    sm_ready = true;
    return BDDMMA_OK;
}

template <typename REAL>
PullSweep<REAL> SolverT<REAL>::sm_fwd_sweep() const
{
    return {&k_sm_fwd<REAL, true, false>, &k_sm_fwd<REAL, false, false>, &k_sm_fwd<REAL, false, true>, &sm_lds_bytes, d_sm_scratch};
}
template <typename REAL>
PullSweep<REAL> SolverT<REAL>::sm_bwd_sweep() const
{
    return {&k_sm_bwd<REAL, true, false>, &k_sm_bwd<REAL, false, false>, &k_sm_bwd<REAL, false, true>, &sm_lds_bytes, d_sm_scratch};
}

template <typename REAL>
int SolverT<REAL>::sm_launch_fwd()
{
    if (int rc = launch_pull(sm_fwd_sweep())) return rc;
    fwd_valid = false;
    return BDDMMA_OK;
}

template <typename REAL>
int SolverT<REAL>::sm_launch_bwd()
{
    bwd_valid = false;
    lb_cached = false;
    ++lb_gen;
    return launch_pull(sm_bwd_sweep());
}

template <typename REAL>
int SolverT<REAL>::sm_sum_marginals(int sorted, int log_probs, int32_t* var, void* sm0, void* sm1, int on_device)
{
    HIPCHK(hipSetDevice(device));
    int rc;
    if ((rc = sm_prepare())) return rc;
    if ((rc = sm_launch_fwd())) return rc;
    if ((rc = sm_launch_bwd())) return rc;
    if (!log_probs) hipLaunchKernelGGL((k_exp_pair<REAL>), dim3(cdiv(n_layers, 256)), dim3(256), 0, stream, d_tmp0, d_tmp1, (uint32_t)n_layers);
    return marginals_out(sorted, var, sm0, sm1, on_device);
}

template <typename REAL>
int SolverT<REAL>::sm_smooth_solution(void* out, int on_device)
{
    HIPCHK(hipSetDevice(device));
    int rc;
    if ((rc = sm_prepare())) return rc;
    if ((rc = sm_launch_fwd())) return rc;
    if ((rc = sm_launch_bwd())) return rc;
    REAL* dst = on_device ? (REAL*)out : d_tmp0;
    hipLaunchKernelGGL((k_smooth_solution<REAL>), dim3(cdiv(n_layers, 256)), dim3(256), 0, stream, (const REAL*)d_tmp0, (const REAL*)d_tmp1, dst, (uint32_t)n_layers);
    if (!on_device) return copy_out(out, dst, n_layers * sizeof(REAL), 0);
    HIPCHK(hipStreamSynchronize(stream));
    return BDDMMA_OK;
}

}
```

### bdd_amd/solver.py

```python
from __future__ import annotations

import ctypes as C

import numpy as np

from . import capi
from .bdd_collection import BddCollection


def _ptr(a):
    return a.ctypes.data_as(C.c_void_p) if a is not None else None


def _is_dev(x):
    return hasattr(x, "data_ptr") and bool(getattr(x, "is_cuda", False))


def _dev_ptr(x, n, dtype):
    assert x.is_contiguous() and x.numel() >= n, "device buffer too small or not contiguous"
    assert x.element_size() == np.dtype(dtype).itemsize, "device buffer has the wrong element type"
    return C.c_void_p(x.data_ptr())


class bdd_hip_parallel_mma:

    def __init__(self, bdd_col: BddCollection, costs_hi=None, precision: str = "double", device: int = 0,
                 pack_width: int = 0, wide_pack_width: int = 0, deterministic: bool = False,
                 vars_per_bin: int = 0, stage_cap: int = 0, waves_per_block: int = 0, keep_bdd_order: bool = False,
                 resident_sweeps: int = 0, exchange_by_variable: int = 0, variant_flags: int = 0, pack_fill: int = 0, pack_stagger: int = 0, _handle=None):
        self._L = capi.lib()
        self.value_type = {"double": np.float64, "float": np.float32, "single": np.float32}[precision]
        self._prec = capi.F64 if self.value_type == np.float64 else capi.F32
        if _handle is not None:
            self._h = _handle
            return
        instr = np.ascontiguousarray(bdd_col.instr, dtype=np.uint64)
        delims = np.ascontiguousarray(bdd_col.delims, dtype=np.uint64)
        opts = capi.Options(pack_width, wide_pack_width, 1 if deterministic else 0, vars_per_bin, stage_cap, waves_per_block)
        opts.keep_bdd_order = int(keep_bdd_order)
        opts.resident_sweeps = int(resident_sweeps)
        opts.exchange_by_variable = int(exchange_by_variable)
        opts.pack_fill = int(pack_fill)
        opts.pack_stagger = int(pack_stagger)
        opts.variant_flags = int(variant_flags)
        h = C.c_void_p()
        costs = None if costs_hi is None else np.ascontiguousarray(costs_hi, dtype=np.float64)
        rc = self._L.bddmma_create(C.byref(h), self._prec, device, _ptr(instr), _ptr(delims), bdd_col.nr_bdds(),
                                   _ptr(costs), 0 if costs is None else costs.size, C.byref(opts))
        capi.check(rc, None)
        self._h = h

    def close(self):
        if getattr(self, "_h", None):
            self._L.bddmma_destroy(self._h)
            self._h = None

    def __del__(self):
        try:
            self.close()
        except Exception:
            pass

    def _ck(self, rc):
        capi.check(rc, self._h)

    def nr_variables(self): return int(self._L.bddmma_nr_variables(self._h))
    def nr_layers(self): return int(self._L.bddmma_nr_layers(self._h))
    def nr_bdd_nodes(self): return int(self._L.bddmma_nr_bdd_nodes(self._h))
    def nr_hops(self): return int(self._L.bddmma_nr_hops(self._h))
    def nr_packs(self): return int(self._L.bddmma_nr_packs(self._h))

    SWEEP_KINDS = ("none", "mixed", "streaming1", "streaming2", "streaming3", "resident1", "resident2")

    def solve_sweep_kind(self) -> str:
        return self.SWEEP_KINDS[int(self._L.bddmma_solve_sweep_kind(self._h))]
    def fused_small(self) -> bool:
        return bool(self._L.bddmma_fused_small(self._h))
    def nontemporal_loads(self) -> bool:
        return bool(self._L.bddmma_nontemporal_loads(self._h))
    def device_bytes(self): return int(self._L.bddmma_device_bytes(self._h))
    def device_allocated_bytes(self): return int(self._L.bddmma_device_allocated_bytes(self._h))

    def nr_bdds(self, var=None):
        if var is None:
            return int(self._L.bddmma_nr_bdds(self._h))
        return int(self.get_num_bdds_per_var()[var])

    def get_num_bdds_per_var(self):
        out = np.zeros(self.nr_variables(), np.int32)
        self._ck(self._L.bddmma_num_bdds_per_var(self._h, _ptr(out)))
        return out

    def get_primal_variable_index(self):
        out = np.zeros(self.nr_layers(), np.int32)
        self._ck(self._L.bddmma_layer_variables(self._h, _ptr(out)))
        return out

    def get_bdd_index(self):
        out = np.zeros(self.nr_layers(), np.int32)
        self._ck(self._L.bddmma_layer_bdds(self._h, _ptr(out)))
        return out

    def nodes_per_hop(self):
        out = np.zeros(self.nr_hops(), np.uint64)
        self._ck(self._L.bddmma_nodes_per_hop(self._h, _ptr(out)))
        return out

    def layers_per_hop(self):
        out = np.zeros(self.nr_hops(), np.uint64)
        self._ck(self._L.bddmma_layers_per_hop(self._h, _ptr(out)))
        return out

    def bdd_major_order(self):
        return np.argsort(self.get_bdd_index(), kind="stable")

    def update_costs(self, cost_delta_0, cost_delta_1):
        if _is_dev(cost_delta_0) or _is_dev(cost_delta_1):
            n0 = cost_delta_0.numel() if cost_delta_0 is not None else 0
            n1 = cost_delta_1.numel() if cost_delta_1 is not None else 0
            self._ck(self._L.bddmma_update_costs(self._h, _dev_ptr(cost_delta_0, n0, self.value_type) if n0 else None, n0,
                                                 _dev_ptr(cost_delta_1, n1, self.value_type) if n1 else None, n1, self._prec, 1))
            return
        lo = np.ascontiguousarray(cost_delta_0, dtype=np.float64)
        hi = np.ascontiguousarray(cost_delta_1, dtype=np.float64)
        self._ck(self._L.bddmma_update_costs(self._h, _ptr(lo), lo.size, _ptr(hi), hi.size, capi.F64, 0))

    def set_cost(self, c, var):
        self._ck(self._L.bddmma_set_cost(self._h, float(c), int(var)))

    def get_solver_costs(self, out=None):
        n = self.nr_layers()
        if out is not None:
            self._ck(self._L.bddmma_get_solver_costs(self._h, *(_dev_ptr(x, n, self.value_type) for x in out), 1))
            return out
        lo, hi, mm = (np.zeros(n, self.value_type) for _ in range(3))
        self._ck(self._L.bddmma_get_solver_costs(self._h, _ptr(lo), _ptr(hi), _ptr(mm), 0))
        return lo, hi, mm

    def set_solver_costs(self, lo, hi, mm):
        if _is_dev(lo):
            n = self.nr_layers()
            self._ck(self._L.bddmma_set_solver_costs(self._h, *(_dev_ptr(x, n, self.value_type) for x in (lo, hi, mm)), 1))
            return
        lo, hi, mm = (np.ascontiguousarray(x, dtype=self.value_type) for x in (lo, hi, mm))
        self._ck(self._L.bddmma_set_solver_costs(self._h, _ptr(lo), _ptr(hi), _ptr(mm), 0))

    def get_primal_objective_vector(self, out):
        self._ck(self._L.bddmma_primal_objective_vec(self._h, _dev_ptr(out, self.nr_variables(), self.value_type), 1))
        return out

    def get_primal_objective_vector_host(self):
        out = np.zeros(self.nr_variables(), self.value_type)
        self._ck(self._L.bddmma_primal_objective_vec(self._h, _ptr(out), 0))
        return out

    def forward_run(self): self._ck(self._L.bddmma_forward_run(self._h))
    def backward_run(self): self._ck(self._L.bddmma_backward_run(self._h))

    def lower_bound(self) -> float:
        lb = C.c_double()
        self._ck(self._L.bddmma_lower_bound(self._h, C.byref(lb)))
        return lb.value

    def lower_bound_per_bdd(self, out=None):
        if out is not None:
            self._ck(self._L.bddmma_lower_bound_per_bdd(self._h, _dev_ptr(out, self.nr_bdds(), self.value_type), 1))
            return out
        out = np.zeros(self.nr_bdds(), self.value_type)
        self._ck(self._L.bddmma_lower_bound_per_bdd(self._h, _ptr(out), 0))
        return out

    def iteration(self, omega=0.5):
        self._ck(self._L.bddmma_iteration(self._h, float(omega)))

    def iterations(self, n, omega=0.5):
        self._ck(self._L.bddmma_iterations(self._h, float(omega), int(n)))

    def forward_mm(self, omega, delta_lo_hi):
        if _is_dev(delta_lo_hi):
            self._ck(self._L.bddmma_forward_mm(self._h, float(omega), _dev_ptr(delta_lo_hi, 2 * self.nr_variables(), self.value_type), 1))
            return
        assert delta_lo_hi.dtype == self.value_type and delta_lo_hi.size == 2 * self.nr_variables()
        self._ck(self._L.bddmma_forward_mm(self._h, float(omega), _ptr(delta_lo_hi), 0))

    def backward_mm(self, omega, delta_lo_hi):
        if _is_dev(delta_lo_hi):
            self._ck(self._L.bddmma_backward_mm(self._h, float(omega), _dev_ptr(delta_lo_hi, 2 * self.nr_variables(), self.value_type), 1))
            return
        assert delta_lo_hi.dtype == self.value_type and delta_lo_hi.size == 2 * self.nr_variables()
        self._ck(self._L.bddmma_backward_mm(self._h, float(omega), _ptr(delta_lo_hi), 0))

    def normalize_delta(self, delta_lo_hi):
        if _is_dev(delta_lo_hi):
            self._ck(self._L.bddmma_normalize_delta(self._h, _dev_ptr(delta_lo_hi, 2 * self.nr_variables(), self.value_type), 1))
            return
        self._ck(self._L.bddmma_normalize_delta(self._h, _ptr(delta_lo_hi), 0))

    def distribute_delta(self):
        self._ck(self._L.bddmma_distribute_delta(self._h))

    def _learned_buf(self, x, n, what):
        if _is_dev(x):
            if x.numel() != n:
                raise capi.BddMmaError(f"bdd_mma error {capi.ERR_INVALID_ARGUMENT}: {what} has {x.numel()} values, the solver needs {n}")
            if not x.is_contiguous():
                raise capi.BddMmaError(f"bdd_mma error {capi.ERR_INVALID_ARGUMENT}: {what} must be contiguous")
            if x.element_size() != np.dtype(self.value_type).itemsize or not x.is_floating_point():
                raise capi.BddMmaError(f"bdd_mma error {capi.ERR_INVALID_ARGUMENT}: {what} is {x.dtype}, the solver's values are "
                                       f"{np.dtype(self.value_type).name}")
            return _dev_ptr(x, n, self.value_type), 1
        if not isinstance(x, np.ndarray):
            raise capi.BddMmaError(f"bdd_mma error {capi.ERR_INVALID_ARGUMENT}: {what} must be a numpy array or a device tensor")
        if x.dtype != self.value_type:
            raise capi.BddMmaError(f"bdd_mma error {capi.ERR_INVALID_ARGUMENT}: {what} is {x.dtype}, the solver's values are "
                                   f"{np.dtype(self.value_type).name}")
        if x.size != n:
            raise capi.BddMmaError(f"bdd_mma error {capi.ERR_INVALID_ARGUMENT}: {what} has {x.size} values, the solver needs {n}")
        if not x.flags.c_contiguous:
            raise capi.BddMmaError(f"bdd_mma error {capi.ERR_INVALID_ARGUMENT}: {what} must be contiguous")
        return _ptr(x), 0

    def learned_iterations(self, dist_weights, num_itr, omega=0.5, improvement_slope=1e-6, sol_avg=None, lb_first_diff_avg=None,
                           lb_second_diff_avg=None, compute_history_for_itr=0, history_avg_beta=0.9, omega_vec=None) -> int:
        w, w_dev = self._learned_buf(dist_weights, self.nr_layers(), "dist_weights")
        if omega_vec is not None:
            ov, ov_dev = self._learned_buf(omega_vec, self.nr_layers(), "omega_vec")
        outs = [None, None, None]
        out_dev = 0
        if int(compute_history_for_itr) > 0:
            bufs = (sol_avg, lb_first_diff_avg, lb_second_diff_avg)
            if any(b is None for b in bufs):
                raise capi.BddMmaError(f"bdd_mma error {capi.ERR_INVALID_ARGUMENT}: compute_history_for_itr > 0 needs sol_avg, "
# ... 333 lines not shown
```

### include/bdd_mma.h

```cpp
#ifndef BDD_MMA_H
#define BDD_MMA_H

#include <stddef.h>
#include <stdint.h>

#ifdef __cplusplus
extern "C" {
#endif

#define BDDMMA_OK 0
#define BDDMMA_ERR_INVALID_ARGUMENT (-1)
#define BDDMMA_ERR_INVALID_BDD (-2)
#define BDDMMA_ERR_DEVICE (-3)
#define BDDMMA_ERR_STATE (-4)
#define BDDMMA_ERR_UNSUPPORTED (-5)
#define BDDMMA_ERR_IO (-6)

#define BDDMMA_F32 0
#define BDDMMA_F64 1

typedef struct bddmma_instruction {
    uint64_t lo;
    uint64_t hi;
    uint64_t index;
} bddmma_instruction;

#define BDDMMA_TOPSINK UINT64_MAX
#define BDDMMA_BOTSINK (UINT64_MAX - 1)

typedef struct bddmma_solver bddmma_solver;

typedef struct bddmma_options {
    uint32_t pack_width;
    uint32_t wide_pack_width;
    uint32_t deterministic;
    uint32_t vars_per_bin;
    uint32_t stage_cap;
    uint32_t waves_per_block;
    uint32_t keep_bdd_order;
    uint32_t resident_sweeps;
    uint32_t exchange_by_variable;
    uint32_t variant_flags;
    uint32_t pack_fill;
    uint32_t pack_stagger;
} bddmma_options;


int bddmma_create(bddmma_solver** out, int precision, int device,
                  const bddmma_instruction* instr, const uint64_t* bdd_delims, uint64_t n_bdds,
                  const double* costs_hi, uint64_t n_costs, const bddmma_options* opts);
void bddmma_destroy(bddmma_solver* s);

int bddmma_device_count(void);
int bddmma_device_chip(int device, uint32_t* n_cus, uint32_t* lds_bytes_per_cu, uint64_t* max_resident_threads);
int bddmma_set_layout_threads(int n);
int bddmma_set_thread_layout_threads(int n);
const char* bddmma_last_error(const bddmma_solver* s);

uint64_t bddmma_nr_variables(const bddmma_solver* s);
uint64_t bddmma_nr_bdds(const bddmma_solver* s);
uint64_t bddmma_nr_layers(const bddmma_solver* s);
uint64_t bddmma_nr_bdd_nodes(const bddmma_solver* s);
uint64_t bddmma_nr_hops(const bddmma_solver* s);
uint64_t bddmma_nr_packs(const bddmma_solver* s);
enum {
    BDDMMA_SWEEPS_NONE = 0,
    BDDMMA_SWEEPS_MIXED = 1,
    BDDMMA_SWEEPS_STREAMING1 = 2,
    BDDMMA_SWEEPS_STREAMING2 = 3,
    BDDMMA_SWEEPS_STREAMING3 = 4,
    BDDMMA_SWEEPS_RESIDENT1 = 5,
    BDDMMA_SWEEPS_RESIDENT2 = 6
};
int bddmma_solve_sweep_kind(const bddmma_solver* s);
int bddmma_fused_small(const bddmma_solver* s);
int bddmma_nontemporal_loads(const bddmma_solver* s);
int bddmma_precision(const bddmma_solver* s);
int bddmma_device(const bddmma_solver* s);
int bddmma_num_bdds_per_var(const bddmma_solver* s, int32_t* out);
int bddmma_layer_variables(const bddmma_solver* s, int32_t* out);
int bddmma_layer_bdds(const bddmma_solver* s, int32_t* out);
int bddmma_nodes_per_hop(const bddmma_solver* s, uint64_t* out);
int bddmma_layers_per_hop(const bddmma_solver* s, uint64_t* out);

int bddmma_update_costs(bddmma_solver* s, const void* lo, uint64_t n_lo, const void* hi, uint64_t n_hi,
                        int elem_precision, int on_device);
int bddmma_set_cost(bddmma_solver* s, double c, uint64_t var);
int bddmma_get_solver_costs(const bddmma_solver* s, void* lo, void* hi, void* deferred_mm_diff, int on_device);
int bddmma_set_solver_costs(bddmma_solver* s, const void* lo, const void* hi, const void* deferred_mm_diff, int on_device);
int bddmma_primal_objective_vec(bddmma_solver* s, void* out, int on_device);

int bddmma_forward_run(bddmma_solver* s);
int bddmma_backward_run(bddmma_solver* s);
int bddmma_lower_bound(bddmma_solver* s, double* lb);
int bddmma_lower_bound_per_bdd(bddmma_solver* s, void* out, int on_device);

int bddmma_iteration(bddmma_solver* s, double omega);
int bddmma_iterations(bddmma_solver* s, double omega, uint64_t n);
int bddmma_forward_mm(bddmma_solver* s, double omega, void* delta_lo_hi, int on_device);
int bddmma_backward_mm(bddmma_solver* s, double omega, void* delta_lo_hi, int on_device);
int bddmma_normalize_delta(const bddmma_solver* s, void* delta_lo_hi, int on_device);
int bddmma_distribute_delta(bddmma_solver* s);
int bddmma_get_delta(const bddmma_solver* s, void* out, int on_device);
int bddmma_set_delta(bddmma_solver* s, const void* in, int on_device);

int bddmma_learned_iterations(bddmma_solver* s, const void* dist_weights, int weights_on_device, uint64_t num_itr, double omega,
                              double improvement_slope, void* sol_avg, void* lb_first_diff_avg, void* lb_second_diff_avg,
                              uint64_t compute_history_for_itr, double history_avg_beta, int outputs_on_device, uint64_t* itr_done);
int bddmma_learned_iterations_omega_vec(bddmma_solver* s, const void* dist_weights, int weights_on_device, uint64_t num_itr, const void* omega_vec,
                                        int omega_vec_on_device, double improvement_slope, void* sol_avg, void* lb_first_diff_avg,
                                        void* lb_second_diff_avg, uint64_t compute_history_for_itr, double history_avg_beta, int outputs_on_device,
                                        uint64_t* itr_done);
int bddmma_isotropic_dist_weights(bddmma_solver* s, void* out, int on_device);

int bddmma_min_marginals(bddmma_solver* s, int sorted, int32_t* var, void* mm0, void* mm1, int on_device);
int bddmma_min_marginal_diff(bddmma_solver* s, void* out, int on_device);
int bddmma_sum_marginals(bddmma_solver* s, int sorted, int log_probs, int32_t* var, void* sm0, void* sm1, int on_device);
int bddmma_smooth_solution(bddmma_solver* s, void* out, int on_device);
int bddmma_bdds_solution(bddmma_solver* s, int sorted, char* sol, int on_device);

int bddmma_grad_min_marginal_diff(bddmma_solver* s, const void* grad_mm, void* grad_lo_out, void* grad_hi_out, int on_device);
int bddmma_grad_lower_bound_per_bdd(bddmma_solver* s, const void* grad_lb_per_bdd, void* grad_lo_out, void* grad_hi_out, int smooth, int on_device);
int bddmma_grad_distribute_delta(bddmma_solver* s, const void* grad_lo, const void* grad_hi, void* grad_deferred_mm_out, int on_device);
int bddmma_grad_cost_perturbation(bddmma_solver* s, const void* grad_lo, const void* grad_hi, void* grad_lo_pert_out, void* grad_hi_pert_out, int on_device);

int bddmma_grad_learned_iterations(bddmma_solver* s, const void* dist_weights, int weights_on_device, double omega, const void* omega_vec,
                                   int omega_vec_on_device, void* grad_lo, void* grad_hi, void* grad_mm, void* grad_dist_weights_out, void* grad_omega_out,
                                   uint64_t track_grad_after_itr, uint64_t track_grad_for_num_itr, uint64_t num_caches, int on_device);

int bddmma_net_solver_costs(const bddmma_solver* s, void* out, int on_device);
int bddmma_make_dual_feasible(const bddmma_solver* s, void* g, int on_device);
int bddmma_gradient_step(bddmma_solver* s, const void* g, double step_size, int on_device);

typedef struct bddmma_lbfgs bddmma_lbfgs;
typedef struct bddmma_lbfgs_params {
    int32_t history_size;
    double init_step_size;
    double req_rel_lb_increase;
    double step_size_decrease_factor;
    double step_size_increase_factor;
} bddmma_lbfgs_params;
int bddmma_lbfgs_create(bddmma_lbfgs** out, bddmma_solver* s, const bddmma_lbfgs_params* p);
void bddmma_lbfgs_destroy(bddmma_lbfgs* l);
int bddmma_lbfgs_iteration(bddmma_lbfgs* l);
int bddmma_lbfgs_update_costs(bddmma_lbfgs* l, const void* lo, uint64_t n_lo, const void* hi, uint64_t n_hi,
                              int elem_precision, int on_device);
int bddmma_lbfgs_flush(bddmma_lbfgs* l);
typedef struct bddmma_lbfgs_state {
    double step_size;
    double last_applied_step;
    uint64_t mma_iterations;
    uint64_t lbfgs_iterations;
    int32_t history_entries;
    int32_t num_unsuccessful_updates;
    int32_t last_kind;
    int32_t last_trials;
} bddmma_lbfgs_state;
int bddmma_lbfgs_get_state(const bddmma_lbfgs* l, bddmma_lbfgs_state* out);

typedef struct bddmma_run_result {
    uint64_t iterations;
    double lb_initial;
    double lb_final;
    double seconds;
    int32_t stop_reason;
} bddmma_run_result;
int bddmma_run_solver(bddmma_solver* s, bddmma_lbfgs* lbfgs_or_null, uint64_t max_iter, double tolerance,
                      double improvement_slope, double time_limit, int verbose, bddmma_run_result* res);
int bddmma_run_solver_host_loop(bddmma_solver* s, bddmma_lbfgs* lbfgs_or_null, uint64_t max_iter, double tolerance,
                                double improvement_slope, double time_limit, int verbose, bddmma_run_result* res);

typedef struct bddmma_batch bddmma_batch;
int bddmma_batch_create(bddmma_batch** out, bddmma_solver* const* members, uint64_t n);
void bddmma_batch_destroy(bddmma_batch* b);
const char* bddmma_batch_last_error(const bddmma_batch* b);
uint64_t bddmma_batch_size(const bddmma_batch* b);
int bddmma_batch_iterations(bddmma_batch* b, double omega, uint64_t n);
int bddmma_batch_run_solver(bddmma_batch* b, uint64_t max_iter, double tolerance, double improvement_slope, double time_limit,
                            bddmma_run_result* res);
int bddmma_batch_time_iterations(bddmma_batch* b, double omega, uint64_t n, double* ms);
int bddmma_batch_lower_bounds(bddmma_batch* b, double* out);

int bddmma_incremental_mm_agreement_rounding(bddmma_solver* s, bddmma_lbfgs* lbfgs_or_null, double init_delta,
                                             double delta_growth_rate, uint64_t num_itr_lb, uint64_t num_rounds,
                                             uint32_t seed, int verbose, char* sol, int* found);

int bddmma_perturb_primal_costs(bddmma_solver* s, bddmma_lbfgs* lbfgs_or_null, double cur_delta, uint32_t round_index, uint32_t seed,
                                uint32_t counts[4], char* sol, void* cost_delta_0, void* cost_delta_1);

int bddmma_save(const bddmma_solver* s, const char* path);
int bddmma_load(bddmma_solver** out, int device, const char* path);

int bddmma_synchronize(bddmma_solver* s);
#define BDDMMA_K_FORWARD_MM 0
#define BDDMMA_K_BACKWARD_MM 1
#define BDDMMA_K_FINISH_DELTA 2
#define BDDMMA_K_OTHER 3
#define BDDMMA_K_COUNT 4
typedef struct bddmma_profile {
    uint64_t launches[BDDMMA_K_COUNT];
    double total_ms[BDDMMA_K_COUNT];
} bddmma_profile;
int bddmma_set_profiling(bddmma_solver* s, int on);
int bddmma_get_profile(bddmma_solver* s, bddmma_profile* out);
int bddmma_time_iterations(bddmma_solver* s, double omega, uint64_t n, double* ms);
#define BDDMMA_TRIAD_BYTES (1ull << 30)
int bddmma_time_kernel(bddmma_solver* s, int kind, uint64_t reps, double* ms);
uint64_t bddmma_device_bytes(const bddmma_solver* s);
uint64_t bddmma_device_allocated_bytes(const bddmma_solver* s);

typedef struct bddmma_layout bddmma_layout;
int bddmma_layout_create(bddmma_layout** out, const bddmma_instruction* instr, const uint64_t* bdd_delims,
                         uint64_t n_bdds, const bddmma_options* opts);
int bddmma_layout_create_for_chip(bddmma_layout** out, const bddmma_instruction* instr, const uint64_t* bdd_delims,
                                  uint64_t n_bdds, const bddmma_options* opts, int real_size, uint32_t n_cus, uint32_t lds_bytes_per_cu);
void bddmma_layout_destroy(bddmma_layout* l);
uint64_t bddmma_layout_size(const bddmma_layout* l, int what);
int bddmma_layout_copy(const bddmma_layout* l, int which, void* out);
int bddmma_layout_res2_records(const bddmma_layout* l, int real_size, uint32_t* info, uint32_t* words, uint32_t* rec_off);
int bddmma_layout_stream_records(const bddmma_layout* l, int real_size, uint32_t* info, uint32_t* words, uint32_t* rec_off);
int bddmma_layout_layer_records(const bddmma_layout* l, int real_size, uint32_t* info, uint32_t* words, uint32_t* rec_off);
int bddmma_layout_seg_exchange(const bddmma_layout* l, int threads, int real_size, uint32_t* info, uint32_t* bin, uint16_t* perm, uint32_t* thr);

#ifdef __cplusplus
}
#endif
#endif
```

Before: 8764.

## Recompute opposite-direction potentials in LDS instead of streaming them from HBM

Adds a recompute mode for the narrow3 forward and backward MMA sweeps. Each wave first rebuilds the opposite-direction potentials (backward T for the forward sweep, forward F for the backward sweep) in per-wave dynamic LDS with a pre-pass over the pack's hops. The sweeps then no longer load or store those potential arrays in global memory. This removes most of the potential traffic from a bandwidth-bound sweep, at the cost of extra LDS per block (lower occupancy), a serial pre-pass with a wave sync per hop, and new state tracking so the lower bound stays valid when potentials are never written back.

```diff
diff --git a/bdd_amd/capi.py b/bdd_amd/capi.py
--- a/bdd_amd/capi.py
+++ b/bdd_amd/capi.py
@@ -58,6 +58,7 @@
     "bddmma_solve_sweep_kind": (_I, [_V]),
     "bddmma_fused_small": (_I, [_V]),
     "bddmma_nontemporal_loads": (_I, [_V]),
+    "bddmma_recomputes_potentials": (_I, [_V]),
     "bddmma_precision": (_I, [_V]),
     "bddmma_device": (_I, [_V]),
     "bddmma_num_bdds_per_var": (_I, [_V, _V]),
diff --git a/bdd_amd/csrc/capi.cpp b/bdd_amd/csrc/capi.cpp
--- a/bdd_amd/csrc/capi.cpp
+++ b/bdd_amd/csrc/capi.cpp
@@ -154,6 +154,7 @@
 int bddmma_solve_sweep_kind(const bddmma_solver* s) { return s && s->impl ? s->impl->solve_sweep_kind : -1; }
 int bddmma_fused_small(const bddmma_solver* s) { return s && s->impl ? (s->impl->fused_small ? 1 : 0) : -1; }
 int bddmma_nontemporal_loads(const bddmma_solver* s) { return s && s->impl ? (s->impl->nt_loads ? 1 : 0) : -1; }
+int bddmma_recomputes_potentials(const bddmma_solver* s) { return s && s->impl ? (s->impl->recomputes ? 1 : 0) : -1; }
 int bddmma_precision(const bddmma_solver* s) { return s && s->impl ? s->impl->precision : -1; }
 int bddmma_device(const bddmma_solver* s) { return s && s->impl ? s->impl->device : -1; }
 uint64_t bddmma_device_bytes(const bddmma_solver* s) { return s && s->impl ? s->impl->dev_bytes : 0; }
diff --git a/bdd_amd/csrc/kernels/common.hpp b/bdd_amd/csrc/kernels/common.hpp
--- a/bdd_amd/csrc/kernels/common.hpp
+++ b/bdd_amd/csrc/kernels/common.hpp
@@ -69,6 +69,7 @@
     uint32_t xcd_chunk;
     const uint32_t* hdr_pack;
     const uint32_t* hdr_quad;
+    uint32_t rc_stride = 0;
 };
 
 #ifdef BDDMMA_STAMPS
diff --git a/bdd_amd/csrc/kernels/narrow3.hpp b/bdd_amd/csrc/kernels/narrow3.hpp
--- a/bdd_amd/csrc/kernels/narrow3.hpp
+++ b/bdd_amd/csrc/kernels/narrow3.hpp
@@ -48,10 +48,31 @@
     }
 }
 
+#ifndef BDDMMA_N3_RC_DEFAULT
+#define BDDMMA_N3_RC_DEFAULT(REAL) true
+#endif
+#define N3_RC_DEFAULT(REAL) BDDMMA_N3_RC_DEFAULT(REAL)
+#ifndef BDDMMA_N3_RC_LDS_BUDGET
+#define BDDMMA_N3_RC_LDS_BUDGET (32u * 1024u)
+#endif
+constexpr uint32_t N3_RC_LDS_BUDGET = BDDMMA_N3_RC_LDS_BUDGET;
+constexpr uint32_t N3_RC_HEAD = 16;
+constexpr uint32_t n3_rc_stride(uint32_t real_size, uint32_t max_hops) { return (max_hops * (uint32_t)N3_W + 64u) * real_size; }
+template <uint32_t WS, uint32_t S>
+__device__ __forceinline__ uint32_t n3_rc_gather(uint32_t off, uint32_t hop_base)
+{
+    return off < WS ? hop_base + off : (off & S);
+}
+template <uint32_t WS>
+__device__ __forceinline__ uint32_t n3_rc_push(uint32_t off, uint32_t hop_base, uint32_t dummy)
+{
+    return off < WS ? hop_base + off : dummy;
+}
+
 #ifndef BDDMMA_N3_LOOKAHEAD
 #define BDDMMA_N3_LOOKAHEAD(REAL) (sizeof(REAL) == 8 ? 2 : BDDMMA_LOOKAHEAD)
 #endif
-template <typename REAL, int WPB, bool NT = false, int LA = BDDMMA_LOOKAHEAD, bool OV = false>
+template <typename REAL, int WPB, bool NT = false, int LA = BDDMMA_LOOKAHEAD, bool OV = false, bool RC = false>
 __device__ __forceinline__ void fwd_narrow3_body(const DevPtrs<REAL>& d, const PackDev& pk, const uint32_t* __restrict__ lrec,
                                                  const uint32_t* __restrict__ lrec_off, uint32_t lrec_words, REAL omega, uint32_t block_id)
 {
@@ -62,13 +83,13 @@
     extern __shared__ __attribute__((aligned(16))) unsigned char dyn_lds[];
     P2* sD = reinterpret_cast<P2*>(dyn_lds);
     __shared__ __attribute__((aligned(16))) unsigned char sF_[WPB][2][BUF];
-    __shared__ __attribute__((aligned(16))) unsigned char sT_[WPB][2][BUF];
+    __shared__ __attribute__((aligned(16))) unsigned char sT_[WPB][RC ? 1 : 2][RC ? 16 : BUF];
     __shared__ uint32_t sOffN_[WPB][HOP_WIN], sOffL_[WPB][HOP_WIN], sOffR_[WPB][HOP_WIN];
     const uint32_t tid = threadIdx.x;
     const int wave = __builtin_amdgcn_readfirstlane((int)(tid >> 6));
     const int lane = tid & 63;
     unsigned char* sFw = &sF_[wave][0][0];
-    unsigned char* sTw = &sT_[wave][0][0];
+    unsigned char* sTw = RC ? dyn_lds + pk.seg_off + (uint32_t)wave * pk.rc_stride : &sT_[wave][0][0];
     const uint32_t n_quads = (pk.n_packs + WPB - 1) / WPB;
     const uint32_t quad = block_to_pack(block_id, n_quads, pk.xcd_chunk);
     BDDMMA_EXIT_IF(quad >= n_quads, d)
@@ -117,18 +138,29 @@
             const uint32_t j = lane + 64 * r;
             lds_st<REAL>(sFw, j * S, (j < o[1] - o[0]) ? REAL(0) : INF);
         }
-#pragma unroll
-        for (int b = 0; b < 2; ++b) {
-            lds_st<REAL>(sTw, b * BUF + sink, REAL(0));
-            lds_st<REAL>(sTw, b * BUF + sink + S, INF);
+        if constexpr (RC) {
+            lds_st<REAL>(sTw, 0, REAL(0));
+            lds_st<REAL>(sTw, S, INF);
+        } else {
+#pragma unroll
+            for (int b = 0; b < 2; ++b) {
+                lds_st<REAL>(sTw, b * BUF + sink, REAL(0));
+                lds_st<REAL>(sTw, b * BUF + sink + S, INF);
+            }
         }
 #pragma unroll
         for (int i = 0; i < 2 * D; ++i) rc[i] = ldrec((uint32_t)i);
-        {
+        if constexpr (!RC) {
+#ifndef BDDMMA_EXP_NO_POT_TRAFFIC
             P2 t1;
             pot_pair_load<REAL, NT>(t1, hop_rsrc(Tp, o[1], o[2] - o[1]), 2u * (uint32_t)lane * S, o[1] * S);
 #pragma unroll
             for (int i = 0; i < D; ++i) pot_pair_load<REAL, NT>(tr[i], hop_rsrc(Tp, o[i + 2], o[i + 3] - o[i + 2]), 2u * (uint32_t)lane * S, o[i + 2] * S);
+#else
+            const P2 t1{REAL(0), REAL(0)};
+#pragma unroll
+            for (int i = 0; i <= D; ++i) tr[i] = t1;
+#endif
             if (2u * (uint32_t)lane < o[2] - o[1]) lds_st<P2>(sTw, 2u * (uint32_t)lane * S, t1);
         }
 #pragma unroll
@@ -138,6 +170,34 @@
             for (int i = 0; i < D; ++i) hop_load(Wr[i], rw, (uint32_t)lane * S, lb[i] * S);
         }
         wave_sync();
+        if constexpr (RC) {
+            constexpr int PD = 2;
+            const uint32_t nh = q1 - q0;
+            u4v pr[PD + 1];
+            P2 pc[PD + 1];
+            auto pld = [&](u4v& r, P2& c, uint32_t h) {
+                r = ldrec(h);
+                hop_load(c, rs.lohi, (uint32_t)lane * (uint32_t)sizeof(P2), hw.layer_off(q0 + h) * (uint32_t)sizeof(P2));
+            };
+#pragma unroll
+            for (int i = 0; i < PD; ++i) pld(pr[i], pc[i], nh > 1u + i ? nh - 1u - i : 0u);
+            for (uint32_t h = nh - 1; h >= 1 && h < nh; --h) {
+                pld(pr[PD], pc[PD], h > PD ? h - PD : 0u);
+                const u4v ra = pr[0];
+                const P2 c = pc[0];
+                const uint32_t flags = ra[2] >> 16;
+                const uint32_t tn = N3_RC_HEAD + h * (W * S);
+                const REAL tla = lds_ld<REAL>(sTw, n3_rc_gather<W * S, S>(ra[0] & 0xFFFFu, tn)), tha = lds_ld<REAL>(sTw, n3_rc_gather<W * S, S>(ra[0] >> 16, tn));
+                const REAL tlb = lds_ld<REAL>(sTw, n3_rc_gather<W * S, S>(ra[1] & 0xFFFFu, tn)), thb = lds_ld<REAL>(sTw, n3_rc_gather<W * S, S>(ra[1] >> 16, tn));
+                const REAL ta = rmin(c.y + tha, c.x + tla);
+                const REAL tb = rmin(c.y + thb, c.x + tlb);
+                if (flags & LREC_REAL) lds_st<REAL>(sTw, tn - W * S + (ra[2] & 0xFFFFu), ta);
+                if (flags & LREC_TWO) lds_st<REAL>(sTw, tn - W * S + (ra[2] & 0xFFFFu) + S, tb);
+                wave_sync();
+                shift(pr);
+                shift(pc);
+            }
+        }
     } else {
 #pragma unroll
         for (int i = 0; i < 2 * D; ++i) rc[i] = u4v{0u, 0u, 0u, 0u};
@@ -176,7 +236,9 @@
         const uint32_t stg = db + (lb[0] - gl0 + (uint32_t)lane) * (uint32_t)sizeof(P2);
         rc[2 * D] = ldrec(q - q0 + 2 * D);
 #ifndef BDDMMA_EXP_NO_HOP_LOADS
-        pot_pair_load<REAL, NT>(tr[D], hop_rsrc(Tp, o[D + 2], o[D + 3] - o[D + 2]), 2u * (uint32_t)lane * S, o[D + 2] * S);
+#ifndef BDDMMA_EXP_NO_POT_TRAFFIC
+        if constexpr (!RC) pot_pair_load<REAL, NT>(tr[D], hop_rsrc(Tp, o[D + 2], o[D + 3] - o[D + 2]), 2u * (uint32_t)lane * S, o[D + 2] * S);
+#endif
         hop_load(Lr[D], rs.lohi, (uint32_t)lane * (uint32_t)sizeof(P2), lb[D] * (uint32_t)sizeof(P2));
         if constexpr (OV) hop_load(Wr[D], rw, (uint32_t)lane * S, lb[D] * S);
 #endif
@@ -185,12 +247,16 @@
         const uint32_t flags = ra[2] >> 16;
         REAL fa, fb;
         lds_ld2(fa, fb, sFw, fc + (ra[2] & 0xFFFFu));
-        const REAL tla = lds_ld<REAL>(sTw, fc + (ra[0] & 0xFFFFu)), tha = lds_ld<REAL>(sTw, fc + (ra[0] >> 16));
-        const REAL tlb = lds_ld<REAL>(sTw, fc + (ra[1] & 0xFFFFu)), thb = lds_ld<REAL>(sTw, fc + (ra[1] >> 16));
+        const uint32_t tc = RC ? N3_RC_HEAD + (q - q0) * (W * S) : fc;
+        const uint32_t g0l = RC ? n3_rc_gather<W * S, S>(ra[0] & 0xFFFFu, tc) : tc + (ra[0] & 0xFFFFu), g0h = RC ? n3_rc_gather<W * S, S>(ra[0] >> 16, tc) : tc + (ra[0] >> 16);
+        const uint32_t g1l = RC ? n3_rc_gather<W * S, S>(ra[1] & 0xFFFFu, tc) : tc + (ra[1] & 0xFFFFu), g1h = RC ? n3_rc_gather<W * S, S>(ra[1] >> 16, tc) : tc + (ra[1] >> 16);
+        const REAL tla = lds_ld<REAL>(sTw, g0l), tha = lds_ld<REAL>(sTw, g0h);
+        const REAL tlb = lds_ld<REAL>(sTw, g1l), thb = lds_ld<REAL>(sTw, g1h);
         const P2 dd = lds_ld<P2>(dyn_lds, stg);
         const uint32_t o_new = hw.node_off(q + 2 * D + 3);
         const uint32_t l_next = hw.layer_off(q + D + 2);
-        if (2u * (uint32_t)lane < n3) lds_st<P2>(sTw, fn + 2u * (uint32_t)lane * S, tr[0]);
+        if constexpr (!RC)
+            if (2u * (uint32_t)lane < n3) lds_st<P2>(sTw, fn + 2u * (uint32_t)lane * S, tr[0]);
         lds_st<P2>(sFw, fn + 2u * (uint32_t)lane * S, P2{INF, INF});
         wave_sync();
         fa = (flags & LREC_REAL) ? fa : INF;
@@ -210,8 +276,8 @@
         lds_min(reinterpret_cast<REAL*>(sFw + fn + (ra[0] >> 16)), fa + nc.y);
         lds_min(reinterpret_cast<REAL*>(sFw + fn + (ra[1] & 0xFFFFu)), fb + nc.x);
         lds_min(reinterpret_cast<REAL*>(sFw + fn + (ra[1] >> 16)), fb + nc.y);
-#ifndef BDDMMA_EXP_NO_HOP_STORES
-        {
+#if !defined(BDDMMA_EXP_NO_HOP_STORES) && !defined(BDDMMA_EXP_NO_POT_TRAFFIC)
+        if constexpr (!RC) {
             const rsrc_t rf = hop_rsrc(Fp, nb, o[1] - o[0]);
             pot_store_layer<REAL>(fa, fb, (flags & LREC_TWO) != 0, rf, ra[3] & 0xFFFFu, nb * S, pk.nt_potentials);
         }
@@ -222,7 +288,7 @@
         shift(lb, l_next);
         shift(rc);
         shift(Lr);
-        shift(tr);
+        if constexpr (!RC) shift(tr);
         shift(Wr);
         ++q;
     };
@@ -243,14 +309,14 @@
 #ifndef BDDMMA_N3_WAVES
 #define BDDMMA_N3_WAVES(REAL) (sizeof(REAL) == 4 ? 5 : 4)
 #endif
-template <typename REAL, int WPB, bool NT = false, bool OV = false>
+template <typename REAL, int WPB, bool NT = false, bool OV = false, bool RC = false>
 __global__ void __launch_bounds__(64 * WPB) __attribute__((amdgpu_waves_per_eu(BDDMMA_N3_WAVES(REAL)))) k_fwd_narrow3(DevPtrs<REAL> d, PackDev pk, const uint32_t* __restrict__ lrec, const uint32_t* __restrict__ lrec_off,
                                                           uint32_t lrec_words, REAL omega)
 {
-    fwd_narrow3_body<REAL, WPB, NT, BDDMMA_N3_LOOKAHEAD(REAL), OV>(d, pk, lrec, lrec_off, lrec_words, omega, blockIdx.x);
-}
-
-template <typename REAL, int WPB, bool NT = false, int LA = BDDMMA_LOOKAHEAD, bool OV = false>
+    fwd_narrow3_body<REAL, WPB, NT, BDDMMA_N3_LOOKAHEAD(REAL), OV, RC>(d, pk, lrec, lrec_off, lrec_words, omega, blockIdx.x);
+}
+
+template <typename REAL, int WPB, bool NT = false, int LA = BDDMMA_LOOKAHEAD, bool OV = false, bool RC = false>
 __device__ __forceinline__ void bwd_narrow3_body(const DevPtrs<REAL>& d, const PackDev& pk, const uint32_t* __restrict__ lrec,
                                                  const uint32_t* __restrict__ lrec_off, uint32_t lrec_words, REAL omega, uint32_t block_id)
 {
@@ -266,6 +332,7 @@
     const int wave = __builtin_amdgcn_readfirstlane((int)(tid >> 6));
     const int lane = tid & 63;
     unsigned char* sTw = &sT_[wave][0][0];
+    unsigned char* const sFa = dyn_lds + pk.seg_off + (uint32_t)wave * pk.rc_stride;
     const uint32_t n_quads = (pk.n_packs + WPB - 1) / WPB;
     const uint32_t quad = block_to_pack(block_id, n_quads, pk.xcd_chunk);
     BDDMMA_EXIT_IF(quad >= n_quads, d)
@@ -306,7 +373,11 @@
     uint32_t q = q1;
     auto ldrec = [&](uint32_t qq) { return __builtin_amdgcn_raw_buffer_load_b128(rr, (uint32_t)lane * 16u, (rbase + (qq >= q0 ? qq - q0 : 0u) * 64u) * 16u, 0); };
     auto ldf = [&](P2& f, const u4v& r, uint32_t nb, uint32_t n) {
+#ifndef BDDMMA_EXP_NO_POT_TRAFFIC
         pot_pair_load<REAL, NT>(f, hop_rsrc(Fp, nb, n), r[3] & 0xFFFFu, nb * S);
+#else
+        f = P2{REAL(0), REAL(0)};
+#endif
     };
     const uint32_t sink = (W + 2 * (uint32_t)lane) * S;
     if (has_pack) {
@@ -324,9 +395,51 @@
         for (int i = 0; i < 2 * D; ++i) rc[i] = ldrec(q1 >= q0 + i + 1 ? q1 - 1 - i : q0);
 #pragma unroll
         for (int i = 0; i < D; ++i) {
-            ldf(fr[i], rc[i], o[i + 1], o[i] - o[i + 1]);
+            if constexpr (!RC) ldf(fr[i], rc[i], o[i + 1], o[i] - o[i + 1]);
             hop_load(Lr[i], rs.lohi, (uint32_t)lane * (uint32_t)sizeof(P2), lb[i + 1] * (uint32_t)sizeof(P2));
             if constexpr (OV) hop_load(Wr[i], rw, (uint32_t)lane * S, lb[i + 1] * S);
+        }
+        if constexpr (RC) {
+            constexpr int PD = 2;
+            const uint32_t nh = q1 - q0;
+            const uint32_t dummy = pk.rc_stride - 64u * S + (uint32_t)lane * S;
+            u4v pr[PD + 1];
+            P2 pc[PD + 1];
+            auto pld = [&](u4v& r, P2& c, uint32_t h) {
+                r = ldrec(q0 + h);
+                hop_load(c, rs.lohi, (uint32_t)lane * (uint32_t)sizeof(P2), hw.layer_off(q0 + h) * (uint32_t)sizeof(P2));
+            };
+#pragma unroll
+            for (int i = 0; i < PD; ++i) pld(pr[i], pc[i], (uint32_t)i);
+            {
+                const uint32_t n0 = nb_of(q0 + 1) - nb_of(q0);
+#pragma unroll
+                for (int r = 0; r < 2; ++r) {
+                    const uint32_t j = lane + 64 * r;
+                    lds_st<REAL>(sFa, j * S, (j < n0) ? REAL(0) : INF);
+                }
+            }
+            wave_sync();
+            for (uint32_t h = 0; h + 1 < nh; ++h) {
+                pld(pr[PD], pc[PD], h + PD);
+                const u4v ra = pr[0];
+                const P2 c = pc[0];
+                const uint32_t flags = ra[2] >> 16;
+                const uint32_t fc = h * (W * S), fn = fc + W * S;
+                REAL fa, fb;
+                lds_ld2(fa, fb, sFa, fc + ((ra[2] & 0xFFFFu) & (W * S - 1u)));
+                lds_st<P2>(sFa, fn + 2u * (uint32_t)lane * S, P2{INF, INF});
+                wave_sync();
+                fa = (flags & LREC_REAL) ? fa : INF;
+                fb = (flags & LREC_TWO) ? fb : INF;
+                lds_min(reinterpret_cast<REAL*>(sFa + n3_rc_push<W * S>(ra[0] & 0xFFFFu, fn, dummy)), fa + c.x);
+                lds_min(reinterpret_cast<REAL*>(sFa + n3_rc_push<W * S>(ra[0] >> 16, fn, dummy)), fa + c.y);
+                lds_min(reinterpret_cast<REAL*>(sFa + n3_rc_push<W * S>(ra[1] & 0xFFFFu, fn, dummy)), fb + c.x);
+                lds_min(reinterpret_cast<REAL*>(sFa + n3_rc_push<W * S>(ra[1] >> 16, fn, dummy)), fb + c.y);
+                wave_sync();
+                shift(pr);
+                shift(pc);
+            }
         }
     } else {
 #pragma unroll
@@ -365,7 +478,7 @@
         const uint32_t stg = db + (lb[1] - gl0 + (uint32_t)lane) * (uint32_t)sizeof(P2);
         rc[2 * D] = ldrec(q >= q0 + 2 * D ? q - 2 * D : q0);
 #ifndef BDDMMA_EXP_NO_HOP_LOADS
-        ldf(fr[D], rc[D], o[D + 1], o[D] - o[D + 1]);
+        if constexpr (!RC) ldf(fr[D], rc[D], o[D + 1], o[D] - o[D + 1]);
         hop_load(Lr[D], rs.lohi, (uint32_t)lane * (uint32_t)sizeof(P2), lb[D + 1] * (uint32_t)sizeof(P2));
         if constexpr (OV) hop_load(Wr[D], rw, (uint32_t)lane * S, lb[D + 1] * S);
 #endif
@@ -377,6 +490,7 @@
         const P2 dd = lds_ld<P2>(dyn_lds, stg);
         const uint32_t o_new = (q >= q0 + 2 * D + 1) ? nb_of(q - 1 - 2 * D) : o[2 * D + 1];
         const uint32_t l_next = hw.layer_off(q >= q0 + D + 1 ? q - 1 - D : q0);
+        if constexpr (RC) lds_ld2(fr[0].x, fr[0].y, sFa, (q - q0) * (W * S) + ((ra[2] & 0xFFFFu) & (W * S - 1u)));
         const REAL fa = (flags & LREC_REAL) ? fr[0].x : INF;
         const REAL fb = (flags & LREC_TWO) ? fr[0].y : INF;
         const REAL m0 = rmin((fa + c.x) + tla, (fb + c.x) + tlb);
@@ -400,8 +514,8 @@
             const rsrc_t rx = hop_rsrc(x_p, lb[1], lb[0] - lb[1]);
             hop_store((nc.y - nc.x) + mm, rx, (uint32_t)lane * S, lb[1] * S);
         }
-#ifndef BDDMMA_EXP_NO_HOP_STORES
-        {
+#if !defined(BDDMMA_EXP_NO_HOP_STORES) && !defined(BDDMMA_EXP_NO_POT_TRAFFIC)
+        if constexpr (!RC) {
             const rsrc_t rt = hop_rsrc(Tp, nb, o[0] - o[1]);
             pot_store_layer<REAL>(ta, tb, (flags & LREC_TWO) != 0, rt, ra[3] & 0xFFFFu, nb * S, pk.nt_potentials);
         }
@@ -412,7 +526,7 @@
         shift(lb, l_next);
         shift(rc);
         shift(Lr);
-        shift(fr);
+        if constexpr (!RC) shift(fr);
         shift(Wr);
     };
     while (q >= qs + HOP_UNROLL) {
@@ -439,11 +553,11 @@
     if (lane == 0) d.lb_partial[pk.lb_base + p] = s;
 }
 
-template <typename REAL, int WPB, bool NT = false, bool OV = false>
+template <typename REAL, int WPB, bool NT = false, bool OV = false, bool RC = false>
 __global__ void __launch_bounds__(64 * WPB) __attribute__((amdgpu_waves_per_eu(BDDMMA_N3_WAVES(REAL)))) k_bwd_narrow3(DevPtrs<REAL> d, PackDev pk, const uint32_t* __restrict__ lrec, const uint32_t* __restrict__ lrec_off,
                                                           uint32_t lrec_words, REAL omega)
 {
-    bwd_narrow3_body<REAL, WPB, NT, BDDMMA_N3_LOOKAHEAD(REAL), OV>(d, pk, lrec, lrec_off, lrec_words, omega, blockIdx.x);
-}
-
-}
+    bwd_narrow3_body<REAL, WPB, NT, BDDMMA_N3_LOOKAHEAD(REAL), OV, RC>(d, pk, lrec, lrec_off, lrec_words, omega, blockIdx.x);
+}
+
+}
diff --git a/bdd_amd/csrc/solver.hpp b/bdd_amd/csrc/solver.hpp
--- a/bdd_amd/csrc/solver.hpp
+++ b/bdd_amd/csrc/solver.hpp
@@ -66,6 +66,7 @@
     std::shared_ptr<int> lbfgs_attached = std::make_shared<int>(0);
     bool fused_small = false;
     bool nt_loads = false;
+    bool recomputes = false;
     virtual int run_plain(uint64_t max_iter, double tolerance, double slope, double time_limit, int verbose, bddmma_run_result* res) = 0;
     virtual int forward_mm(double omega, void* delta, int on_device) = 0;
     virtual int backward_mm(double omega, void* delta, int on_device) = 0;
diff --git a/bdd_amd/csrc/solver_impl.hpp b/bdd_amd/csrc/solver_impl.hpp
--- a/bdd_amd/csrc/solver_impl.hpp
+++ b/bdd_amd/csrc/solver_impl.hpp
@@ -117,6 +117,7 @@
     void costs_changed()
     {
         fwd_valid = bwd_valid = x_layer_valid = false;
+        rc_fwd_done = rc_lb_valid = false;
         ++cost_epoch;
     }
     CostQuot* d_cost_q = nullptr;
@@ -156,6 +157,11 @@
     SmallDev small{};
     uint32_t* d_small_lds = nullptr;
     bool use_narrow3 = false;
+    bool use_rc = false;
+    uint32_t rc_stride = 0;
+    bool rc_fwd_done = false;
+    bool rc_lb_valid = false;
+    bool rc_on() const { return use_rc && d_x_layer == nullptr; }
     uint32_t *d_lrec = nullptr, *d_lrec_off = nullptr;
     uint32_t lrec_words = 0;
     uint32_t huge_pack_width = 0;
@@ -473,6 +479,16 @@
                 lrec_words = (uint32_t)LR.rec.size();
                 use_narrow3 = true;
                 n3_nt = sizeof(REAL) == 8 && nt_potentials != 0;
+                if (res_hdr_ok && !(opts && (opts->variant_flags & 0x200000u))) {
+                    uint32_t max_hops = 0;
+                    for (uint32_t p = 0; p < nb_.n_packs; ++p) max_hops = std::max(max_hops, L.res.pack_hdr[8 * (size_t)p + 5] & 0xFFFFu);
+                    const uint32_t stride = n3_rc_stride((uint32_t)sizeof(REAL), max_hops);
+                    const uint32_t per_wave = stage_lds / L.ex.waves_per_block + 2 * (128 + 128) * (uint32_t)sizeof(REAL) + 3 * 64 * 4 + stride;
+                    if (max_hops >= 1 && max_hops <= 40 && per_wave <= N3_RC_LDS_BUDGET && (per_wave + 16) * L.ex.waves_per_block <= lds_cu - 1024 && (forced || N3_RC_DEFAULT(REAL))) {
+                        use_rc = true;
+                        rc_stride = stride;
+                    }
+                }
             }
         }
         if (nb_.n_packs && !use_res && !use_narrow3 && !wb_.n_packs && !hb_.n_packs && !narrow_seg && !narrow_gen && pack_width == 128 &&
@@ -483,6 +499,7 @@
             n12_nt = false;
 #endif
         nt_loads = n3_nt || n12_nt;
+        recomputes = use_rc;
         if (wb_.n_packs) {
             wide_threads = std::min<uint32_t>(1024, std::max<uint32_t>(64, ((wide_pack_width + 1) / 2 + 63) / 64 * 64));
             wide_npt = (wide_pack_width + wide_threads - 1) / wide_threads;
@@ -601,6 +618,7 @@
         uint32_t narrow_lds = 0, w = 1, seg_off = 0;
         const uint32_t *rec_tab = nullptr, *rec_off = nullptr;
         uint32_t rec_words = 0;
+        uint32_t rc_stride = 0;
         Kern<WideFn> wide;
         Kern<MixedFn> mixed;
         HugeFn huge = nullptr;
@@ -617,6 +635,7 @@
         Kern<LincombFn> lincomb[2];
     } kern;
     Sweep ov_sweep[2];
+    Sweep rc_sweep[2];
     template <int MODE, bool OV>
     Sweep resolve_sweep(bool bwd) const
     {
@@ -678,6 +697,16 @@
             kern.sweep[bwd][FWD_PLAIN] = resolve_sweep<FWD_PLAIN, false>(bwd);
             kern.sweep[bwd][FWD_SOLVE] = resolve_sweep<FWD_SOLVE, false>(bwd);
             kern.sweep[bwd][FWD_SOLUTION] = resolve_sweep<FWD_SOLUTION, false>(bwd);
+            if (use_rc) {
+                Sweep s = kern.sweep[bwd][FWD_SOLVE];
+                s.rec = pick<4, 8>(wpb, [&](auto W) -> RecFn { return bwd ? &k_bwd_narrow3<REAL, W.value, false, false, true> : &k_fwd_narrow3<REAL, W.value, false, false, true>; });
+                if constexpr (sizeof(REAL) == 8)
+                    if (n3_nt) s.rec = pick<4, 8>(wpb, [&](auto W) -> RecFn { return bwd ? &k_bwd_narrow3<REAL, W.value, true, false, true> : &k_fwd_narrow3<REAL, W.value, true, false, true>; });
+                s.seg_off = (s.narrow_lds + 15u) & ~15u;
+                s.rc_stride = rc_stride;
+                s.narrow_lds = s.seg_off + wpb * rc_stride;
+                rc_sweep[bwd] = s;
+            }
         }
         kern.ex_threads = exch_small ? EXS_THREADS : exch_medium ? EXM_THREADS : EX_THREADS;
         pick<EXS_THREADS, EXM_THREADS, EX_THREADS>(kern.ex_threads, [&](auto T_) {
@@ -727,6 +756,8 @@
         for (const auto& dir : k.sweep)
             for (const Sweep& s : dir)
                 if ((rc = raise_lds_limits(s))) return rc;
+        for (const Sweep& s : rc_sweep)
+            if ((rc = raise_lds_limits(s))) return rc;
         for (const auto* e : {&k.ex[0], &k.ex[1], &k.ex_w, &k.ex_raw})
             if ((rc = raise_lds_limit(*e))) return rc;
         for (const auto* e : {&k.seg[0], &k.seg[1], &k.seg_w})
@@ -746,6 +777,7 @@
         if (bwd) {
             lb_cached = false;
             ++lb_gen;
+            rc_lb_valid = false;
         }
         DevPtrs<REAL> d = ptrs(delta_lay);
         if (ov) d.omega_lay = d_omega_lay;
@@ -758,7 +790,8 @@
         } else {
             if (s.wide.fn) hipLaunchKernelGGL(s.wide.fn, dim3(wb_.n_packs), dim3(wide_threads), s.wide.lds, stream, d, pdev(wb_, nb_.n_packs), omega, wide_pack_width);
             if (nb_.n_packs) {
-                const PackDev pk = pdev(nb_, 0, s.seg_off);
+                PackDev pk = pdev(nb_, 0, s.seg_off);
+                pk.rc_stride = s.rc_stride;
                 const dim3 grid(narrow_grid(cdiv(nb_.n_packs, s.w))), block(64 * s.w);
                 if (s.res2)
                     hipLaunchKernelGGL(s.res2, grid, block, s.narrow_lds, stream, d_pack_hdr, d_quad_hdr, res2_ns, res2_nl, pk.n_packs, pk.xcd_chunk, d.stop, d.run_iter,
@@ -839,9 +872,10 @@
         bwd_valid = true;
         return BDDMMA_OK;
     }
+    int bound_ready() { return rc_lb_valid ? BDDMMA_OK : backward_run(); }
     int lower_bound(double* lb) override
     {
-        int rc = backward_run();
+        int rc = bound_ready();
         if (rc) return rc;
         if (lb_cached) {
             *lb = lb_cache;
@@ -879,7 +913,7 @@
     int lower_bound_enqueue(int slot) override
     {
         if (slot < 0 || slot > 1) { err = "lower_bound_enqueue: slot must be 0 or 1"; return BDDMMA_ERR_INVALID_ARGUMENT; }
-        int rc = backward_run();
+        int rc = bound_ready();
         if (rc) return rc;
         lb_slot_gen[slot] = lb_gen;
         if (lb_cached) {
@@ -903,7 +937,7 @@
             lb_slot_known[slot] = true;
         }
         *lb = lb_slot_value[slot];
-        if (lb_slot_gen[slot] == lb_gen && bwd_valid) {
+        if (lb_slot_gen[slot] == lb_gen && (bwd_valid || rc_lb_valid)) {
             lb_cache = *lb;
             lb_cached = true;
         }
@@ -926,28 +960,32 @@
         return BDDMMA_OK;
     }
 
-    int mma_forward(REAL omega, const REAL* delta_lay, bool ov = false)
+    int mma_forward(REAL omega, const REAL* delta_lay, bool ov = false, bool rc_pair = false)
     {
         int rc;
-        if (!bwd_valid && (rc = backward_run())) return rc;
-        rc = launch_sweep(false, ov ? ov_sweep[0] : kern.sweep[0][FWD_SOLVE], delta_lay, omega, BDDMMA_K_FORWARD_MM, ov);
+        if (!rc_pair && !bwd_valid && (rc = backward_run())) return rc;
+        rc = launch_sweep(false, rc_pair ? rc_sweep[0] : ov ? ov_sweep[0] : kern.sweep[0][FWD_SOLVE], delta_lay, omega, BDDMMA_K_FORWARD_MM, ov);
         x_layer_valid = false;
         if (rc) return rc;
-        fwd_valid = true;
+        fwd_valid = !rc_pair;
+        rc_fwd_done = rc_pair;
         bwd_valid = false;
-        return BDDMMA_OK;
-    }
-    int mma_backward(REAL omega, const REAL* delta_lay, bool ov = false)
-    {
-        if (!fwd_valid) {
+        rc_lb_valid = false;
+        return BDDMMA_OK;
+    }
+    int mma_backward(REAL omega, const REAL* delta_lay, bool ov = false, bool rc_pair = false)
+    {
+        if (!(rc_pair ? (rc_fwd_done || fwd_valid) : fwd_valid)) {
             err = "backward_mm requires a valid forward state (call forward_mm first)";
             return BDDMMA_ERR_STATE;
         }
-        int rc = launch_sweep(true, ov ? ov_sweep[1] : kern.sweep[1][BWD_SOLVE], delta_lay, omega, BDDMMA_K_BACKWARD_MM, ov);
+        int rc = launch_sweep(true, rc_pair ? rc_sweep[1] : ov ? ov_sweep[1] : kern.sweep[1][BWD_SOLVE], delta_lay, omega, BDDMMA_K_BACKWARD_MM, ov);
         if (rc) return rc;
         x_layer_valid = d_x_layer != nullptr;
         fwd_valid = false;
-        bwd_valid = true;
+        rc_fwd_done = false;
+        bwd_valid = !rc_pair;
+        rc_lb_valid = rc_pair;
         return BDDMMA_OK;
     }
     bool small_usable() const { return small_ok && !profiling && d_x_layer == nullptr; }
@@ -958,6 +996,7 @@
         x_layer_valid = false;
         fwd_valid = false;
         bwd_valid = true;
+        rc_fwd_done = rc_lb_valid = false;
         delta_var_valid = false;
     }
     int launch_small(REAL omega, uint32_t n, const RunStep& rstep)
@@ -993,9 +1032,10 @@
         int rc;
         if (small_usable() && !run_stop) return launch_small((REAL)omega, 1, RunStep{});
         prof_active = profiling && (prof_iter++ % prof_stride == 0);
-        if ((rc = mma_forward((REAL)omega, d_delta_lay))) return rc;
+        const bool rcp = rc_on();
+        if ((rc = mma_forward((REAL)omega, d_delta_lay, false, rcp))) return rc;
         if ((rc = exchange())) return rc;
-        if ((rc = mma_backward((REAL)omega, d_delta_lay))) return rc;
+        if ((rc = mma_backward((REAL)omega, d_delta_lay, false, rcp))) return rc;
         if ((rc = exchange(true))) return rc;
         return BDDMMA_OK;
     }
diff --git a/bdd_amd/csrc/solver_sm.hpp b/bdd_amd/csrc/solver_sm.hpp
--- a/bdd_amd/csrc/solver_sm.hpp
+++ b/bdd_amd/csrc/solver_sm.hpp
@@ -137,6 +137,7 @@
     bwd_valid = false;
     lb_cached = false;
     ++lb_gen;
+    rc_lb_valid = false;
     return launch_pull(sm_bwd_sweep());
 }
 
diff --git a/bdd_amd/solver.py b/bdd_amd/solver.py
--- a/bdd_amd/solver.py
+++ b/bdd_amd/solver.py
@@ -78,6 +78,8 @@
         return bool(self._L.bddmma_fused_small(self._h))
     def nontemporal_loads(self) -> bool:
         return bool(self._L.bddmma_nontemporal_loads(self._h))
+    def recomputes_potentials(self) -> bool:
+        return bool(self._L.bddmma_recomputes_potentials(self._h))
     def device_bytes(self): return int(self._L.bddmma_device_bytes(self._h))
     def device_allocated_bytes(self): return int(self._L.bddmma_device_allocated_bytes(self._h))
 
diff --git a/include/bdd_mma.h b/include/bdd_mma.h
--- a/include/bdd_mma.h
+++ b/include/bdd_mma.h
@@ -75,6 +75,7 @@
 int bddmma_solve_sweep_kind(const bddmma_solver* s);
 int bddmma_fused_small(const bddmma_solver* s);
 int bddmma_nontemporal_loads(const bddmma_solver* s);
+int bddmma_recomputes_potentials(const bddmma_solver* s);
 int bddmma_precision(const bddmma_solver* s);
 int bddmma_device(const bddmma_solver* s);
 int bddmma_num_bdds_per_var(const bddmma_solver* s, int32_t* out);
```

After: 8141. -7.1%, worse.
